# abusch/rustracer

Measured on AMD Instinct MI355X. Metric: Msamples/s, higher is better.
Workload: dtype f32; 1 GPU; cornell-box (synthetic S1, 32 triangles, 2 area lights) 1024x1024 PathIntegrator maxdepth=5 1024spp 02sequence box-filter; sampler_mode=pixel-keyed, light_distribution=cached across frames; first-frame build 32.0 ms

## Files before the change

include/rtx_hip.h:

```cpp
#ifndef RTX_HIP_H
#define RTX_HIP_H

#include <stdint.h>

#ifdef __cplusplus
extern "C" {
#endif

#define RT_OK 0
#define RT_ERR_INVALID (-1)
#define RT_ERR_NO_DEVICE (-2)
#define RT_ERR_HIP (-3)
#define RT_ERR_OOM (-4)
#define RT_ERR_UNSUPPORTED (-5)

typedef struct rt_bvh_node {
  float bmin[3];
  float bmax[3];
  uint32_t offset;
  uint16_t n_prims;
  uint8_t axis;
  uint8_t pad;
} rt_bvh_node;

// ... 132 lines not shown
  uint64_t camera_rays;
  uint64_t rays_closest, rays_shadow, rays_mis;
  uint64_t nodes_closest, nodes_shadow, nodes_mis;
  uint64_t tris_closest, tris_shadow, tris_mis;
  uint64_t paths_scrubbed;
  double ms_total;
  double ms_sampler, ms_raygen, ms_trace_closest, ms_trace_any, ms_trace_mis, ms_shade, ms_resolve, ms_film, ms_lightdist;
  uint64_t launches_trace_closest;
  uint64_t n_passes;
  uint64_t vertices_lambert_const, vertices_lambert, vertices_two_lobe, vertices_generic;
  double ms_shade_lambert_const, ms_shade_lambert, ms_shade_two_lobe, ms_shade_generic, ms_shade_bin, ms_shade_miss;
  uint64_t shade_section_cycles[32];
  uint64_t rays_mis_any, nodes_mis_any, tris_mis_any;
  double ms_trace_mis_any;
  double ms_gather;
  uint64_t rays_mis_not_cast;
  uint64_t rays_tail_not_cast;
  uint64_t launches_trace_path, launches_trace_shadow, launches_trace_mis, launches_trace_mis_any, launches_shade;
  uint64_t rays_shadow_not_cast;
} rt_stats;

#define RT_FLAG_COUNT_TRAVERSAL 1u
#define RT_FLAG_FILM_ON_DEVICE 2u
#define RT_FLAG_TIME_KERNELS 4u
#define RT_FLAG_COUNT_AS_RENDERED 8u
#define RT_FLAG_REF_STREAM 16u
#define RT_FLAG_FRAME_STATS 32u
#define RT_FLAG_FRAME_FEATURES 64u

typedef struct rt_scene rt_scene;

int rt_scene_create(const rt_scene_desc* desc, int device, rt_scene** out);
void rt_scene_destroy(rt_scene* scene);

int rt_bvh_build(const float* tri_p, uint32_t n_tris, int32_t max_prims_per_node, rt_bvh_node* nodes, uint32_t* n_nodes, int32_t* ordered,
                 float* ms_device );

int rt_mip_build(const float* rgb, int32_t width, int32_t height, int32_t px, int32_t py, const int32_t* s_first, const float* s_wts, const int32_t* t_first,
                 const float* t_wts, int32_t wrap, int32_t n_levels, const int32_t* lvl_w, const int32_t* lvl_h, const uint64_t* lvl_off, float* texels_out);
int rt_env_distribution(const rt_image* image, int32_t width, int32_t height, int32_t mode, int32_t il, float delta, const float* sin_theta,
                        float* func, float* cdf, float* func_int, float* marg_cdf, float* marg_func_int);

int rt_render(rt_scene* scene, const rt_camera* camera, const rt_film_desc* film, const rt_sampler_desc* sampler,
              const rt_path_desc* path, const rt_shard* shard, uint32_t flags, void* stream, float* film_xyzw, rt_stats* stats);

typedef struct rt_multi rt_multi;
int rt_multi_create(const rt_scene_desc* desc, const int32_t* devices, int32_t n_devices, rt_multi** out);
void rt_multi_destroy(rt_multi* multi);
int rt_multi_render(rt_multi* multi, const rt_camera* camera, const rt_film_desc* film, const rt_sampler_desc* sampler, const rt_path_desc* path,
                    int32_t chunks_per_device, uint32_t flags, float* film_xyzw, rt_stats* total, rt_stats* per_device);

int rt_trace_closest(rt_scene* scene, const float* rays, uint64_t n, float* hits, uint64_t counters[2]);
int rt_trace_any(rt_scene* scene, const float* rays, uint64_t n, uint32_t* occluded, uint64_t counters[2]);
int rt_trace_closest_device(rt_scene* scene, const void* d_rays, uint64_t n, void* d_hits, int reps, void* stream, float* ms_per_launch);

int rt_sampler_tables(int32_t spp, int32_t dimensions, uint64_t pixel0, uint64_t n_pixels, uint32_t* scrambles, uint16_t* perms);
int rt_sampler_tables_plain(int32_t spp, int32_t dimensions, uint64_t pixel0, uint64_t n_pixels, uint32_t* scrambles, uint16_t* perms);

int rt_offset_ray_origin(const float* p, const float* p_error, const float* n, const float* w, uint64_t count, float* out);

int rt_fourier_eval(rt_scene* scene, int32_t material, uint64_t n, const float* wo, const float* wi, const float* u, float* out);

int rt_texture_eval(rt_scene* scene, int32_t texture, uint64_t n, const float* records, float* rgb_out);

enum { RT_BSDF_FRONT_AUTO = 0, RT_BSDF_FRONT_GENERIC = 1, RT_BSDF_FRONT_LAMBERT = 2, RT_BSDF_FRONT_TWO_LOBE = 3, RT_BSDF_FRONT_TWO_LOBE_WIDE = 4 };
#define RT_BSDF_SURFACE_FLOATS 40
#define RT_BSDF_OUT_FLOATS 13
int rt_bsdf_eval(rt_scene* scene, int32_t material, int32_t front_end, uint64_t n, const float* surface, const float* wo, const float* wi, const float* u,
                 float* out);

#define RT_SAMPLES_MAX 134217728
int rt_render_samples(rt_scene* scene, const rt_camera* camera, const rt_film_desc* film, const rt_sampler_desc* sampler, const rt_path_desc* path,
                      uint32_t flags, void* stream, float* radiance, float* p_film, rt_stats* stats);

#define RT_FEATURE_FLOATS 16
#define RT_FEATURE_SAMPLES_MAX 33554432
int rt_render_sample_features(rt_scene* scene, const rt_camera* camera, const rt_film_desc* film, const rt_sampler_desc* sampler, const rt_path_desc* path,
                              uint32_t flags, void* stream, float* features);

enum { RT_FRAME_XYZW = 0, RT_FRAME_RGB = 1, RT_FRAME_RGB8 = 2, RT_FRAME_STATS = 3, RT_FRAME_FEATURES = 4 };
enum { RT_FRAME_SAMPLES_DONE = 0, RT_FRAME_SPP = 1, RT_FRAME_TABLES_RESIDENT = 2, RT_FRAME_STATE_BYTES = 3, RT_FRAME_SAMPLES_TAKEN = 4, RT_FRAME_ACTIVE_PIXELS = 5 };
typedef struct rt_frame rt_frame;
int rt_frame_begin(rt_scene* scene, const rt_camera* camera, const rt_film_desc* film, const rt_sampler_desc* sampler, const rt_path_desc* path,
                   const rt_shard* shard , uint32_t flags, uint64_t table_budget_bytes, rt_frame** out);
int rt_frame_advance(rt_frame* frame, int32_t n_samples, void* stream, rt_stats* stats );
int rt_frame_advance_adaptive(rt_frame* frame, int32_t n_samples, float threshold, float floor_y, int32_t min_samples, void* stream, rt_stats* stats );
int rt_frame_read(rt_frame* frame, int32_t what, float scale, uint32_t flags, void* stream, void* out);
int rt_frame_query(rt_frame* frame, int32_t what, uint64_t* value);
void rt_frame_end(rt_frame* frame);

typedef struct rt_multi_frame rt_multi_frame;
int rt_multi_frame_begin(rt_multi* multi, const rt_camera* camera, const rt_film_desc* film, const rt_sampler_desc* sampler, const rt_path_desc* path,
                         uint32_t flags, uint64_t table_budget_bytes, rt_multi_frame** out);
int rt_multi_frame_advance(rt_multi_frame* frame, int32_t n_samples, rt_stats* total , rt_stats* per_device );
int rt_multi_frame_advance_adaptive(rt_multi_frame* frame, int32_t n_samples, float threshold, float floor_y, int32_t min_samples, rt_stats* total, rt_stats* per_device);
int rt_multi_frame_read(rt_multi_frame* frame, int32_t what, float scale, uint32_t flags, void* out);
int rt_multi_frame_query(rt_multi_frame* frame, int32_t what, uint64_t* value);
void rt_multi_frame_end(rt_multi_frame* frame);

int rt_light_distribution(rt_scene* scene, int32_t n_voxels[3], float* func, float* cdf, float* func_int);

enum { RT_QUERY_LDS_RESIDENT = 0, RT_QUERY_LDS_NODES_TESTED = 1 ,
       RT_QUERY_LDS_OCCLUSION = 2 ,
       RT_QUERY_SHADOW_PAIRS = 3 ,
       RT_QUERY_SHADOW_EMPTY = 4 ,
       RT_QUERY_BSDF_LAUNCHED = 5  };
int rt_scene_query(rt_scene* scene, int32_t what);
int rt_link_tables(const rt_scene_desc* desc, int32_t mid, uint32_t* link_kept, uint32_t* link_full, uint64_t capacity_words, double* stats);
int rt_shadow_sets(const rt_scene_desc* desc, uint32_t* words, uint64_t capacity_words, int32_t n_voxels[3], uint64_t* stats);
int rt_sizeof(const char* struct_name);

const char* rt_last_error(void);
int rt_device_available(void);
const char* rt_version(void);

#ifdef __cplusplus
}
#endif
#endif
```

include/rtx_host.h:

```cpp
#ifndef RTX_HOST_H
#define RTX_HOST_H
#include <stdint.h>
#include "rtx_hip.h"

#ifdef __cplusplus
extern "C" {
#endif

typedef struct rtxh_scene rtxh_scene;

typedef struct rtxh_render_params {
  int32_t xres, yres;
  float crop[4];
  int32_t filter_kind;
  float filter_params[4];
  float film_scale, max_sample_luminance;
  float cam_to_world[16], cam_to_world_inv[16];
  float fov, lens_radius, focal_distance;
  int32_t spp, sampler_dims;
  int32_t max_depth; float rr_threshold; int32_t light_strategy;
  int32_t pixel_bounds[4];
  int32_t rank, world_size;
  uint32_t flags;
  float screen_window[4];
// ... 26 lines not shown
int rtxh_texture_words(rtxh_scene*, int32_t texture, float* out, int32_t capacity);
int rtxh_scene_add_material(rtxh_scene*, int32_t kind, const int32_t* slots16, int32_t remap_roughness, int32_t bump_texture );
int rtxh_scene_add_light(rtxh_scene*, int32_t kind, int32_t tri, const float* rgb3, int32_t two_sided, const float* vec3, int32_t mip,
                         const float* l2w16, const float* w2l16);
int rtxh_scene_commit(rtxh_scene*, int32_t max_prims_per_node);
int rtxh_scene_commit_device_bvh(rtxh_scene*, int32_t max_prims_per_node, float* ms_device);
int rtxh_scene_upload(rtxh_scene*, int32_t device);

int rtxh_scene_bvh_sizes(rtxh_scene*, int32_t* n_nodes, int32_t* n_prims);
int rtxh_scene_bvh_get(rtxh_scene*, float* bounds6, uint32_t* offset, uint16_t* n_prims, uint8_t* axis, int32_t* ordered);
int rtxh_camera_film_setup(const rtxh_render_params*, float* raster_to_camera16, float* dxdy6, float* filter_table256, int32_t* sample_bounds4,
                           int32_t* cropped4);
int rtxh_mip_level(rtxh_scene*, int32_t mip, int32_t level, int32_t* w, int32_t* h, float* rgb_out );
enum { RTXH_TABLE_TEXTURES = 0, RTXH_TABLE_MATERIALS, RTXH_TABLE_LIGHTS, RTXH_TABLE_P, RTXH_TABLE_N, RTXH_TABLE_UV, RTXH_TABLE_S, RTXH_TABLE_INDICES,
       RTXH_TABLE_TRI_MATERIAL, RTXH_TABLE_TRI_LIGHT, RTXH_TABLE_TRI_FLAGS,
       RTXH_TABLE_ENV_FUNC, RTXH_TABLE_ENV_CDF, RTXH_TABLE_ENV_ROW_INT, RTXH_TABLE_ENV_MARG_CDF,
       RTXH_TABLE_INSTANCES,
       RTXH_TABLE_EMITTERS,
       RTXH_TABLE_QUADRICS,
       RTXH_TABLE_OBJECT_BASE = 1000 ,
       RTXH_TABLE_OBJECT_EXTRA_BASE = 100000  };
typedef struct rtxh_emitter_info { float rgb[3]; int32_t two_sided; } rtxh_emitter_info;
typedef struct rtxh_instance_info { int32_t object; float o2w[16], w2o[16]; } rtxh_instance_info;
typedef struct rtxh_light_info { int32_t kind, tri; float rgb[3]; int32_t two_sided; float vec[3]; int32_t mip; float l2w[12], w2l[12]; } rtxh_light_info;
int rtxh_scene_inspect(rtxh_scene*, int32_t table, void* out, uint64_t capacity_bytes, uint64_t* n_items);
int rtxh_look_at(const float* pos, const float* look, const float* up, float* m16, float* m_inv16);

int rtxh_render(rtxh_scene*, const rtxh_render_params*, void* hip_stream, float* film_xyzw, rt_stats* stats);
int rtxh_render_samples(rtxh_scene*, const rtxh_render_params*, void* hip_stream, float* radiance, float* p_film, rt_stats* stats);
int rtxh_render_sample_features(rtxh_scene*, const rtxh_render_params*, void* hip_stream, float* features);
typedef struct rtxh_frame rtxh_frame;
int rtxh_frame_begin(rtxh_scene*, const rtxh_render_params*, uint64_t table_budget_bytes, rtxh_frame** out);
int rtxh_frame_advance(rtxh_frame*, int32_t n_samples, void* hip_stream, rt_stats* stats );
int rtxh_frame_advance_adaptive(rtxh_frame*, int32_t n_samples, float threshold, float floor_y, int32_t min_samples, void* hip_stream, rt_stats* stats );
int rtxh_frame_read(rtxh_frame*, int32_t what, float scale, uint32_t flags, void* hip_stream, void* out);
int rtxh_frame_query(rtxh_frame*, int32_t what, uint64_t* value);
void rtxh_frame_end(rtxh_frame*);
int rtxh_render_multi(rtxh_scene*, const rtxh_render_params*, const int32_t* devices, int32_t n_devices, int32_t chunks_per_device, float* film_xyzw,
                      rt_stats* total, rt_stats* per_device );
typedef struct rtxh_multi_frame rtxh_multi_frame;
int rtxh_multi_frame_begin(rtxh_scene*, const rtxh_render_params*, const int32_t* devices, int32_t n_devices, uint64_t table_budget_bytes, rtxh_multi_frame** out);
int rtxh_multi_frame_advance(rtxh_multi_frame*, int32_t n_samples, rt_stats* total, rt_stats* per_device);
int rtxh_multi_frame_advance_adaptive(rtxh_multi_frame*, int32_t n_samples, float threshold, float floor_y, int32_t min_samples, rt_stats* total, rt_stats* per_device);
int rtxh_multi_frame_read(rtxh_multi_frame*, int32_t what, float scale, uint32_t flags, void* out);
int rtxh_multi_frame_query(rtxh_multi_frame*, int32_t what, uint64_t* value);
void rtxh_multi_frame_end(rtxh_multi_frame*);
int rtxh_trace(rtxh_scene*, const float* rays, uint64_t n, int32_t any_hit, float* hits4_or_occ, uint64_t counters[2]);
int rtxh_trace_device(rtxh_scene*, const void* d_rays, uint64_t n, void* d_hits, int32_t reps, void* hip_stream, float* ms_per_launch);
int rtxh_light_distribution(rtxh_scene*, int32_t n_voxels[3], float* func, float* cdf, float* func_int);
int rtxh_scene_query(rtxh_scene*, int32_t what);
int rtxh_scene_device(rtxh_scene*, rt_scene** out);
int rtxh_scene_link_tables(rtxh_scene*, int32_t mid, uint32_t* link_kept, uint32_t* link_full, uint64_t capacity_words, double* stats);
int rtxh_scene_shadow_sets(rtxh_scene*, uint32_t* words, uint64_t capacity_words, int32_t n_voxels[3], uint64_t* stats);
int rtxh_sizeof(const char* struct_name);
const char* rtxh_last_error(void);

typedef struct rtxh_ply {
  int32_t n_verts, n_tris;
  float* P;
  float* N;
  float* UV;
  int32_t* idx;
  int32_t n_dropped_faces;
} rtxh_ply;
int rtxh_ply_read(const char* path, rtxh_ply* out);
void rtxh_ply_free(rtxh_ply* ply);
int rtxh_pfm_read(const char* path, int32_t* width, int32_t* height, float** rgb);
void rtxh_free(void* p);
int rtxh_image_read(const char* path, int32_t* width, int32_t* height, float** rgb);

int rtxh_spectrum_from_sampled(const float* lambda_nm, const float* values, int32_t n, float rgb[3]);
int rtxh_spectrum_blackbody(float temperature_kelvin, float scale, float rgb[3]);
void rtxh_copper(float eta_rgb[3], float k_rgb[3]);

typedef struct rtxh_pbrt_result {
  rtxh_scene* scene;
  rtxh_render_params params;
  int32_t max_prims_per_node;
  int32_t n_warnings;
  char film_filename[512];
} rtxh_pbrt_result;
int rtxh_pbrt_load(const char* path, rtxh_pbrt_result* out);
int rtxh_pbrt_parse(const char* text, const char* base_dir, rtxh_pbrt_result* out);
int rtxh_pbrt_tokens(const char* text, char* out, uint64_t capacity);

#ifdef __cplusplus
}
#endif
#endif
```

rustracer_amd/csrc/rtx_hip.hip:

```cpp
#include <hip/hip_runtime.h>
#include <chrono>
#include <cmath>
#include <cstdio>
#include <cstring>
#include <string>
#include <vector>
#include <limits>
#include <algorithm>
#include <memory>
#include <atomic>
#include <mutex>
#include <thread>

#include "../../include/rtx_hip.h"
#include "rtx_kernels.h"
#include "rtx_shade_launch.h"
#include "rtx_ref_launch.h"

using namespace rtx;
#include "rtx_scene_plan.h"

static thread_local std::string g_err;
static int fail(int code, const std::string& msg) { g_err = msg; return code; }
static bool env_is(const char* name, char c) { const char* e = getenv(name); return e && e[0] == c; }
// ... 10 lines not shown
  hipError_t ensure(size_t n) {
    if (n <= bytes && p) return hipSuccess;
    if (p) { (void)hipFree(p); p = nullptr; bytes = 0; }
    hipError_t e = hipMalloc(&p, n > 0 ? n : 16);
    if (e == hipSuccess) bytes = n;
    return e;
  }
  void release() { if (p) (void)hipFree(p); p = nullptr; bytes = 0; }
  template <class T> T* as() const { return (T*)p; }
};

struct SamplerPlan {
  unsigned spp = 0, dims = 0, seg_len = 0, n_segs = 0;
  DevBuf segs, magic, dirty, partners;
};

struct rt_scene {
  int device = 0;
  SamplerPlan sampler_plan;
  DScene d{};
  bool small = false;
  bool lambert_materials = false;
  bool lds_records_q = false;
  bool lds_tables = false;
  bool lds_mats = false;
  bool lds_records = false;
  bool lambert_only = false;
  bool lean_qlights = false;
  bool lean_shade = false;
  int stack_depth = 64;
  unsigned n_nodes = 0, n_tris = 0; int n_lights = 0;
  DevBuf link8, link8_full; unsigned lds_nodes_tested = 0;
  DevBuf pairs, tmin_stack;
  DevBuf top_pairs, deep_stack; bool use_top = false;
  bool top_for_closest = false;
  bool use_pairs = false;
  bool deep_column = false;
  DevBuf quads; bool use_quads = false; int quad_stack_depth = 0;
  DevBuf tri_rec;
  DevBuf nodes, tri_p, tri_n, tri_uv, tri_s, tri_alpha, spheres, textures, images, materials, lights, texels, dist, guides, prim_class;
  DevBuf fourier;
  std::vector<int> mat_kind, mat_table;
  std::vector<uint64_t> fourier_at;
  bool has_spheres = false;
  bool has_instances = false;
  DevBuf instances;
  bool mid = false;
  bool general_prims = false;
  bool obj_general = false;
  bool has_masks = false;
  bool masked_emitters = false;
  DevBuf ld_func, ld_cdf, ld_int, ld_mark, ld_list, ld_slot, ld_guide, ld_rows8, ld_dense8;
  bool shadow_sets = false; RtShadowSets shadow; DevBuf ld_shadow;
  DevBuf self;
  int ld_strategy_built = -1; bool ld_all_voxels = false;
  std::mutex render_mutex;
  DevBuf ws[32];
  DevBuf film_acc, own_acc, film_out, counters, stats, filter_table, ref_samples, ref_stack;
  DevBuf samples_rad, samples_pf;
  DevBuf samples_feat;
  DevBuf feat;
  DevBuf bsdf_self, bsdf_tris;
  int bsdf_launched = -1;
  std::vector<int> mat_class;
  DevBuf bin_words, bin_sorted, bin_at;
  unsigned n_materials = 0, n_code_classes = 0, n_lambert_classes = 0, n_small_classes = 0, n_wide_classes = 0;
  DevBuf scrambles[2], perms[2];
  hipStream_t aux_stream = nullptr;
  hipEvent_t ev_tables[2][3] = {{nullptr, nullptr, nullptr}, {nullptr, nullptr, nullptr}}, ev_batch_done[2] = {nullptr, nullptr}, ev_frame_begin = nullptr;
  int n_cu = 256;
  std::vector<hipEvent_t> event_pool;
  ~rt_scene() {
    for (hipEvent_t e : event_pool) (void)hipEventDestroy(e);
    for (int i = 0; i < 2; ++i) { for (int g = 0; g < 3; ++g) if (ev_tables[i][g]) (void)hipEventDestroy(ev_tables[i][g]); if (ev_batch_done[i]) (void)hipEventDestroy(ev_batch_done[i]); }
    if (ev_frame_begin) (void)hipEventDestroy(ev_frame_begin);
    if (aux_stream) (void)hipStreamDestroy(aux_stream);
  }
};

extern "C" const char* rt_last_error(void) { return g_err.c_str(); }
extern "C" const char* rt_version(void) { return "rtx-mi355x 0.5 (gfx950 wavefront path tracer)"; }
extern "C" int rt_sizeof(const char* name) {
  if (!name) return -1;
#define RT_SZ(T) if (!strcmp(name, #T)) return (int)sizeof(T);
  RT_SZ(rt_bvh_node) RT_SZ(rt_tri_meta) RT_SZ(rt_sphere) RT_SZ(rt_instance) RT_SZ(rt_texture) RT_SZ(rt_image) RT_SZ(rt_material) RT_SZ(rt_light) RT_SZ(rt_scene_desc)
  RT_SZ(rt_camera) RT_SZ(rt_film_desc) RT_SZ(rt_sampler_desc) RT_SZ(rt_path_desc) RT_SZ(rt_shard) RT_SZ(rt_stats)
#undef RT_SZ
  return -1;
}
extern "C" int rt_device_available(void) {
  int n = 0;
  if (hipGetDeviceCount(&n) != hipSuccess || n <= 0) return 0;
  return 1;
}

static int upload(DevBuf& b, const void* src, size_t bytes) {
  HIP_TRY(b.ensure(bytes));
  if (bytes) HIP_TRY(hipMemcpy(b.p, src, bytes, hipMemcpyHostToDevice));
  return RT_OK;
}

static void fill_ewa_lut() {
  float lut[128];
  for (int i = 0; i < 128; ++i) {
    float alpha = 2.0f;
    float r2 = (float)i / (128.0f - 1.0f);
// ... 148 lines not shown
  a.material = material; a.surface = surface ? b[4].as<float4>() : nullptr; a.wo = b[0].as<float>(); a.wi = b[1].as<float>(); a.u = b[2].as<float>(); a.n = (unsigned)n; a.out = b[3].as<float>();
  const unsigned grid = (unsigned)std::min<uint64_t>((n + 255) / 256, (uint64_t)scene->n_cu * 16u);
  rtx_launch_bsdf_eval(mode, const_tex, grid, nullptr, d, a);
  HIP_TRY(hipGetLastError());
  scene->bsdf_launched = 2 * mode + (const_tex ? 1 : 0);
  HIP_TRY(hipMemcpy(out, b[3].p, no, hipMemcpyDeviceToHost));
  return RT_OK;
}
extern "C" int rt_link_tables(const rt_scene_desc* desc, int32_t mid, uint32_t* link_kept, uint32_t* link_full, uint64_t capacity_words, double* stats) {
  if (!desc || !desc->nodes || desc->n_nodes == 0 || !desc->tri_p || !desc->tri_meta || !link_kept || !link_full) return fail(RT_ERR_INVALID, "null argument");
  const size_t words = (size_t)9 * desc->n_nodes + 9;
  if (desc->n_nodes > (mid ? RT_MID_NODES : RT_SMALL_NODES) || desc->n_tris > (uint64_t)(mid ? RT_MID_TRIS : RT_SMALL_TRIS) || desc->n_instances != 0) return fail(RT_ERR_INVALID, "not an LDS-sized scene");
  if (capacity_words < words) return fail(RT_ERR_INVALID, "link table capacity too small");
  {
    const uint32_t nn = desc->n_nodes;
    std::vector<uint32_t> size(nn, 1u);
    for (uint32_t i = nn; i-- > 0;) {
      const rt_bvh_node& n = desc->nodes[i];
      if (n.n_prims != 0) {
        if ((uint64_t)n.offset + n.n_prims > desc->n_tris) return fail(RT_ERR_INVALID, "leaf range out of bounds");
        if (n.n_prims >= (1u << (15 - RT_LINK_OFF_BITS(mid ? RT_MID_NODES : RT_SMALL_NODES)))) return fail(RT_ERR_INVALID, "a leaf holds more primitives than a link word can name");
        continue;
      }
      if (i + 1 >= nn || n.offset != i + 1 + size[i + 1] || n.offset >= nn) return fail(RT_ERR_INVALID, "nodes are not a pre-order tree");
      size[i] = 1u + size[i + 1] + size[n.offset];
    }
    if (size[0] != nn) return fail(RT_ERR_INVALID, "nodes are not one tree");
    for (uint64_t t = 0; t < desc->n_tris; ++t)
      if (desc->tri_meta[t].flags & RT_PRIM_SPHERE) {
        uint32_t k; memcpy(&k, desc->tri_p + 9 * t + 6, 4);
        if (!desc->spheres || k >= desc->n_spheres) return fail(RT_ERR_INVALID, "sphere index out of range");
      }
  }
  RtLinkTables lt;
  rt_build_link_tables(desc, mid != 0, stats != nullptr, lt);
  memcpy(link_kept, lt.link_kept.data(), words * 4); memcpy(link_full, lt.link_full.data(), words * 4);
  if (stats) for (int w = 0; w < 9; ++w) { stats[w] = (double)lt.n_rays[w]; stats[9 + w] = lt.tests_all[w]; stats[18 + w] = lt.tests_kept[w]; }
  return RT_OK;
}
extern "C" int rt_shadow_sets(const rt_scene_desc* desc, uint32_t* words, uint64_t capacity_words, int32_t n_voxels[3], uint64_t* stats) {
  if (!desc || !desc->nodes || desc->n_nodes == 0 || !desc->tri_p || !desc->tri_meta) return fail(RT_ERR_INVALID, "null argument");
  bool plain = desc->n_instances == 0 && desc->n_spheres == 0 && desc->n_nodes <= RT_SMALL_NODES && desc->n_tris <= RT_SMALL_TRIS;
  for (uint32_t i = 0; i < desc->n_tris && plain; ++i) if (desc->tri_meta[i].flags & ~(uint32_t)RT_SHADOW_PLAIN_FLAGS) plain = false;
  if (!shadow_sets_apply(desc, plain)) return fail(RT_ERR_INVALID, "not a scene the shadow sets serve (LDS-resident plain triangles, two triangle lights)");
  int32_t lp[2] = {0, 0};
  for (uint32_t k = 0; k < desc->n_lights; ++k) lp[k] = desc->lights[k].prim;
  RtShadowSets ss;
  rt_build_shadow_sets(desc->tri_p, desc->n_tris, lp, (int)desc->n_lights, desc->nodes[0].bmin, desc->nodes[0].bmax, ss);
  if (n_voxels) { n_voxels[0] = ss.nvox[0]; n_voxels[1] = ss.nvox[1]; n_voxels[2] = ss.nvox[2]; }
  if (stats) { stats[0] = ss.pairs; stats[1] = ss.empty; }
  if (words) {
    if (capacity_words < ss.word.size()) return fail(RT_ERR_INVALID, "rt_shadow_sets: capacity too small");
    std::memcpy(words, ss.word.data(), ss.word.size() * 4);
  }
  return RT_OK;
}

extern "C" int rt_scene_query(rt_scene* s, int32_t what) {
  if (!s) return fail(RT_ERR_INVALID, "null scene");
  if (what == RT_QUERY_LDS_RESIDENT) return s->small ? 1 : 0;
  if (what == RT_QUERY_LDS_NODES_TESTED) return (s->small || s->mid) ? (int)s->lds_nodes_tested : 0;
  if (what == RT_QUERY_LDS_OCCLUSION) return s->mid ? 1 : 0;
  if (what == RT_QUERY_SHADOW_PAIRS) return s->shadow_sets ? (int)s->shadow.pairs : 0;
  if (what == RT_QUERY_SHADOW_EMPTY) return s->shadow_sets ? (int)s->shadow.empty : 0;
  if (what == RT_QUERY_BSDF_LAUNCHED) return s->bsdf_launched < 0 ? 0 : s->bsdf_launched + 1;
  return fail(RT_ERR_INVALID, "unknown rt_scene_query item");
}

static int build_light_distribution(rt_scene* s, int strategy, hipStream_t stream, bool all_voxels = false) {
  DScene& d = s->d;
  if (s->ld_strategy_built == strategy && (s->ld_all_voxels || !all_voxels)) return RT_OK;
  s->ld_strategy_built = -1;
  const int nl = s->n_lights;
  size_t ld_rows_built = 1;
  const bool uniform = strategy == 1 || nl == 1 || nl == 0;
  int glog = -1;
  if (nl >= 64 && nl <= 65534) { const long q = guide_quarters(); glog = 0; while (glog < 16 && (long)(2 << glog) * q <= 4l * nl) ++glog; }
  d.ld_glog = glog; d.ld_guide = nullptr;
  if (uniform) {
    const int n = nl > 0 ? nl : 1;
    std::vector<float> func(n, 1.0f), cdf(n + 1, 0.0f);
    for (int i = 1; i < n + 1; ++i) cdf[i] = cdf[i - 1] + func[i - 1] / (float)n;
    float func_int = cdf[n];
    if (func_int == 0.0f) for (int i = 1; i < n + 1; ++i) cdf[i] = (float)i / (float)n;
    else for (int i = 1; i < n + 1; ++i) cdf[i] /= func_int;
    int rc;
    if ((rc = upload(s->ld_func, func.data(), func.size() * 4)) != RT_OK) return rc;
    if ((rc = upload(s->ld_cdf, cdf.data(), cdf.size() * 4)) != RT_OK) return rc;
    if ((rc = upload(s->ld_int, &func_int, 4)) != RT_OK) return rc;
    if (glog >= 0) {
      const int G = 1 << glog; std::vector<unsigned short> g((size_t)G + 1); int i = 0;
      for (int k = 0; k <= G; ++k) { const float x = (float)k / (float)G; while (i <= n && cdf[i] <= x) ++i; g[k] = (unsigned short)i; }
      if ((rc = upload(s->ld_guide, g.data(), g.size() * 2)) != RT_OK) return rc;
    }
    d.ld_uniform = 1; d.nvox[0] = d.nvox[1] = d.nvox[2] = 1;
  } else {
    float diag[3] = {d.wb_max.x - d.wb_min.x, d.wb_max.y - d.wb_min.y, d.wb_max.z - d.wb_min.z};
    int ext = diag[0] > diag[1] ? (diag[0] > diag[2] ? 0 : 2) : (diag[1] > diag[2] ? 1 : 2);
    float b_max = diag[ext];
    size_t total = 1;
    for (int i = 0; i < 3; ++i) {
      float r = roundf(diag[i] / b_max * 64.0f);
      unsigned v = (r != r || r <= 0.0f) ? 0u : (unsigned)r;
      d.nvox[i] = (int)(v > 1u ? v : 1u);
      total *= (size_t)d.nvox[i];
    }
// ... 93 lines not shown
static size_t deep_stack_bytes(const rt_scene* s) {
  if (!s->use_top) return 0;
  return (size_t)std::max(top_grid(s), top_grid(s, true)) * RT_TOP_BLOCK * (size_t)std::max(1, s->stack_depth - RT_TOP_LDS_DEPTH) * 4;
}
static int scene_from_plan(const RtScenePlan& p, const rt_scene_desc* desc, int device, rt_scene** out) {
  if (device >= 0) HIP_TRY(hipSetDevice(device));
  int dev = 0; HIP_TRY(hipGetDevice(&dev));
  std::unique_ptr<rt_scene> owner(new rt_scene());
  rt_scene* s = owner.get();
  s->device = dev;
  hipDeviceProp_t prop; if (hipGetDeviceProperties(&prop, dev) == hipSuccess) s->n_cu = prop.multiProcessorCount;
  s->n_nodes = desc->n_nodes; s->n_tris = desc->n_tris; s->n_lights = (int)desc->n_lights; s->n_materials = desc->n_materials;
  s->small = p.small; s->mid = p.mid; s->general_prims = p.general_prims; s->obj_general = p.obj_general; s->has_masks = p.has_masks; s->has_spheres = p.has_spheres;
  s->has_instances = p.has_instances; s->masked_emitters = p.masked_emitters; s->lambert_only = p.lambert_only; s->lambert_materials = p.lambert_materials;
  s->lean_shade = p.lean_shade; s->lean_qlights = p.lean_qlights; s->lds_records = p.lds_records; s->lds_records_q = p.lds_records_q; s->lds_tables = p.lds_tables;
  s->lds_mats = p.lds_mats; s->use_pairs = p.use_pairs; s->use_top = p.use_top; s->top_for_closest = p.top_for_closest; s->use_quads = p.use_quads;
  s->deep_column = p.deep_column; s->shadow_sets = p.shadow_sets; s->shadow = p.shadow; s->stack_depth = p.stack_depth; s->quad_stack_depth = p.quad_stack_depth;
  s->mat_kind = p.mat_kind; s->mat_table = p.mat_table; s->mat_class = p.mat_class; s->fourier_at = p.fourier_at;
  s->n_code_classes = p.n_code_classes; s->n_lambert_classes = p.n_lambert_classes; s->n_small_classes = p.n_small_classes; s->n_wide_classes = p.n_wide_classes;
  if (s->mid) {
    int fit_any = 0, fit_closest = 0;
    if (hipOccupancyMaxActiveBlocksPerMultiprocessor(&fit_any, (const void*)(k_trace<true, false, 1024, 16, 0, 1>), 1024, 0) != hipSuccess) fit_any = 0;
    if (hipOccupancyMaxActiveBlocksPerMultiprocessor(&fit_closest, (const void*)(k_trace<false, false, 1024, 16, 0, 1>), 1024, 0) != hipSuccess) fit_closest = 0;
    (void)hipGetLastError();
    if (fit_any < 1 || fit_closest < 1) s->mid = false;
  }
  const bool links = s->small || s->mid;
  if (links) s->lds_nodes_tested = p.links.nodes_tested;
  int rc = RT_OK;
  auto up = [&rc](DevBuf& b, const void* src, size_t bytes) { if (rc == RT_OK) rc = upload(b, src, bytes); };
  auto up_all = [&up](DevBuf& b, const auto& v) { up(b, v.data(), v.size() * sizeof(v[0])); };
  auto room = [&rc](DevBuf& b, size_t bytes, const char* what) { if (rc == RT_OK && bytes && b.ensure(bytes) != hipSuccess) rc = fail(RT_ERR_OOM, what); };
  up(s->nodes, desc->nodes, sizeof(rt_bvh_node) * (size_t)desc->n_nodes);
  up_all(s->tri_p, p.tri_p);
  if (desc->tri_n) up(s->tri_n, desc->tri_n, (size_t)desc->n_tris * 36);
  if (desc->tri_uv) up(s->tri_uv, desc->tri_uv, (size_t)desc->n_tris * 24);
  if (desc->tri_s) up(s->tri_s, desc->tri_s, (size_t)desc->n_tris * 36);
  if (p.has_masks) up(s->tri_alpha, desc->tri_alpha, (size_t)desc->n_tris * 8);
  if (p.has_spheres) up(s->spheres, desc->spheres, (size_t)desc->n_spheres * sizeof(rt_sphere));
  if (p.has_instances) up_all(s->instances, p.instances);
  up_all(s->texels, p.texels); up_all(s->fourier, p.fourier);
  std::vector<DImage> images = p.images;
  for (DImage& im : images) im.texels = s->texels.as<float4>();
  up_all(s->images, images); up_all(s->textures, p.textures); up_all(s->materials, p.materials); up_all(s->prim_class, p.prim_class);
  up_all(s->dist, p.dist); up_all(s->guides, p.guides);
  std::vector<DLight> lights = p.lights;
  for (DLight& l : lights)
    if (l.kind == RT_LIGHT_INFINITE) {
      rt_blob_rebase(l.cf, s->dist.p); rt_blob_rebase(l.func_int, s->dist.p); rt_blob_rebase(l.mfunc, s->dist.p); rt_blob_rebase(l.mcdf, s->dist.p);
      rt_blob_rebase(l.guide, s->guides.p); rt_blob_rebase(l.mguide, s->guides.p);
    }
  up_all(s->lights, lights);
  if (links) { up_all(s->link8_full, p.links.link_full); up_all(s->link8, p.links.link_kept); }
  if (p.use_pairs) up_all(s->pairs, p.pairs);
  if (p.use_top) up_all(s->top_pairs, p.top_pairs);
  if (p.use_quads) up_all(s->quads, p.quads);
  room(s->tmin_stack, tmin_stack_bytes(s), "traversal stack allocation failed");
  room(s->deep_stack, deep_stack_bytes(s), "traversal stack allocation failed");
  room(s->tri_rec, (size_t)desc->n_tris * 128, "shade record allocation failed");
  room(s->self, sizeof(DScene), "scene record allocation failed");
  if (rc != RT_OK) return rc;
  DScene& d = s->d;
  d.nodes = s->nodes.as<float4>(); d.n_nodes = desc->n_nodes;
  d.tri_p = s->tri_p.as<float4>(); d.n_tris = desc->n_tris;
  d.tri_n = s->tri_n.as<float>(); d.tri_uv = s->tri_uv.as<float>(); d.tri_s = s->tri_s.as<float>();
  d.tri_alpha = s->tri_alpha.as<int2>();
  d.spheres = s->spheres.as<DSphere>();
  d.instances = s->instances.as<DInstance>(); d.n_instances = s->has_instances ? desc->n_instances : 0u; d.n_top_prims = p.n_top_prims;
  d.textures = s->textures.as<DTexture>(); d.images = s->images.as<DImage>(); d.materials = s->materials.as<DMaterial>(); d.lights = s->lights.as<DLight>();
  d.fourier = s->fourier.as<unsigned>();
  d.n_materials = (int)desc->n_materials; d.n_textures = (int)desc->n_textures; d.n_images = (int)desc->n_images;
  d.n_lights = (int)desc->n_lights; d.n_infinite = p.n_infinite;
  for (int k = 0; k < 4; ++k) d.infinite_ids[k] = p.infinite_ids[k];
  d.wb_min = f3{desc->nodes[0].bmin[0], desc->nodes[0].bmin[1], desc->nodes[0].bmin[2]};
  d.wb_max = f3{desc->nodes[0].bmax[0], desc->nodes[0].bmax[1], desc->nodes[0].bmax[2]};
  d.ld_uniform = 1; d.nvox[0] = d.nvox[1] = d.nvox[2] = 1; d.ld_glog = -1; d.ld_guide = nullptr;
  d.needs_differentials = p.needs_differentials;
#ifdef RT_ABLATE
  d.dbg = env_int("RTX_DBG", 0);
#endif
  d.obj_pairs = p.obj_pairs; d.obj_general = s->obj_general ? 1 : 0;
  d.link8_full = s->link8_full.as<unsigned>(); d.link8 = s->link8.as<unsigned>();
  d.pairs = s->pairs.as<float4>(); d.top_pairs = s->top_pairs.as<float4>(); d.n_top = (unsigned)(p.top_pairs.size() / 16); d.quads = s->quads.as<float4>();
  fill_ewa_lut();
  d.tri_rec = s->tri_rec.as<float4>();
  hipLaunchKernelGGL(k_tri_records, dim3((desc->n_tris + 255u) / 256u), dim3(256), 0, nullptr, d, s->tri_rec.as<float4>());
  d.n_lights_all = (int)p.n_all_lights;
  if (p.n_all_lights) hipLaunchKernelGGL(k_light_consts, dim3((p.n_all_lights + 255u) / 256u), dim3(256), 0, nullptr, d, s->lights.as<DLight>(), (int)p.n_all_lights);
  if (hipGetLastError() != hipSuccess) return fail(RT_ERR_HIP, "constant precomputation launch failed");
  d.prim_class = s->prim_class.as<unsigned short>();
  d.route_quadric_hits = p.route_quadric_hits;
  d.self = s->self.as<DScene>();
  HIP_TRY(hipMemcpy(s->self.p, &d, sizeof(DScene), hipMemcpyHostToDevice));
  HIP_TRY(hipDeviceSynchronize());
  *out = owner.release();
  return RT_OK;
}

extern "C" int rt_scene_create(const rt_scene_desc* desc, int device, rt_scene** out) {
  if (!desc || !out) return fail(RT_ERR_INVALID, "null argument");
  RtScenePlan plan; std::string why;
  if (const int rc = rt_plan_scene(desc, plan, why)) return fail(rc, why);
  if (!rt_device_available()) return fail(RT_ERR_NO_DEVICE, "no HIP device visible; this backend has no CPU fallback");
  return scene_from_plan(plan, desc, device, out);
}
static bool inst_loop_kernel(const rt_scene* s) { return s->has_instances && !s->has_masks && !s->has_spheres && s->use_pairs && s->d.obj_pairs; }
// ... 61 lines not shown
        if (s->use_quads && s->quad_stack_depth <= 32) {
          RT_GEN_LAUNCH3((k_trace_quad<128, 32, RT_GEN_ALL>), (k_trace_quad<128, 32, RT_GEN_NO_MASKS>), (k_trace_quad<128, 32, RT_GEN_INSTANCES_ONLY>), (trace_grid<ANY, false, 128, 32>(s)), 128, RT_KARGS, s->tmin_stack.as<float>(), refill_min);
          return;
        }
      }
      if (s->use_pairs && s->use_top && (ANY || s->top_for_closest)) {
        RT_GEN_LAUNCH((k_trace_top<ANY, RT_TOP_BLOCK, RT_GEN_ALL>), (k_trace_top<ANY, RT_TOP_BLOCK, RT_GEN_NO_MASKS>), (top_grid(s, ANY)), RT_TOP_BLOCK, RT_KARGS, s->tmin_stack.as<float>(), s->deep_stack.as<unsigned>(), refill_min);
        return;
      }
      if (s->use_pairs) {
        if (s->stack_depth <= 32) RT_GEN_LAUNCH3((k_trace_pair<ANY, 128, 32, RT_GEN_ALL>), (k_trace_pair<ANY, 128, 32, RT_GEN_NO_MASKS>), (k_trace_pair<ANY, 128, 32, RT_GEN_INSTANCES_ONLY>), (trace_grid<ANY, false, 128, 32>(s)), 128, RT_KARGS, s->tmin_stack.as<float>(), refill_min);
        else RT_GEN_LAUNCH3((k_trace_pair<ANY, 128, 64, RT_GEN_ALL>), (k_trace_pair<ANY, 128, 64, RT_GEN_NO_MASKS>), (k_trace_pair<ANY, 128, 64, RT_GEN_INSTANCES_ONLY>), (trace_grid<ANY, false, 128, 64>(s)), 128, RT_KARGS, s->tmin_stack.as<float>(), refill_min);
        return;
      }
#undef RT_GEN_LAUNCH3
#undef RT_GEN_LAUNCH
    }
    if (s->stack_depth > 64) hipLaunchKernelGGL((k_trace_big<ANY, COUNT, 64, 128, true>), dim3(trace_grid<ANY, false, 64, 128>(s)), dim3(64), 0, stream, RT_KARGS, st_nodes, st_tris);
    else if (s->stack_depth <= 32) hipLaunchKernelGGL((k_trace_big<ANY, COUNT, 128, 32, true>), dim3(trace_grid<ANY, false, 128, 32>(s)), dim3(128), 0, stream, RT_KARGS, st_nodes, st_tris);
    else hipLaunchKernelGGL((k_trace_big<ANY, COUNT, 128, 64, true>), dim3(trace_grid<ANY, false, 128, 64>(s)), dim3(128), 0, stream, RT_KARGS, st_nodes, st_tris);
    return;
  }
  if constexpr (!COUNT) {
    if (s->mid && (ANY || mid_closest_on())) {
      hipLaunchKernelGGL((k_trace<ANY, false, 1024, 16, 0, 1>), dim3((unsigned)s->n_cu), dim3(1024), 0, stream, RT_KARGS, st_nodes, st_tris);
      return;
    }
    if (s->small) {
      hipLaunchKernelGGL((k_trace<ANY, false, 256, 16>), dim3(trace_grid<ANY, true, 256, 16>(s, true)), dim3(256), 0, stream, RT_KARGS, st_nodes, st_tris);
      return;
    }
  }
  if (s->small) {
    if (s->stack_depth <= 16) hipLaunchKernelGGL((k_trace<ANY, true, 256, 16>), dim3(trace_grid<ANY, true, 256, 16>(s)), dim3(256), 0, stream, RT_KARGS, st_nodes, st_tris);
    else if (s->stack_depth <= 32) hipLaunchKernelGGL((k_trace<ANY, true, 256, 32>), dim3(trace_grid<ANY, true, 256, 32>(s)), dim3(256), 0, stream, RT_KARGS, st_nodes, st_tris);
    else hipLaunchKernelGGL((k_trace<ANY, true, 128, 64>), dim3(trace_grid<ANY, true, 128, 64>(s)), dim3(128), 0, stream, RT_KARGS, st_nodes, st_tris);
  } else {
    if (s->stack_depth <= 32) launch_trace_hbm<ANY, COUNT, 128, 32>(RT_ARGS);
    else launch_trace_hbm<ANY, COUNT, 128, 64>(RT_ARGS);
  }
#undef RT_KARGS
#undef RT_ARGS
}
static bool closest_is_k_trace(const rt_scene* s, bool count) {
  if (s->general_prims) return !count && !s->obj_general && s->small;
  return s->small || (!count && s->mid && mid_closest_on());
}
template <bool ANY>
static void launch_trace(rt_scene* s, bool count, const TraceIO& io, const unsigned* queue, const unsigned* count_ptr, unsigned shard_cap, unsigned count_static,
                         unsigned long long* stats, int st_rays, int st_nodes, int st_tris, hipStream_t stream) {
  if (count) launch_trace_c<ANY, true>(s, io, queue, count_ptr, shard_cap, count_static, stats, st_rays, st_nodes, st_tris, stream);
  else launch_trace_c<ANY, false>(s, io, queue, count_ptr, shard_cap, count_static, stats, st_rays, st_nodes, st_tris, stream);
}
static TraceIO trace_io_planar(const float4* ro, const float4* rd, float4* hits, unsigned* occ) {
  TraceIO io{}; io.ray_o = ro; io.ray_d = rd; io.ray_stride = 1; io.hits = hits; io.hit_stride = 1; io.hit_b2 = 0; io.occluded = occ; io.occ_stride = 1;
  io.shadow_masks = 1;
  return io;
}

static int trace_batch(rt_scene* s, const float* rays, uint64_t n, bool any, float* hits, uint32_t* occluded, uint64_t counters[2]) {
  if (!s || !rays || n == 0 || n > 0x7fffffffull) return fail(RT_ERR_INVALID, "bad trace batch");
  HIP_TRY(hipSetDevice(s->device));
  DevBuf ro, rd, out, st;
  HIP_TRY(ro.ensure(n * 16)); HIP_TRY(rd.ensure(n * 16)); HIP_TRY(out.ensure(n * 16)); HIP_TRY(st.ensure(ST_COUNT * 8));
  std::vector<float> o(n * 4), d(n * 4);
  for (uint64_t i = 0; i < n; ++i) {
    const float* r = rays + 8 * i;
    o[4 * i] = r[0]; o[4 * i + 1] = r[1]; o[4 * i + 2] = r[2]; o[4 * i + 3] = r[3];
    d[4 * i] = r[4]; d[4 * i + 1] = r[5]; d[4 * i + 2] = r[6]; d[4 * i + 3] = 0.0f;
  }
  HIP_TRY(hipMemcpy(ro.p, o.data(), n * 16, hipMemcpyHostToDevice));
  HIP_TRY(hipMemcpy(rd.p, d.data(), n * 16, hipMemcpyHostToDevice));
  HIP_TRY(hipMemset(st.p, 0, ST_COUNT * 8));
  const TraceIO io = trace_io_planar(ro.as<float4>(), rd.as<float4>(), any ? nullptr : out.as<float4>(), any ? out.as<unsigned>() : nullptr);
  if (any) launch_trace<true>(s, counters != nullptr, io, nullptr, nullptr, 0, (unsigned)n, st.as<unsigned long long>(), ST_RAYS_SHADOW, ST_NODES_SHADOW, ST_TRIS_SHADOW, nullptr);
  else launch_trace<false>(s, counters != nullptr, io, nullptr, nullptr, 0, (unsigned)n, st.as<unsigned long long>(), ST_RAYS_CLOSEST, ST_NODES_CLOSEST, ST_TRIS_CLOSEST, nullptr);
  HIP_TRY(hipGetLastError());
  HIP_TRY(hipDeviceSynchronize());
  if (any) HIP_TRY(hipMemcpy(occluded, out.p, n * 4, hipMemcpyDeviceToHost));
  else HIP_TRY(hipMemcpy(hits, out.p, n * 16, hipMemcpyDeviceToHost));
  if (counters) {
    unsigned long long h[ST_COUNT];
    HIP_TRY(hipMemcpy(h, st.p, sizeof(h), hipMemcpyDeviceToHost));
    counters[0] = any ? h[ST_NODES_SHADOW] : h[ST_NODES_CLOSEST];
    counters[1] = any ? h[ST_TRIS_SHADOW] : h[ST_TRIS_CLOSEST];
  }
  return RT_OK;
}
extern "C" int rt_trace_closest(rt_scene* s, const float* rays, uint64_t n, float* hits, uint64_t counters[2]) { return trace_batch(s, rays, n, false, hits, nullptr, counters); }
extern "C" int rt_trace_any(rt_scene* s, const float* rays, uint64_t n, uint32_t* occluded, uint64_t counters[2]) { return trace_batch(s, rays, n, true, nullptr, occluded, counters); }

extern "C" int rt_trace_closest_device(rt_scene* s, const void* d_rays, uint64_t n, void* d_hits, int reps, void* stream_, float* ms_per_launch) {
  if (!s || !d_rays || !d_hits || n == 0 || reps <= 0) return fail(RT_ERR_INVALID, "bad arguments");
  HIP_TRY(hipSetDevice(s->device));
  hipStream_t stream = (hipStream_t)stream_;
  const float4* ro = (const float4*)d_rays; const float4* rd = ro + n;
  hipEvent_t e0, e1; HIP_TRY(hipEventCreate(&e0)); HIP_TRY(hipEventCreate(&e1));
  HIP_TRY(hipEventRecord(e0, stream));
  const TraceIO io = trace_io_planar(ro, rd, (float4*)d_hits, nullptr);
  for (int i = 0; i < reps; ++i) launch_trace<false>(s, false, io, nullptr, nullptr, 0, (unsigned)n, nullptr, 0, 0, 0, stream);
  HIP_TRY(hipEventRecord(e1, stream));
  HIP_TRY(hipEventSynchronize(e1));
  float ms = 0; HIP_TRY(hipEventElapsedTime(&ms, e0, e1));
  if (ms_per_launch) *ms_per_launch = ms / (float)reps;
  (void)hipEventDestroy(e0); (void)hipEventDestroy(e1);
  return RT_OK;
}

static unsigned next_pow2(unsigned v) { unsigned p = 1; while (p < v) p <<= 1; return p; }
static unsigned sampler_lanes_per_block(unsigned spp) {
  unsigned l = (32u * 1024u) / ((spp + 2u) * 2u);
  if (l >= 64u) return 64u;
  if (l >= 32u) return 32u;
  if (l >= 16u) return 16u;
  if (l >= 8u) return 8u;
  return 4u;
}

static void pcg_advance_constants(unsigned long long n, unsigned long long& mul, unsigned long long& sum) {
  unsigned long long cur_mul = 0x5851f42d4c957f2dULL, cur_sum = 1ull;
  mul = 1ull; sum = 0ull;
  while (n) {
    if (n & 1ull) { sum = sum * cur_mul + cur_sum; mul *= cur_mul; }
    cur_sum = (cur_mul + 1ull) * cur_sum; cur_mul *= cur_mul;
    n >>= 1;
  }
}
static int sampler_plan_prepare(SamplerPlan& pl, unsigned spp_, unsigned dims_) {
  unsigned &spp = pl.spp, &dims = pl.dims, &seg_len = pl.seg_len, &n_segs = pl.n_segs;
  DevBuf &segs = pl.segs, &magic = pl.magic, &dirty = pl.dirty;
  {
    if (spp == spp_ && dims == dims_ && segs.p) return RT_OK;
    seg_len = spp_ < 256u ? spp_ : 256u;
    const unsigned per_half = spp_ / seg_len;
    std::vector<SamplerSeg> h;
    unsigned long long pos = 0;
    for (unsigned t = 0; t < 2u * dims_; ++t) {
      const unsigned n_scr = t < dims_ ? 1u : 2u;
      for (unsigned half = 0; half < 2u; ++half)
        for (unsigned g = 0; g < per_half; ++g) {
          SamplerSeg sg{};
          const bool first = half == 0u && g == 0u;
          const unsigned long long start = first ? pos : pos + n_scr + (unsigned long long)half * spp_ + (unsigned long long)g * seg_len;
// ... 317 lines not shown
    for (const Want& w : want) if (!w.buf->p || w.buf->bytes < w.bytes) grow += w.bytes;
    size_t held = 0;
    for (const Want& w : want) if (w.buf->p && w.buf->bytes < w.bytes) held += w.buf->bytes;
    size_t mem_free = 0, mem_total = 0;
    HIP_TRY(hipMemGetInfo(&mem_free, &mem_total));
    if (grow > mem_free + held - std::min<size_t>(mem_free + held, (size_t)256 << 20)) continue;
    bool ok = true;
    for (const Want& w : want) if (w.buf->ensure(w.bytes) != hipSuccess) { ok = false; break; }
    if (ok) break;
    (void)hipGetLastError();
  }
  if (!s->aux_stream) {
    int lo = 0, hi = 0; (void)hipDeviceGetStreamPriorityRange(&lo, &hi);
    HIP_TRY(hipStreamCreateWithPriority(&s->aux_stream, hipStreamNonBlocking, lo));
    for (int i = 0; i < 2; ++i) { for (int g = 0; g < 3; ++g) HIP_TRY(hipEventCreateWithFlags(&s->ev_tables[i][g], hipEventDisableTiming)); HIP_TRY(hipEventCreateWithFlags(&s->ev_batch_done[i], hipEventDisableTiming)); }
    HIP_TRY(hipEventCreateWithFlags(&s->ev_frame_begin, hipEventDisableTiming));
  }
  float4* const d_out = (flags & RT_FLAG_FILM_ON_DEVICE) ? (float4*)film_xyzw : s->film_out.as<float4>();
  float4* const d_samples_rad = (flags & RT_FLAG_FILM_ON_DEVICE) ? (float4*)samples_rad : s->samples_rad.as<float4>();
  float2* const d_samples_pf = !samples_pf ? nullptr : ((flags & RT_FLAG_FILM_ON_DEVICE) ? (float2*)samples_pf : s->samples_pf.as<float2>());
  FeatureOut fo{};
  if (fsamples) { fo.samples = (flags & RT_FLAG_FILM_ON_DEVICE) ? (float4*)samples_feat : s->samples_feat.as<float4>(); fo.wx0 = wx0; fo.wy0 = wy0; fo.ww = wx1 - wx0; }
  else if (features) { fo.nd = s->feat.as<float4>(); fo.ah = fo.nd + cap; }
  if (!samples && !fsamples && !fr) {
    HIP_TRY(hipMemcpyAsync(s->filter_table.p, film->filter_table, 1024, hipMemcpyHostToDevice, stream));
    HIP_TRY(hipMemsetAsync(s->film_acc.p, 0, (size_t)cw * ch * 16, stream));
  }
  HIP_TRY(hipMemsetAsync(s->stats.p, 0, ST_COUNT * 8, stream));

  PassState ps{};
  ps.spp = spp; ps.spp_log2 = spp_log2; ps.dims = dims;
  auto gen_of = [&](int b) { PathGen g; char* p = (char*)s->ws[b].p; g.o = (float4*)p; g.d = (float4*)(p + n_slots * 16); g.beta = (float4*)(p + n_slots * 32); g.st = (uint4*)(p + n_slots * 48); return g; };
  const PathGen gen0 = gen_of(B_GEN0), gen1 = gen_of(B_GEN1);
  ps.hit = s->ws[B_HIT].as<float4>(); ps.lacc = s->ws[B_LACC].as<float4>(); ps.pfilm = s->ws[B_PFILM].as<float2>();
  { char* p = (char*)s->ws[B_SH].p; ps.sh.o = (float4*)p; ps.sh.d = (float4*)(p + cap * 16); ps.sh.add = (float4*)(p + cap * 32);
    char* q = (char*)s->ws[B_MI].p; ps.mi.o = (float4*)q; ps.mi.d = (float4*)(q + cap * 16); ps.mi.hit = (float4*)(q + cap * 32); ps.mi.a = (float4*)(q + cap * 48);
    ps.mi.b = (float4*)(q + cap * 64); ps.mi.c = (float4*)(q + cap * 80); ps.mi.flags = (unsigned*)(q + cap * 96); }
  ps.occ_sh = s->ws[B_OCCSH].as<unsigned char>(); ps.occ_mi = s->ws[B_OCCMI].as<unsigned char>();
  ps.q_shadow = s->ws[B_QSH].as<unsigned>(); ps.q_mis = s->ws[B_QMI].as<unsigned>(); ps.q_misany = s->ws[B_QMA].as<unsigned>();
  ps.own_acc = s->own_acc.as<float4>(); ps.shard_cap = shard_cap;
  ps.stats = s->stats.as<unsigned long long>();

  if ((rc = sampler_plan_prepare(s->sampler_plan, spp, dims)) != RT_OK) return rc;
  if ((rc = sampler_set_lds_limits(spp)) != RT_OK) return rc;
  TraceIO io_path{}, io_shadow{}, io_mis{}, io_mis_any{};
  {
    io_path.ray_stride = 1; io_path.hits = ps.hit; io_path.hit_stride = 1; io_path.hit_b2 = 1; io_path.queue_is_slots = 1;
    io_shadow.ray_o = ps.sh.o; io_shadow.ray_d = ps.sh.d; io_shadow.ray_stride = 1; io_shadow.occluded = (unsigned*)ps.occ_sh; io_shadow.occ_stride = 0;
    io_shadow.shadow_masks = 1; io_shadow.lacc = ps.lacc; io_shadow.lacc_stride = 1; io_shadow.direct_add = ps.sh.add; io_shadow.add_stride = 1;
    io_mis.ray_o = ps.mi.o; io_mis.ray_d = ps.mi.d; io_mis.ray_stride = 1; io_mis.hits = ps.mi.hit; io_mis.hit_stride = 1; io_mis.hit_b2 = 0;
    io_mis_any = io_mis; io_mis_any.shadow_masks = 0; io_mis_any.hits = nullptr; io_mis_any.occluded = (unsigned*)ps.occ_mi; io_mis_any.occ_stride = 0;
  }
  const bool count = (flags & RT_FLAG_COUNT_TRAVERSAL) != 0;
  const unsigned pgrid = (unsigned)s->n_cu * 8u;
  const unsigned sblock = 256u, sgrid = pgrid;
  unsigned long long* dstats = s->stats.as<unsigned long long>();

  const char* ov = getenv("RTX_K0_OVERLAP");
  hipStream_t aux = (ov && ov[0] == '0') ? stream : s->aux_stream;
  if (build_tables) {
    HIP_TRY(hipEventRecord(s->ev_frame_begin, stream));
    HIP_TRY(hipStreamWaitEvent(aux, s->ev_frame_begin, 0));
  }
  int tables_rc = RT_OK;
  std::vector<std::pair<unsigned long long, unsigned long long>> batches;
  for (unsigned long long first = 0; first < owned_pixels;) {
    const unsigned long long npx = (first == 0 && lead_pixels) ? lead_pixels : std::min(chunk_pixels, owned_pixels - first);
    batches.push_back({first, npx}); first += npx;
  }
  if (resident && !fr->tables_built) {
    fr->scr_off.clear(); fr->perm_off.clear();
    size_t so = 0, po = 0;
    for (const auto& b : batches) {
      fr->scr_off.push_back(so); fr->perm_off.push_back(po);
      so += ((size_t)b.second * 3 * dims * 4 + 255) & ~(size_t)255; po += ((size_t)(b.second * table_bytes_per_pixel) + 255) & ~(size_t)255;
    }
    if (so > fr->scrambles.bytes || po > fr->perms.bytes) return fail(RT_ERR_INVALID, "rt_frame_advance: the batches' sampler tables do not fit the frame's buffers");
  }
  if (resident && fr->scr_off.size() != batches.size()) return fail(RT_ERR_INVALID, "rt_frame_advance: the batch cut changed under resident sampler tables");
  auto scrambles_of = [&](size_t b, int buf) { return resident ? (unsigned*)((char*)fr->scrambles.p + fr->scr_off[b]) : s->scrambles[buf].as<unsigned>(); };
  auto perms_of = [&](size_t b, int buf) { return resident ? (unsigned short*)((char*)fr->perms.p + fr->perm_off[b]) : s->perms[buf].as<unsigned short>(); };
  TableGroups tgroups = table_groups_frame(dims, !(fp.lens_radius > 0.0f));
  auto launch_tables = [&](size_t b, int buf) {
    FrameParams f2 = fp; f2.chunk_first = batches[b].first;
    tm.begin(&stats.ms_sampler, aux);
    const int trc = launch_sampler_tables(s->sampler_plan, f2, (unsigned)batches[b].second, 0ull, 0, scrambles_of(b, buf), perms_of(b, buf), aux, tgroups, s->ev_tables[buf]);
    if (trc != RT_OK && tables_rc == RT_OK) tables_rc = trc;
    tm.end(aux);
  };
  if (!batches.empty() && build_tables) launch_tables(0, 0);
  for (size_t batch_no = 0; batch_no < batches.size(); ++batch_no) {
    const unsigned long long first = batches[batch_no].first, npx = batches[batch_no].second;
    const int buf = (int)(batch_no & 1ull);
    fp.chunk_first = first;
    ps.n_pixels = (unsigned)npx; ps.n_pixels_recip = npx > 1 ? (unsigned)((1ull << 32) / npx) : 0xffffffffu;
    ps.scrambles = scrambles_of(batch_no, buf); ps.perms = perms_of(batch_no, buf);
    if (build_tables && batch_no + 1 < batches.size()) {
      if (batch_no >= 1 && !resident) HIP_TRY(hipStreamWaitEvent(aux, s->ev_batch_done[buf ^ 1], 0));
      launch_tables(batch_no + 1, buf ^ 1);
    }
    const unsigned batch_pass_samples = (unsigned)std::min<unsigned long long>(spp, std::max<unsigned long long>(pass_samples, cap / npx));
    if (tables_rc != RT_OK) { (void)hipDeviceSynchronize(); return tables_rc; }
    if (build_tables) HIP_TRY(hipStreamWaitEvent(stream, s->ev_tables[buf][0], 0));
    for (unsigned s0 = s_begin; s0 < s_end; s0 += batch_pass_samples) {
      ps.s0 = s0; ps.n_samples = std::min(batch_pass_samples, s_end - s0); ps.cap = (unsigned)(npx * ps.n_samples);
      ps.q_in = nullptr; ps.in = gen1; ps.out = gen0;
      HIP_TRY(hipMemsetAsync(s->counters.p, 0, counter_words * 4, stream));
      if (use_bins) HIP_TRY(hipMemsetAsync(s->bin_words.p, 0, (size_t)(fp.max_depth + 1) * bin_stride * 4, stream));
      unsigned* const cb = s->counters.as<unsigned>();
      ps.cnt_in = nullptr; ps.cnt_out = cb;
      ps.all_in_bounds = all_in_bounds ? 1 : 0;
      const int fresh_planes = all_in_bounds ? ((s->lambert_only && s->lds_records) ? (shade_split ? 3 : RT_FRESH_RECORDS_LDS) : RT_FRESH_RECORDS) : 0;
      ps.fresh = fresh_planes;
      ps.shadow_sets = (s->shadow_sets && !count) ? 1 : 0;
      ps.mis_any = (has_infinite && (!count || (flags & RT_FLAG_COUNT_AS_RENDERED))) ? 1 : 0;
      static const bool reach_off = env_is("RTX_MIS_REACH", '0');
      ps.skip_unreachable_mis = (!reach_off && (!count || (flags & RT_FLAG_COUNT_AS_RENDERED))) ? 1 : 0;
      static const bool tail_off = env_is("RTX_DEAD_TAIL", '0');
      ps.skip_dead_tail = (!tail_off && (!count || (flags & RT_FLAG_COUNT_AS_RENDERED))) ? 1 : 0;
      const int skip_dead_tail = ps.skip_dead_tail;
      tm.begin(&stats.ms_raygen);
      if (active_mask) hipLaunchKernelGGL(k_raygen_masked, dim3(pgrid), dim3(256), 0, stream, fp, ps, active_mask);
      else hipLaunchKernelGGL(k_raygen, dim3(pgrid), dim3(256), 0, stream, fp, ps);
      tm.end();
      for (int bounce = 0; bounce <= fp.max_depth; ++bounce) {
        ps.cnt_in = cb + (size_t)bounce * RT_NQ * RT_QSHARDS * RT_CNT_STRIDE; ps.cnt_out = cb + (size_t)(bounce + 1) * RT_NQ * RT_QSHARDS * RT_CNT_STRIDE;
        std::swap(ps.in, ps.out);
        if (bounce == 0 && all_in_bounds) ps.cnt_in = nullptr;
        ps.skip_dead_tail = (features && bounce == 0 && fp.max_depth == 1) ? 0 : skip_dead_tail;
        ps.fresh = bounce == 0 ? fresh_planes : 0;
        io_path.ray_o = ps.in.o; io_path.ray_d = ps.in.d;
        const bool split_launch = shade_split && (bounce >= 1 || all_in_bounds);
        io_path.hit_mask = split_launch ? s->ws[B_HITMASK].as<unsigned long long>() : nullptr;
        tm.begin(&stats.ms_trace_closest);
        launch_trace<false>(s, count, io_path, ps.cnt_in, ps.cnt_in, ps.shard_cap, ps.cap, dstats, ST_RAYS_CLOSEST, ST_NODES_CLOSEST, ST_TRIS_CLOSEST, stream);
        tm.end();
        if (bounce <= 1 && build_tables) HIP_TRY(hipStreamWaitEvent(stream, s->ev_tables[buf][bounce + 1], 0));
#define RT_SHADE(MODE, P) stats.launches_shade += 1, launch_shade<MODE>(gshade, lean_shade, bounce >= 1, sgrid, sblock, stream, s->d, fp, P, qlights, lds_shade)
        if (s->lambert_only) {
          tm.begin(&stats.ms_shade_lambert_const);
          if (split_launch) rtx_launch_shade_split(bounce == 0, sgrid, stream, s->d, fp, ps, io_path.hit_mask);
          else rtx_launch_shade_const(s->lds_records ? 1 : (s->lds_tables ? 3 : 0), sgrid, sblock, stream, s->d, fp, ps);
          tm.end(); stats.launches_shade += 1;
        }
        else if (s->lambert_materials) { tm.begin(&stats.ms_shade_lambert); RT_SHADE(3, ps); tm.end(); }
        else if (!use_bins) { tm.begin(&stats.ms_shade_generic); RT_SHADE(0, ps); tm.end(); }
        else {
          tm.begin(&stats.ms_shade_bin);
          unsigned* bw = s->bin_words.as<unsigned>() + (size_t)bounce * bin_stride;
          unsigned* hist = bw; unsigned* cursor = bw + (RT_BIN_MAX + 1); unsigned* sorted_cnt = cursor + (size_t)(RT_BIN_MAX + 1) * RT_CNT_STRIDE;
          hipLaunchKernelGGL(k_bin_count, dim3(pgrid), dim3(256), 0, stream, s->d, ps, n_bins, hist, s->bin_at.as<unsigned short>());
          unsigned* ranges = sorted_cnt + (size_t)RT_QSHARDS * RT_CNT_STRIDE;
#define RT_BIN_ARGS dim3(pgrid), dim3(256), 0, stream, s->d, ps, n_bins, hist, cursor, s->bin_sorted.as<unsigned>(), sorted_cnt, split_classes ? n_first : 0u, split_classes ? n_first + n_second : 0u, \
                    split_classes ? n_first + n_second + n_third : 0u, ranges, s->bin_at.as<unsigned short>()
          hipLaunchKernelGGL(k_bin_scatter, RT_BIN_ARGS);
#undef RT_BIN_ARGS
          tm.end();
          PassState pb = ps; pb.q_in = s->bin_sorted.as<unsigned>(); pb.cnt_in = sorted_cnt;
          if (split_classes && n_first) { pb.range = ranges; tm.begin(&stats.ms_shade_lambert); RT_SHADE(3, pb); tm.end(); }
          if (split_classes && n_second) { pb.range = ranges + 2; tm.begin(&stats.ms_shade_two_lobe); RT_SHADE(5, pb); tm.end(); }
          if (split_classes && n_third) { pb.range = ranges + 8; tm.begin(&stats.ms_shade_two_lobe); RT_SHADE(6, pb); tm.end(); }
          pb.range = ranges + 4; tm.begin(&stats.ms_shade_generic); RT_SHADE(0, pb); tm.end();
          pb.range = ranges + 6; tm.begin(&stats.ms_shade_miss); hipLaunchKernelGGL(k_shade_miss, dim3(pgrid), dim3(256), 0, stream, s->d, pb); tm.end();
        }
#undef RT_SHADE
        if (features && bounce == 0) {
          tm.begin(&stats.ms_film);
          rtx_launch_feature_hits(fsamples, s->has_spheres || s->has_instances, pgrid, stream, s->d, fp, ps, fo);
          if (fsamples) hipLaunchKernelGGL(k_feature_albedo<true>, dim3(pgrid), dim3(256), 0, stream, fp, ps, fo);
          else hipLaunchKernelGGL(k_feature_albedo<false>, dim3(pgrid), dim3(256), 0, stream, fp, ps, fo);
          tm.end();
          if (fsamples) break;
        }
        tm.begin(&stats.ms_trace_any);
        launch_trace<true>(s, count, io_shadow, ps.q_shadow, ps.cnt_out + RT_QSHARDS * RT_CNT_STRIDE, ps.shard_cap, 0, dstats, ST_RAYS_SHADOW, ST_NODES_SHADOW, ST_TRIS_SHADOW, stream);
        tm.end();
        tm.begin(&stats.ms_trace_mis);
        launch_trace<false>(s, count, io_mis, ps.q_mis, ps.cnt_out + 2 * RT_QSHARDS * RT_CNT_STRIDE, ps.shard_cap, 0, dstats, ST_RAYS_MIS, ST_NODES_MIS, ST_TRIS_MIS, stream);
        tm.end();
        if (ps.mis_any) {
          tm.begin(&stats.ms_trace_mis_any);
          launch_trace<true>(s, count, io_mis_any, ps.q_misany, ps.cnt_out + 3 * RT_QSHARDS * RT_CNT_STRIDE, ps.shard_cap, 0, dstats, ST_RAYS_MISANY, ST_NODES_MISANY, ST_TRIS_MISANY, stream);
          tm.end();
        }
        tm.begin(&stats.ms_resolve);
        if (s->has_spheres || s->has_instances) hipLaunchKernelGGL(k_resolve<true>, dim3(pgrid), dim3(256), 0, stream, s->d, ps);
        else hipLaunchKernelGGL(k_resolve<false>, dim3(pgrid), dim3(256), 0, stream, s->d, ps);
        tm.end();
        stats.launches_trace_closest += 2; stats.launches_trace_path += 1; stats.launches_trace_mis += 1; stats.launches_trace_shadow += 1; stats.launches_trace_mis_any += ps.mis_any ? 1 : 0;
      }
      tm.begin(&stats.ms_film);
      if (fsamples) { }
      else if (samples) hipLaunchKernelGGL(k_sample_store, dim3(pgrid), dim3(256), 0, stream, fp, ps, wx0, wy0, wx1 - wx0, d_samples_rad, d_samples_pf);
      else if (fr && fr->stats) hipLaunchKernelGGL(k_film_accumulate_frame_stats, dim3(pgrid), dim3(256), 0, stream, fp, ps, fr->filter_table.as<float>(), fr->film_acc.as<float4>(), fr->own_acc.as<float4>(), fr->moments.as<PixMoments>());
      else if (fr) hipLaunchKernelGGL(k_film_accumulate_frame, dim3(pgrid), dim3(256), 0, stream, fp, ps, fr->filter_table.as<float>(), fr->film_acc.as<float4>(), fr->own_acc.as<float4>());
      else hipLaunchKernelGGL(k_film_accumulate, dim3(pgrid), dim3(256), 0, stream, fp, ps, s->filter_table.as<float>(), s->film_acc.as<float4>());
      if (fr && fr->features) hipLaunchKernelGGL(k_feature_accumulate, dim3(pgrid), dim3(256), 0, stream, fp, ps, fo.nd, fo.ah, fr->feature_plane.as<PixFeatures>());
      tm.end();
      stats.n_passes += 1;
      HIP_TRY(hipGetLastError());
    }
    HIP_TRY(hipEventRecord(s->ev_batch_done[buf], stream));
  }
  if (fr) {
    if (resident && build_tables) {
      HIP_TRY(hipStreamSynchronize(aux));
      fr->tables_built = true; fr->batch_pixels = batch_pixels; fr->lead_pixels = lead_pixels;
    }
  } else if (fsamples) {
    if (!(flags & RT_FLAG_FILM_ON_DEVICE)) HIP_TRY(hipMemcpyAsync(samples_feat, fo.samples, (size_t)n_window_samples * RT_FEATURE_FLOATS * 4, hipMemcpyDeviceToHost, stream));
  } else if (!samples) {
    tm.begin(&stats.ms_film);
    {
      unsigned long long n = (unsigned long long)cw * ch;
      hipLaunchKernelGGL(k_film_finalize, dim3((unsigned)((n + 255) / 256)), dim3(256), 0, stream, s->film_acc.as<float4>(), d_out, n);
    }
    tm.end();
    HIP_TRY(hipGetLastError());
    if (!(flags & RT_FLAG_FILM_ON_DEVICE)) HIP_TRY(hipMemcpyAsync(film_xyzw, d_out, (size_t)cw * ch * 16, hipMemcpyDeviceToHost, stream));
  } else if (!(flags & RT_FLAG_FILM_ON_DEVICE)) {
    HIP_TRY(hipMemcpyAsync(samples_rad, d_samples_rad, (size_t)n_window_samples * 16, hipMemcpyDeviceToHost, stream));
    if (samples_pf) HIP_TRY(hipMemcpyAsync(samples_pf, d_samples_pf, (size_t)n_window_samples * 8, hipMemcpyDeviceToHost, stream));
  }
  HIP_TRY(hipStreamSynchronize(stream));
  tm.collect();
  stats.ms_shade = stats.ms_shade_lambert_const + stats.ms_shade_lambert + stats.ms_shade_two_lobe + stats.ms_shade_generic + stats.ms_shade_bin + stats.ms_shade_miss;
  unsigned long long h[ST_COUNT];
  HIP_TRY(hipMemcpy(h, s->stats.p, sizeof(h), hipMemcpyDeviceToHost));
// ... 567 lines not shown
```

rustracer_amd/csrc/rtx_host.cpp:

```cpp
#include "../../include/rtx_host.h"

#include <algorithm>
#include <array>
#include <initializer_list>
#include <map>
#include <atomic>
#include <thread>
#include <cmath>
#include <cstdio>
#include <cstdlib>
#include <cstring>
#include <limits>
#include <sstream>
#include <string>
#include <vector>

namespace {

thread_local std::string g_err;
int fail(int code, const std::string& m) { g_err = m; return code; }

struct Box { float lo[3], hi[3]; };
const float kFmax = std::numeric_limits<float>::max();
inline Box box_empty() { return Box{{kFmax, kFmax, kFmax}, {-kFmax, -kFmax, -kFmax}}; }
// ... 1343 lines not shown
  if (!f || !value) return fail(RT_ERR_INVALID, "rtxh_multi_frame_query: null argument");
  g_err.clear();
  return rt_multi_frame_query(f->f, what, value);
}
void rtxh_multi_frame_end(rtxh_multi_frame* f) {
  if (!f) return;
  rt_multi_frame_end(f->f);
  f->scene->multi_frames -= 1;
  delete f;
}
int rtxh_trace(rtxh_scene* s, const float* rays, uint64_t n, int32_t any_hit, float* out, uint64_t counters[2]) {
  if (!s) return fail(RT_ERR_INVALID, "null scene");
  g_err.clear();
  if (!s->dev) { int rc = rtxh_scene_upload(s, -1); if (rc != RT_OK) return rc; }
  return any_hit ? rt_trace_any(s->dev, rays, n, (uint32_t*)out, counters) : rt_trace_closest(s->dev, rays, n, out, counters);
}
int rtxh_trace_device(rtxh_scene* s, const void* d_rays, uint64_t n, void* d_hits, int32_t reps, void* stream, float* ms) {
  if (!s) return fail(RT_ERR_INVALID, "null scene");
  g_err.clear();
  if (!s->dev) { int rc = rtxh_scene_upload(s, -1); if (rc != RT_OK) return rc; }
  return rt_trace_closest_device(s->dev, d_rays, n, d_hits, reps, stream, ms);
}
int rtxh_light_distribution(rtxh_scene* s, int32_t n_voxels[3], float* func, float* cdf, float* func_int) {
  if (!s) return fail(RT_ERR_INVALID, "null scene");
  g_err.clear();
  if (!s->dev) { int rc = rtxh_scene_upload(s, -1); if (rc != RT_OK) return rc; }
  return rt_light_distribution(s->dev, n_voxels, func, cdf, func_int);
}
int rtxh_scene_query(rtxh_scene* s, int32_t what) {
  if (!s) return fail(RT_ERR_INVALID, "null scene");
  g_err.clear();
  if (!s->dev) { int rc = rtxh_scene_upload(s, -1); if (rc != RT_OK) return rc; }
  return rt_scene_query(s->dev, what);
}
int rtxh_scene_device(rtxh_scene* s, rt_scene** out) {
  if (!s || !out) return fail(RT_ERR_INVALID, "null argument");
  g_err.clear();
  if (!s->dev) { int rc = rtxh_scene_upload(s, -1); if (rc != RT_OK) return rc; }
  *out = s->dev;
  return RT_OK;
}
int rtxh_scene_link_tables(rtxh_scene* s, int32_t mid, uint32_t* link_kept, uint32_t* link_full, uint64_t capacity_words, double* stats) {
  if (!s || !s->committed) return fail(RT_ERR_INVALID, "scene not committed");
  g_err.clear();
  rt_scene_desc d = make_desc(s);
  return rt_link_tables(&d, mid, link_kept, link_full, capacity_words, stats);
}
int rtxh_scene_shadow_sets(rtxh_scene* s, uint32_t* words, uint64_t capacity_words, int32_t n_voxels[3], uint64_t* stats) {
  if (!s || !s->committed) return fail(RT_ERR_INVALID, "scene not committed");
  g_err.clear();
  rt_scene_desc d = make_desc(s);
  return rt_shadow_sets(&d, words, capacity_words, n_voxels, stats);
}
int rtxh_sizeof(const char* name) {
  if (!name) return -1;
#define RTXH_SZ(T) if (!strcmp(name, #T)) return (int)sizeof(T);
  RTXH_SZ(rtxh_render_params) RTXH_SZ(rtxh_emitter_info) RTXH_SZ(rtxh_instance_info) RTXH_SZ(rtxh_light_info) RTXH_SZ(rtxh_ply) RTXH_SZ(rtxh_pbrt_result)
#undef RTXH_SZ
  return rt_sizeof(name);
}


namespace {
struct PlyProp { std::string name; int type = -1; bool is_list = false; int count_type = -1; };
struct PlyElem { std::string name; size_t count = 0; std::vector<PlyProp> props; };
int ply_type_id(const std::string& t) {
  static const char* names[][2] = {{"char", "int8"}, {"uchar", "uint8"}, {"short", "int16"}, {"ushort", "uint16"}, {"int", "int32"}, {"uint", "uint32"}, {"float", "float32"}, {"double", "float64"}};
  for (int i = 0; i < 8; ++i) if (t == names[i][0] || t == names[i][1]) return i;
  return -1;
}
const int kPlySize[8] = {1, 1, 2, 2, 4, 4, 4, 8};
struct PlyReader {
  FILE* f = nullptr; int format = 0;
  bool read_scalar(int type, double& out) {
    if (format == 0) { return fscanf(f, "%lf", &out) == 1; }
    unsigned char b[8]; const int n = kPlySize[type];
    if (fread(b, 1, (size_t)n, f) != (size_t)n) return false;
    if (format == 2) for (int i = 0; i < n / 2; ++i) std::swap(b[i], b[n - 1 - i]);
    switch (type) {
      case 0: { int8_t v; memcpy(&v, b, 1); out = v; break; }
      case 1: { uint8_t v; memcpy(&v, b, 1); out = v; break; }
      case 2: { int16_t v; memcpy(&v, b, 2); out = v; break; }
      case 3: { uint16_t v; memcpy(&v, b, 2); out = v; break; }
      case 4: { int32_t v; memcpy(&v, b, 4); out = v; break; }
      case 5: { uint32_t v; memcpy(&v, b, 4); out = v; break; }
      case 6: { float v; memcpy(&v, b, 4); out = v; break; }
      default: { double v; memcpy(&v, b, 8); out = v; break; }
    }
    return true;
  }
};
}

static int ply_read_unguarded(const char* path, rtxh_ply* out);
int rtxh_ply_read(const char* path, rtxh_ply* out) {
  if (!path || !out) return fail(RT_ERR_INVALID, "null argument");
  g_err.clear();
  memset(out, 0, sizeof(*out));
  try { return ply_read_unguarded(path, out); }
  catch (const std::bad_alloc&) { rtxh_ply_free(out); return fail(RT_ERR_OOM, std::string("out of memory while reading ") + path); }
  catch (const std::exception& e) { rtxh_ply_free(out); return fail(RT_ERR_INVALID, std::string(e.what()) + " (" + path + ")"); }
}
static int ply_read_unguarded(const char* path, rtxh_ply* out) {
  PlyReader rd; rd.f = fopen(path, "rb");
  if (!rd.f) return fail(RT_ERR_INVALID, std::string("cannot open ") + path);
  struct Closer { FILE* f; ~Closer() { if (f) fclose(f); } } closer{rd.f};
// ... 180 lines not shown
```

rustracer_amd/csrc/rtx_kernels.h:

```cpp
#pragma once
#include <type_traits>
#include "rtx_dev_shading.h"

namespace rtx {


#ifndef RT_NT_STREAMS
#define RT_NT_STREAMS 1
#endif
#if RT_NT_STREAMS
typedef float nt_v4f __attribute__((ext_vector_type(4)));
typedef unsigned nt_v4u __attribute__((ext_vector_type(4)));
typedef float nt_v2f __attribute__((ext_vector_type(2)));
RT_DEV float4 nt_ld(const float4* p) { const nt_v4f v = __builtin_nontemporal_load((const nt_v4f*)p); return make_float4(v.x, v.y, v.z, v.w); }
RT_DEV uint4 nt_ld(const uint4* p) { const nt_v4u v = __builtin_nontemporal_load((const nt_v4u*)p); return make_uint4(v.x, v.y, v.z, v.w); }
RT_DEV float2 nt_ld(const float2* p) { const nt_v2f v = __builtin_nontemporal_load((const nt_v2f*)p); return make_float2(v.x, v.y); }
RT_DEV unsigned nt_ld(const unsigned* p) { return __builtin_nontemporal_load(p); }
RT_DEV unsigned char nt_ld(const unsigned char* p) { return __builtin_nontemporal_load(p); }
RT_DEV void nt_st(float4 a, float4* p) { nt_v4f v; v.x = a.x; v.y = a.y; v.z = a.z; v.w = a.w; __builtin_nontemporal_store(v, (nt_v4f*)p); }
RT_DEV void nt_st(uint4 a, uint4* p) { nt_v4u v; v.x = a.x; v.y = a.y; v.z = a.z; v.w = a.w; __builtin_nontemporal_store(v, (nt_v4u*)p); }
RT_DEV void nt_st(float2 a, float2* p) { nt_v2f v; v.x = a.x; v.y = a.y; __builtin_nontemporal_store(v, (nt_v2f*)p); }
RT_DEV void nt_st(unsigned a, unsigned* p) { __builtin_nontemporal_store(a, p); }
RT_DEV void nt_st(unsigned char a, unsigned char* p) { __builtin_nontemporal_store(a, p); }
template <class T> struct NtRef {
  T* p;
  RT_DEV operator T() const { return nt_ld((const T*)p); }
  RT_DEV void operator=(const T& v) const { nt_st(v, p); }
};
template <class T> struct NtPtr {
  typedef typename std::remove_const<T>::type V;
  T* p;
  __host__ __device__ NtPtr() : p(nullptr) {}
  __host__ __device__ NtPtr(T* q) : p(q) {}
  template <class U> __host__ __device__ NtPtr(const NtPtr<U>& q) : p(q.p) {}
  RT_DEV typename std::conditional<std::is_const<T>::value, V, NtRef<V>>::type operator[](size_t i) const { if constexpr (std::is_const<T>::value) return nt_ld(p + i); else return NtRef<V>{p + i}; }
  __host__ __device__ explicit operator bool() const { return p != nullptr; }
  __host__ __device__ bool operator!=(std::nullptr_t) const { return p != nullptr; }
  __host__ __device__ bool operator==(std::nullptr_t) const { return p == nullptr; }
};
template <class T> using SPtr = NtPtr<T>;
#define RT_SPTR_R(T) NtPtr<T>
template <class T> __host__ __device__ T* sraw(NtPtr<T> q) { return q.p; }
template <bool NT, class T> RT_DEV typename std::conditional<NT, NtPtr<T>, T*>::type sp(NtPtr<T> q) { if constexpr (NT) return q; else return q.p; }
#else
template <class T> using SPtr = T*;
#define RT_SPTR_R(T) T* __restrict__
template <class T> __host__ __device__ T* sraw(T* q) { return q; }
template <bool NT, class T> RT_DEV T* sp(T* q) { return q; }
#endif
struct PathGen { SPtr<float4> o; SPtr<float4> d; SPtr<float4> beta; SPtr<uint4> st; };
struct ShadowPlanes { SPtr<float4> o; SPtr<float4> d; SPtr<float4> add; };
struct MisPlanes { SPtr<float4> o; SPtr<float4> d; SPtr<float4> hit; SPtr<float4> a; SPtr<float4> b; SPtr<float4> c; SPtr<unsigned> flags; };
#define RT_PEND_SHADOW 1u
#define RT_PEND_MIS_ANY 0x40000000u
struct PassState {
  unsigned cap;
  unsigned spp, spp_log2, dims;
  unsigned n_pixels;
  unsigned n_pixels_recip;
  unsigned s0, n_samples;
  float4* own_acc;
  const unsigned* scrambles;
  const unsigned short* perms;
  PathGen in, out;
  SPtr<float4> hit;
  float4* lacc;
  SPtr<float2> pfilm;
  ShadowPlanes sh; MisPlanes mi;
  unsigned char* occ_sh; unsigned char* occ_mi;
  const unsigned* q_in; unsigned* q_shadow; unsigned* q_mis; unsigned* q_misany;
  const unsigned* cnt_in; unsigned* cnt_out; unsigned shard_cap;
  int all_in_bounds;
  int fresh;
#ifndef RT_FRESH_RECORDS
#define RT_FRESH_RECORDS 3
#endif
#ifndef RT_FRESH_RECORDS_LDS
#define RT_FRESH_RECORDS_LDS 2
#endif
#define RT_FRESH_BETA(ps) (((ps).fresh & 1) != 0)
#define RT_FRESH_ST(ps) (((ps).fresh & 2) != 0)
  int shadow_sets;
  int mis_any;
  int skip_unreachable_mis;
  int skip_dead_tail;
  const unsigned* range;
  unsigned long long* stats;
};
#define RT_NQ 4
#define RT_SHADOW_WALK 0u
#define RT_SHADOW_EMPTY 1u
#define RT_SHADOW_KIND(w) ((w) & 3u)
enum { ST_CAMERA = 0, ST_RAYS_CLOSEST, ST_RAYS_SHADOW, ST_RAYS_MIS, ST_NODES_CLOSEST, ST_NODES_SHADOW, ST_NODES_MIS,
       ST_TRIS_CLOSEST, ST_TRIS_SHADOW, ST_TRIS_MIS, ST_SCRUBBED, ST_UNBUILT_VOXEL,
       ST_RAYS_MISANY, ST_NODES_MISANY, ST_TRIS_MISANY,
       ST_MIS_UNREACHED,
       ST_TAIL_UNCAST,
       ST_SHADED,
       ST_STAMP = ST_SHADED + 4,
       ST_SHADOW_SETS = ST_STAMP + 32,
       ST_COUNT };
#ifdef RT_ABLATE
#define RT_STAMP(k) do { const unsigned long long t_ = clock64(); stamp_acc[k] += t_ - stamp_last; stamp_last = t_; } while (0)
#else
#define RT_STAMP(k) do { } while (0)
#endif

RT_DEV void split_path_id(const PassState& ps, unsigned pid, unsigned& sl, unsigned& pix) {
  unsigned q = __umulhi(pid, ps.n_pixels_recip), r = pid - q * ps.n_pixels;
  if (r >= ps.n_pixels) { q += 1u; r -= ps.n_pixels; }
  sl = q; pix = r;
}

struct FrameParams {
  float r2c[16]; float c2w[16]; f3 dx_camera, dy_camera; float lens_radius, focal_distance;
  int crop_x0, crop_y0, crop_x1, crop_y1; int sb_x0, sb_y0, sb_x1, sb_y1;
  float radius_x, radius_y, max_sample_luminance;
  int max_depth; float rr_threshold; int pb_x0, pb_y0, pb_x1, pb_y1;
  int rank, world, shard_log2;
  unsigned long long chunk_first;
  unsigned w_recip;
};

#define RT_STATE_OUT_OF_BOUNDS (1u << 17)
RT_DEV unsigned pack_state(int bounces, bool spec, int c1, int c2) { return (unsigned)bounces | ((unsigned)spec << 8) | ((unsigned)c1 << 9) | ((unsigned)c2 << 13); }

RT_DEV unsigned wave_push(unsigned* counter, bool pred) {
  unsigned long long mask = __ballot(pred);
  if (mask == 0ull) return 0u;
  unsigned lane = __lane_id();
  int leader = __ffsll((long long)mask) - 1;
  unsigned base = 0;
  if ((int)lane == leader) base = atomicAdd(counter, (unsigned)__popcll(mask));
  base = __shfl(base, leader);
  return base + (unsigned)__popcll(mask & ((1ull << lane) - 1ull));
}

#define RT_QSHARDS 8
#ifndef RT_CNT_STRIDE
#define RT_CNT_STRIDE 64
#endif
struct QView {
  const unsigned* ids; unsigned pre[RT_QSHARDS + 1]; unsigned shard_cap;
  RT_DEV void init(const unsigned* ids_, const unsigned* counts, unsigned cap) {
    ids = ids_; shard_cap = cap; pre[0] = 0;
// ... 579 lines not shown
    }
  }
  return found;
}
template <int N, int T, bool FINITE, int LEAF_MIN, int GENERAL = 0>
RT_DEV bool occluded_small_links_rounds(const float* __restrict__ s_nodes, const float* __restrict__ s_tris, const unsigned* __restrict__ link, const int n_nodes, const int start, const Ray ray, const GeneralCtx gen = GeneralCtx{nullptr, false}) {
  const f3 inv_dir = mk3(1.0f / ray.d.x, 1.0f / ray.d.y, 1.0f / ray.d.z);
  const int neg_x = inv_dir.x < 0.0f, neg_y = inv_dir.y < 0.0f, neg_z = inv_dir.z < 0.0f;
  const RayPre rp = ray_pre(ray);
  const float* const tpx = s_tris + rp.kx * T; const float* const tpy = s_tris + rp.ky * T; const float* const tpz = s_tris + rp.kz * T;
  const f3 op = permute(ray.o, rp.kx, rp.ky, rp.kz);
  bool found = false;
  int cur = start, leaf_off = 0, leaf_n = 0;
  for (;;) {
    unsigned long long holders = 0ull;
    for (;;) {
      if (leaf_n == 0 && cur < n_nodes) {
        const float* nd = s_nodes + cur;
        const float4 n0 = make_float4(nd[0], nd[2 * N], nd[4 * N], nd[N]), n1 = make_float4(nd[3 * N], nd[5 * N], 0.0f, 0.0f);
        const unsigned lk = link[cur];
        int next = (int)(lk & 0xffffu);
        if (slab_test_t<FINITE>(n0, n1, ray, inv_dir, neg_x, neg_y, neg_z)) {
          if ((int)lk < 0) { leaf_off = RT_LINK_LEAF_OFF(lk, N); leaf_n = RT_LINK_LEAF_N(lk, N); }
          else next = (int)(lk >> 16);
        }
        cur = next;
      }
      holders = __ballot(leaf_n > 0);
      if (__ballot(leaf_n == 0 && cur < n_nodes) == 0ull) break;
      if (__builtin_popcount((unsigned)holders) + __builtin_popcount((unsigned)(holders >> 32)) >= LEAF_MIN) break;
    }
    if (holders == 0ull) break;
    if (leaf_n > 0) {
      const int t = leaf_off;
      TriHit h;
      leaf_off += 1; leaf_n -= 1;
      if (GENERAL) { if (leaf_prim_test<GENERAL>(LdsSrcT<N, T>{s_nodes, s_tris}, gen, t, ray, rp, h)) { found = true; cur = n_nodes; leaf_n = 0; } }
      else { const f3 p0t = mk3(tpx[t] - op.x, tpy[t] - op.y, tpz[t] - op.z), p1t = mk3(tpx[3 * T + t] - op.x, tpy[3 * T + t] - op.y, tpz[3 * T + t] - op.z), p2t = mk3(tpx[6 * T + t] - op.x, tpy[6 * T + t] - op.y, tpz[6 * T + t] - op.z);
        if (tri_test_permuted<RT_ANY_EARLY_SIGN != 0>(p0t, p1t, p2t, rp.sx, rp.sy, rp.sz, ray.t_max, h)) { found = true; cur = n_nodes; leaf_n = 0; } }
    }
  }
  return found;
}


struct TraceIO {
  SPtr<const float4> ray_o; SPtr<const float4> ray_d; unsigned ray_stride;
  SPtr<float4> hits; unsigned hit_stride; int hit_b2;
  unsigned* occluded; unsigned occ_stride;
  float4* lacc; unsigned lacc_stride; SPtr<const float4> direct_add; unsigned add_stride;
  int shadow_masks;
  int queue_is_slots;
  unsigned long long* hit_mask;
};
template <class AddPtr>
RT_DEV void trace_write_any(float4* __restrict__ lacc, size_t ls, const AddPtr direct_add, size_t as, unsigned* __restrict__ occluded, size_t os,
                            unsigned pid, float dw, bool found) {
  if (lacc != nullptr && (__float_as_uint(dw) >> 31) != 0u) {
    if (!found) { const size_t path = __float_as_uint(dw) & 0x7fffffffu; float4 a = direct_add[pid * as]; float4 l = lacc[path * ls]; lacc[path * ls] = make_float4(l.x + a.x, l.y + a.y, l.z + a.z, l.w); }
  } else if (os == 0) ((unsigned char*)occluded)[pid] = found ? (unsigned char)1 : (unsigned char)0;
  else occluded[pid * os] = found ? 1u : 0u;
}

#ifndef RT_LDS_TRACE_WAVES
#define RT_LDS_TRACE_WAVES 7
#endif
#ifndef RT_LDS_ANY_WAVES
#define RT_LDS_ANY_WAVES 8
#endif
#ifndef RT_MID_LEAF_MIN_ANY
#define RT_MID_LEAF_MIN_ANY 8
#endif
#ifndef RT_LDS_LEAF_MIN_CLOSEST_GENERAL
#define RT_LDS_LEAF_MIN_CLOSEST_GENERAL 16
#endif
#ifndef RT_LDS_LEAF_MIN_ANY_GENERAL
#define RT_LDS_LEAF_MIN_ANY_GENERAL 56
#endif
#ifndef RT_MID_LEAF_MIN_CLOSEST
#define RT_MID_LEAF_MIN_CLOSEST 16
#endif
#define RT_MID_NODES 2816
#define RT_MID_TRIS 1408
template <bool ANY, bool COUNT, int BLOCK, int DEPTH, int GENERAL = 0, int MID = 0>
__global__ void __launch_bounds__(BLOCK, MID ? 4 : ((GENERAL == 0 && !COUNT) ? (ANY ? RT_LDS_ANY_WAVES : RT_LDS_TRACE_WAVES) : RT_GEN_MIN_WAVES(GENERAL))) k_trace(DScene sc, TraceIO io, const unsigned* __restrict__ queue, const unsigned* __restrict__ shard_counts, unsigned shard_cap,
                                                 unsigned count_static, unsigned long long* stats, int st_rays, int st_nodes, int st_tris) {
  const float4* __restrict__ ray_o = sraw(io.ray_o); const float4* __restrict__ ray_d = sraw(io.ray_d); const size_t rs = io.ray_stride;
  float4* __restrict__ hits = sraw(io.hits); const size_t hs = io.hit_stride; const bool hit_b2 = io.hit_b2 != 0;
  unsigned* __restrict__ occluded = io.occluded; const size_t os = io.occ_stride;
  float4* __restrict__ lacc = io.lacc; const size_t ls = io.lacc_stride; const float4* __restrict__ direct_add = sraw(io.direct_add); const size_t as = io.add_stride;
  typedef unsigned short StackT;
  constexpr bool LINKS = !COUNT;
  __shared__ StackT stack[LINKS ? 1 : DEPTH * BLOCK];
  constexpr int NN = MID ? RT_MID_NODES : RT_SMALL_NODES, NT = MID ? RT_MID_TRIS : RT_SMALL_TRIS;
  static_assert(!MID || (!COUNT && GENERAL == 0), "mid-size LDS scenes: plain triangles, no visit counts");
  constexpr bool MIDC = MID != 0 && !ANY;
  typedef LdsSrcT<NN, NT> LdsS;
  __shared__ float s_nodes[(MIDC ? 6 : 8) * NN];
  __shared__ float s_tris[MIDC ? 1 : 10 * NT];
  QView qv; if (queue) qv.init(io.queue_is_slots ? nullptr : queue, shard_counts, shard_cap);
  const unsigned count = queue ? qv.total() : count_static;
  if (blockIdx.x * BLOCK >= count) return;
  __shared__ unsigned s_link[LINKS ? (ANY ? 1 : 8) * NN + 8 : 1];
  stage_small_scene<BLOCK, NN, NT, MIDC>(sc, s_nodes, s_tris); __syncthreads();
  if (LINKS) {
    if (ANY) { for (unsigned k = threadIdx.x; k < sc.n_nodes; k += BLOCK) s_link[k] = sc.link8[8u * sc.n_nodes + 8u + k]; if (threadIdx.x == 0u) s_link[NN] = sc.link8[9u * sc.n_nodes + 8u]; }
// ... 1 lines not shown
      for (unsigned i = threadIdx.x; i < 8u * sc.n_nodes; i += BLOCK) { const unsigned o = i / sc.n_nodes, k = i - o * sc.n_nodes; s_link[o * NN + k] = sc.link8[i]; }
      if (threadIdx.x < 8u) s_link[8 * NN + threadIdx.x] = sc.link8[8u * sc.n_nodes + threadIdx.x];
    }
    __syncthreads();
  }
  const unsigned stride = gridDim.x * BLOCK;
  unsigned n_nodes = 0, n_tris = 0, n_rays = 0;
  auto trace_one = [&](unsigned pid) {
    float4 o4 = ray_o[pid * rs], d4 = ray_d[pid * rs];
    Ray ray; ray.o = mk3(o4.x, o4.y, o4.z); ray.d = mk3(d4.x, d4.y, d4.z); ray.t_max = o4.w;
    int prim = -1; TriHit h; h.t = kInf; h.b0 = h.b1 = h.b2 = 0.0f;
    bool found;
    constexpr int LM = ANY ? (MID ? RT_MID_LEAF_MIN_ANY : (GENERAL ? RT_LDS_LEAF_MIN_ANY_GENERAL : RT_LDS_LEAF_MIN_ANY)) : (MID ? RT_MID_LEAF_MIN_CLOSEST : (GENERAL ? RT_LDS_LEAF_MIN_CLOSEST_GENERAL : RT_LDS_LEAF_MIN_CLOSEST));
    const GeneralCtx gen{sc.self, ANY && io.shadow_masks != 0};
    constexpr bool FIN_FORMS = !COUNT;
    const bool fin = FIN_FORMS && __ballot(!inv_dir_finite(mk3(1.0f / ray.d.x, 1.0f / ray.d.y, 1.0f / ray.d.z))) == 0ull;
    if (LINKS) {
      static_assert(!LINKS || ANY || (LM > 1 && LM < 64), "the closest-hit link walk tests its leaves in phases: 1 < LEAF_MIN < 64");
      if (!ANY) {
        if (fin) found = closest_small_links<NN, NT, true, LM, GENERAL, MIDC>(s_nodes, s_tris, s_link, NN, (int)sc.n_nodes, ray, prim, h, gen, sc.tri_p);
        else found = closest_small_links<NN, NT, false, LM, GENERAL, MIDC>(s_nodes, s_tris, sc.link8_full, (int)sc.n_nodes, (int)sc.n_nodes, ray, prim, h, gen, sc.tri_p);
      } else if (LM > 1 && LM < 64) {
        found = fin ? occluded_small_links_rounds<NN, NT, true, LM, GENERAL>(s_nodes, s_tris, s_link, (int)sc.n_nodes, (int)s_link[NN], ray, gen)
                    : occluded_small_links_rounds<NN, NT, false, LM, GENERAL>(s_nodes, s_tris, sc.link8_full + 8u * sc.n_nodes + 8u, (int)sc.n_nodes, (int)sc.link8_full[9u * sc.n_nodes + 8u], ray, gen);
      } else {
        found = fin ? occluded_small_links<NN, NT, true, GENERAL>(s_nodes, s_tris, s_link, (int)sc.n_nodes, (int)s_link[NN], ray, gen)
                    : occluded_small_links<NN, NT, false, GENERAL>(s_nodes, s_tris, sc.link8_full + 8u * sc.n_nodes + 8u, (int)sc.n_nodes, (int)sc.link8_full[9u * sc.n_nodes + 8u], ray, gen);
      }
    }
    else {
      LdsS src{s_nodes, s_tris};
      found = traverse<ANY, COUNT, LdsS, StackT, GENERAL>(src, ray, stack + threadIdx.x, BLOCK, prim, h, n_nodes, n_tris, gen);
    }
    n_rays += 1;
    if (ANY) trace_write_any(lacc, ls, direct_add, as, occluded, os, pid, d4.w, found);
    else hits[pid * hs] = make_float4(hit_b2 ? h.b2 : (found ? h.t : kInf), __int_as_float(found ? prim : -1), h.b0, h.b1);
    return found;
  };
  for (unsigned i = blockIdx.x * BLOCK + threadIdx.x; i < count; i += stride) {
    const bool found = trace_one(queue ? qv.get(i) : i);
    if constexpr (!ANY) {
      if (io.hit_mask != nullptr) { const unsigned long long m = __ballot(found); if ((threadIdx.x & 63u) == 0u) io.hit_mask[i >> 6] = m; }
    } else (void)found;
  }
  if (stats) {
    for (int off = 32; off > 0; off >>= 1) { n_rays += __shfl_down(n_rays, off); if (COUNT) { n_nodes += __shfl_down(n_nodes, off); n_tris += __shfl_down(n_tris, off); } }
    if ((threadIdx.x & 63u) == 0u) {
      if (n_rays) atomicAdd(&stats[st_rays], (unsigned long long)n_rays);
      if (COUNT) { atomicAdd(&stats[st_nodes], (unsigned long long)n_nodes); atomicAdd(&stats[st_tris], (unsigned long long)n_tris); }
    }
  }
}

struct TraceOut { SPtr<float4> hits; size_t hs; bool hit_b2; unsigned* occluded; size_t os; float4* lacc; size_t ls; SPtr<const float4> direct_add; size_t as; };
RT_DEV TraceOut trace_out_of(const TraceIO& io) {
  TraceOut o; o.hits = io.hits; o.hs = io.hit_stride; o.hit_b2 = io.hit_b2 != 0; o.occluded = io.occluded; o.os = io.occ_stride;
  o.lacc = io.lacc; o.ls = io.lacc_stride; o.direct_add = io.direct_add; o.as = io.add_stride; return o;
}

#ifndef RT_REFILL_MIN
#define RT_REFILL_MIN 16
#endif
struct NestedCtx { const float4* pairs; float* tstack; size_t grid_lanes; };
template <bool ANY, class StackT>
RT_DEV bool nested_pair_walk(const float4* __restrict__ pairs, const float4* __restrict__ nodes, const float4* __restrict__ tri_p, Ray& r, StackT* stack, int stack_stride,
                             float* tstack, size_t grid_lanes, int& prim_out, TriHit& hit_out);
struct ObjWalkOut { int found, prim; float t, b0, b1, b2; unsigned n_nodes, n_tris; };
template <bool ANY, bool COUNT, class StackT, int G>
RT_DEVN ObjWalkOut object_walk_general(const DScene* self, unsigned node_base, unsigned prim_base, float ox, float oy, float oz, float dx, float dy, float dz, float t_max,
                                       StackT* stack, int stack_stride, bool shadow_masks) {
  const DScene& sc = *self;
  Ray r; r.o = mk3(ox, oy, oz); r.d = mk3(dx, dy, dz); r.t_max = t_max;
  const GlobalSrc src{sc.nodes + 2 * (size_t)node_base, sc.tri_p + 3 * (size_t)prim_base};
  const GeneralCtx gen{self, shadow_masks, (int)prim_base};
  ObjWalkOut o{}; TriHit h; h.t = kInf; h.b0 = h.b1 = h.b2 = 0.0f;
  o.found = traverse<ANY, COUNT, GlobalSrc, StackT, G>(src, r, stack, stack_stride, o.prim, h, o.n_nodes, o.n_tris, gen) ? 1 : 0;
  o.t = h.t; o.b0 = h.b0; o.b1 = h.b1; o.b2 = h.b2;
  return o;
}
template <bool ANY, bool COUNT, class StackT, bool MASKS = false, bool QUADRICS = false>
RT_DEV bool instance_intersect(const DScene& sc, unsigned inst, f3 o, f3 d, float& t_max, int& prim_out, TriHit& hit_out, unsigned& n_nodes, unsigned& n_tris,
                               StackT* stack, int stack_stride, NestedCtx nc = NestedCtx{nullptr, nullptr, 0}, bool shadow_masks = false) {
  const DInstance& in = sc.instances[inst];
  Ray r; r.o = xf34_point(in.w2o, o); r.d = xf34_vector(in.w2o, d); r.t_max = t_max;
  bool found;
  constexpr int OBJ_GENERAL = MASKS ? RT_GEN_ALL : (QUADRICS ? RT_GEN_NO_MASKS : 0);
  if (in.n_nodes == 0u) {
    const float4 pa = sc.tri_p[3 * (size_t)in.prim_base], pb = sc.tri_p[3 * (size_t)in.prim_base + 1], pc = sc.tri_p[3 * (size_t)in.prim_base + 2];
    const f3 p0 = mk3(pa.x, pa.y, pa.z), p1 = mk3(pb.x, pb.y, pb.z), p2 = mk3(pc.x, pc.y, pc.z);
    const unsigned flags = __float_as_uint(pc.w);
    if (COUNT) n_tris += 1;
    TriHit h;
    if (OBJ_GENERAL != 0 && (flags & (RT_FLAG_SPHERE | RT_FLAG_GENERAL_TRI))) found = general_prim_test<MASKS, QUADRICS>(*sc.self, (int)in.prim_base, p0, p1, p2, flags, r, ray_pre(r), shadow_masks, h);
    else found = tri_test(p0, p1, p2, r, h);
    if (found) { prim_out = 0; hit_out = h; r.t_max = h.t; }
  } else if (OBJ_GENERAL != 0 && sc.obj_general) {
    const ObjWalkOut w = object_walk_general<ANY, COUNT, StackT, OBJ_GENERAL>(sc.self, in.node_base, in.prim_base, r.o.x, r.o.y, r.o.z, r.d.x, r.d.y, r.d.z, r.t_max, stack, stack_stride, shadow_masks);
    found = w.found != 0;
    if (COUNT) { n_nodes += w.n_nodes; n_tris += w.n_tris; }
    if (found) { prim_out = w.prim; hit_out.t = w.t; hit_out.b0 = w.b0; hit_out.b1 = w.b1; hit_out.b2 = w.b2; if (!ANY) r.t_max = w.t; }
  } else {
    if (!COUNT && nc.pairs != nullptr) {
      found = nested_pair_walk<ANY, StackT>(nc.pairs + 4 * (size_t)in.node_base, sc.nodes + 2 * (size_t)in.node_base, sc.tri_p + 3 * (size_t)in.prim_base, r, stack, stack_stride,
                                            nc.tstack, nc.grid_lanes, prim_out, hit_out);
    } else {
      const GlobalSrc src{sc.nodes + 2 * (size_t)in.node_base, sc.tri_p + 3 * (size_t)in.prim_base};
// ... 1502 lines not shown
```

rustracer_amd/csrc/rtx_link_tables.h:

```cpp
#pragma once
#include <algorithm>
#include <cmath>
#include <cstdint>
#include <cstdio>
#include <cstdlib>
#include <cstring>
#include <functional>
#include <limits>
#include <vector>
#include "../../include/rtx_hip.h"

struct RtLinkTables {
  std::vector<uint16_t> skip8;
  std::vector<uint32_t> link_full, link_kept;
  std::vector<std::vector<char>> kept;
  std::vector<char> any_swap;
  uint32_t nodes_tested = 0;
  size_t n_rays[9] = {0, 0, 0, 0, 0, 0, 0, 0, 0};
  double tests_all[9] = {0, 0, 0, 0, 0, 0, 0, 0, 0}, tests_kept[9] = {0, 0, 0, 0, 0, 0, 0, 0, 0};
};

static void rt_build_link_tables(const rt_scene_desc* desc, bool mid, bool want_stats, RtLinkTables& out) {
    const uint32_t nn = desc->n_nodes;
    std::vector<uint16_t>& skip = out.skip8; skip.assign((size_t)8 * nn, (uint16_t)nn);
    std::vector<uint32_t> st; st.reserve(64);
    for (uint32_t o = 0; o < 8; ++o) {
      st.clear();
      uint32_t cur = 0;
      for (;;) {
        skip[(size_t)o * nn + cur] = (uint16_t)(st.empty() ? nn : st.back());
        const rt_bvh_node& n = desc->nodes[cur];
        if (n.n_prims == 0) {
          const bool neg = ((o >> (n.axis < 2 ? n.axis : 2)) & 1u) != 0u;
          if (neg) { st.push_back(cur + 1); cur = n.offset; } else { st.push_back(n.offset); cur = cur + 1; }
        } else {
          if (st.empty()) break;
          cur = st.back(); st.pop_back();
        }
      }
    }
    std::vector<std::vector<char>>& kept = out.kept; kept.assign(9, std::vector<char>(nn, 1));
    std::vector<char>& any_swap = out.any_swap; any_swap.assign(nn, 0);
    bool nested = nn >= 3;
    for (uint32_t i = 0; i < nn && nested; ++i) {
      const rt_bvh_node& n = desc->nodes[i];
      if (n.n_prims != 0) continue;
      const uint32_t kids[2] = {i + 1, n.offset};
      for (uint32_t c : kids) for (int k = 0; k < 3; ++k) if (!(desc->nodes[c].bmin[k] >= n.bmin[k] && desc->nodes[c].bmax[k] <= n.bmax[k])) nested = false;
    }
    const char* prune_env = getenv("RTX_LDS_PRUNE");
    out.nodes_tested = nn;
    if (nested && !(prune_env && prune_env[0] == '0')) {
      const uint32_t K = nn <= 64 ? 8192u : 4096u;
      struct CalRay { double o[3], d[3], t_max; };
      std::vector<CalRay> rays[9];
      std::vector<double> cum(desc->n_tris + 1, 0.0);
      auto P = [&](uint32_t t, int v, int k) { return (double)desc->tri_p[9 * (size_t)t + 3 * v + k]; };
      auto quadric = [&](uint32_t t, double* c, double* rad) {
        if (!(desc->tri_meta[t].flags & RT_PRIM_SPHERE)) return 0;
        uint32_t k; memcpy(&k, desc->tri_p + 9 * (size_t)t + 6, 4);
        const rt_sphere& q = desc->spheres[k];
        if (q.kind != 0 || q.z_min > -q.radius || q.z_max < q.radius || q.phi_max < 6.28f) return 2;
        for (int a = 0; a < 3; ++a) c[a] = q.o2w[4 * a + 3];
        *rad = (double)q.radius * std::sqrt((double)q.o2w[0] * q.o2w[0] + (double)q.o2w[4] * q.o2w[4] + (double)q.o2w[8] * q.o2w[8]);
        return 1;
      };
      for (uint32_t t = 0; t < desc->n_tris; ++t) {
        double c[3], rad;
        const int qk = quadric(t, c, &rad);
        if (qk) { cum[t + 1] = cum[t] + (qk == 1 ? 12.566370614359172 * rad * rad : 0.0); continue; }
        const double e1[3] = {P(t, 1, 0) - P(t, 0, 0), P(t, 1, 1) - P(t, 0, 1), P(t, 1, 2) - P(t, 0, 2)}, e2[3] = {P(t, 2, 0) - P(t, 0, 0), P(t, 2, 1) - P(t, 0, 1), P(t, 2, 2) - P(t, 0, 2)};
        const double cx = e1[1] * e2[2] - e1[2] * e2[1], cy = e1[2] * e2[0] - e1[0] * e2[2], cz = e1[0] * e2[1] - e1[1] * e2[0];
        const double ar = 0.5 * std::sqrt(cx * cx + cy * cy + cz * cz);
        cum[t + 1] = cum[t] + (ar < 1e300 ? ar : 0.0);
      }
      std::vector<uint32_t> emitters;
      for (uint32_t i = 0; i < desc->n_lights; ++i) if (desc->lights[i].kind == RT_LIGHT_DIFFUSE_AREA && desc->lights[i].prim >= 0 && (uint32_t)desc->lights[i].prim < desc->n_tris) emitters.push_back((uint32_t)desc->lights[i].prim);
      unsigned long long rs = 0x9e3779b97f4a7c15ull;
      auto rnd = [&]() { rs += 0x9e3779b97f4a7c15ull; unsigned long long z = rs; z = (z ^ (z >> 30)) * 0xbf58476d1ce4e5b9ull; z = (z ^ (z >> 27)) * 0x94d049bb133111ebull; z ^= z >> 31; return (double)(z >> 11) * (1.0 / 9007199254740992.0); };
      const rt_bvh_node& root = desc->nodes[0];
      const double ctr[3] = {0.5 * ((double)root.bmin[0] + root.bmax[0]), 0.5 * ((double)root.bmin[1] + root.bmax[1]), 0.5 * ((double)root.bmin[2] + root.bmax[2])};
      auto surface_point = [&](uint32_t t, double* p, double* n) {
        double c[3], rad;
        const int qk = quadric(t, c, &rad);
        if (qk == 2) return false;
        if (qk == 1) {
          const double z = 1.0 - 2.0 * rnd(), rr = std::sqrt(std::max(0.0, 1.0 - z * z)), ph = 6.283185307179586 * rnd();
          n[0] = rr * std::cos(ph); n[1] = rr * std::sin(ph); n[2] = z;
          for (int k = 0; k < 3; ++k) p[k] = c[k] + rad * n[k];
          return true;
        }
        const double su = std::sqrt(rnd()), b0 = 1.0 - su, b1 = rnd() * su, b2 = 1.0 - b0 - b1;
        for (int k = 0; k < 3; ++k) p[k] = b0 * P(t, 0, k) + b1 * P(t, 1, k) + b2 * P(t, 2, k);
        const double e1[3] = {P(t, 1, 0) - P(t, 0, 0), P(t, 1, 1) - P(t, 0, 1), P(t, 1, 2) - P(t, 0, 2)}, e2[3] = {P(t, 2, 0) - P(t, 0, 0), P(t, 2, 1) - P(t, 0, 1), P(t, 2, 2) - P(t, 0, 2)};
        n[0] = e1[1] * e2[2] - e1[2] * e2[1]; n[1] = e1[2] * e2[0] - e1[0] * e2[2]; n[2] = e1[0] * e2[1] - e1[1] * e2[0];
        const double nl = std::sqrt(n[0] * n[0] + n[1] * n[1] + n[2] * n[2]);
        if (!(nl > 0.0)) return false;
        for (int k = 0; k < 3; ++k) n[k] /= nl;
        return true;
      };
      auto prim_hit = [&](const CalRay& cr, uint32_t t) -> double {
        const double none = std::numeric_limits<double>::infinity();
        double sc_[3], srad;
        const int qk = quadric(t, sc_, &srad);
        if (qk == 2) return none;
        if (qk == 1) {
          const double oc[3] = {cr.o[0] - sc_[0], cr.o[1] - sc_[1], cr.o[2] - sc_[2]};
          const double A = cr.d[0] * cr.d[0] + cr.d[1] * cr.d[1] + cr.d[2] * cr.d[2], B = 2.0 * (oc[0] * cr.d[0] + oc[1] * cr.d[1] + oc[2] * cr.d[2]), Cq = oc[0] * oc[0] + oc[1] * oc[1] + oc[2] * oc[2] - srad * srad;
// ... 34 lines not shown
      auto pick_tri = [&]() { const double x = rnd() * cum[desc->n_tris]; return (uint32_t)std::min<size_t>(desc->n_tris - 1, (size_t)(std::upper_bound(cum.begin(), cum.end(), x) - cum.begin()) - 1); };
      static const char* walk_env = getenv("RTX_CAL_WALK"); static const bool walk_on = !(walk_env && walk_env[0] == '0');
      bool have_vertex = false; int depth = 0; double vp[3] = {0, 0, 0}, vn[3] = {0, 0, 1};
      for (uint32_t r = 0; r < K && cum[desc->n_tris] > 0.0; ++r) {
        CalRay cr; cr.t_max = 1e300;
        double n[3];
        if (walk_on && have_vertex && depth < 5) { for (int k = 0; k < 3; ++k) { n[k] = vn[k]; cr.o[k] = vp[k] + n[k] * 1e-6 * (std::fabs(vp[k]) + 1.0); } }
        else {
          const uint32_t t = pick_tri();
          if (!surface_point(t, cr.o, n)) continue;
          const double side = ((ctr[0] - cr.o[0]) * n[0] + (ctr[1] - cr.o[1]) * n[1] + (ctr[2] - cr.o[2]) * n[2]) < 0.0 ? -1.0 : 1.0;
          const double flip = (rnd() < 0.25 ? -1.0 : 1.0) * side;
          for (int k = 0; k < 3; ++k) { n[k] *= flip; cr.o[k] += n[k] * 1e-6 * (std::fabs(cr.o[k]) + 1.0); }
          depth = 0; have_vertex = false;
          if (walk_on) { for (int k = 0; k < 3; ++k) { vp[k] = cr.o[k]; vn[k] = n[k]; } have_vertex = true; }
        }
        if ((r & 3u) == 3u) {
          double q[3], qn[3];
          if (!surface_point(emitters.empty() ? pick_tri() : emitters[(size_t)(rnd() * emitters.size()) % emitters.size()], q, qn)) continue;
          for (int k = 0; k < 3; ++k) cr.d[k] = q[k] - cr.o[k];
          cr.t_max = 1.0 - 1e-4;
          if (cr.d[0] == 0.0 || cr.d[1] == 0.0 || cr.d[2] == 0.0) continue;
          rays[8].push_back(cr);
          continue;
        }
        const double a[3] = {std::fabs(n[0]) > 0.9 ? 0.0 : 1.0, std::fabs(n[0]) > 0.9 ? 1.0 : 0.0, 0.0};
        double tx[3] = {n[1] * a[2] - n[2] * a[1], n[2] * a[0] - n[0] * a[2], n[0] * a[1] - n[1] * a[0]};
        const double tl = std::sqrt(tx[0] * tx[0] + tx[1] * tx[1] + tx[2] * tx[2]);
        for (int k = 0; k < 3; ++k) tx[k] /= tl;
        const double ty[3] = {n[1] * tx[2] - n[2] * tx[1], n[2] * tx[0] - n[0] * tx[2], n[0] * tx[1] - n[1] * tx[0]};
        const double r1 = rnd(), ph = 6.283185307179586 * rnd(), rr = std::sqrt(r1), cz = std::sqrt(1.0 - r1);
        for (int k = 0; k < 3; ++k) cr.d[k] = tx[k] * rr * std::cos(ph) + ty[k] * rr * std::sin(ph) + n[k] * cz;
        if (cr.d[0] == 0.0 || cr.d[1] == 0.0 || cr.d[2] == 0.0) continue;
        rays[(cr.d[0] < 0.0 ? 1 : 0) | (cr.d[1] < 0.0 ? 2 : 0) | (cr.d[2] < 0.0 ? 4 : 0)].push_back(cr);
        if (walk_on) {
          double th; uint32_t hp;
          have_vertex = closest_hit(cr, th, hp);
          if (have_vertex) {
            double c[3], rad;
            for (int k = 0; k < 3; ++k) vp[k] = cr.o[k] + th * cr.d[k];
            if (quadric(hp, c, &rad) == 1) { for (int k = 0; k < 3; ++k) vn[k] = (vp[k] - c[k]) / rad; }
            else {
              const double e1[3] = {P(hp, 1, 0) - P(hp, 0, 0), P(hp, 1, 1) - P(hp, 0, 1), P(hp, 1, 2) - P(hp, 0, 2)}, e2[3] = {P(hp, 2, 0) - P(hp, 0, 0), P(hp, 2, 1) - P(hp, 0, 1), P(hp, 2, 2) - P(hp, 0, 2)};
              vn[0] = e1[1] * e2[2] - e1[2] * e2[1]; vn[1] = e1[2] * e2[0] - e1[0] * e2[2]; vn[2] = e1[0] * e2[1] - e1[1] * e2[0];
              const double nl = std::sqrt(vn[0] * vn[0] + vn[1] * vn[1] + vn[2] * vn[2]);
              if (nl > 0.0) { for (int k = 0; k < 3; ++k) vn[k] /= nl; } else have_vertex = false;
            }
            if (vn[0] * cr.d[0] + vn[1] * cr.d[1] + vn[2] * cr.d[2] > 0.0) for (int k = 0; k < 3; ++k) vn[k] = -vn[k];
            depth += 1;
          }
        }
      }
      const float kNone = std::numeric_limits<float>::infinity(), kUnknown = std::numeric_limits<float>::quiet_NaN();
      std::vector<float> t_node[9], t_prim[9];
      for (int w = 0; w < 9; ++w) { t_node[w].assign(rays[w].size() * nn, kUnknown); t_prim[w].assign(rays[w].size() * (size_t)desc->n_tris, kUnknown); }
      auto node_t = [&](int w, size_t r, uint32_t i) -> float {
        float& out = t_node[w][r * nn + i];
        if (out == out) return out;
        const CalRay& cr = rays[w][r];
        const rt_bvh_node& n = desc->nodes[i];
        double tn = -1e300, tf = 1e300;
        for (int k = 0; k < 3; ++k) { const double iv = 1.0 / cr.d[k]; double a0 = ((double)n.bmin[k] - cr.o[k]) * iv, a1 = ((double)n.bmax[k] - cr.o[k]) * iv; if (a0 > a1) std::swap(a0, a1); tn = std::max(tn, a0); tf = std::min(tf, a1); }
        return out = (tn <= tf && tf > 0.0) ? (float)tn : kNone;
      };
      auto prim_t = [&](int w, size_t r, uint32_t t) -> float {
        float& out = t_prim[w][r * (size_t)desc->n_tris + t];
        if (out == out) return out;
        const double tt = prim_hit(rays[w][r], t);
        return out = tt < 3.0e38 ? (float)tt : kNone;
      };
      auto simulate = [&](int w, std::vector<uint32_t>& n_pass, std::vector<uint32_t>& n_fail) {
        unsigned long long tests = 0;
        std::fill(n_pass.begin(), n_pass.end(), 0u); std::fill(n_fail.begin(), n_fail.end(), 0u);
        std::vector<uint32_t> stk; stk.reserve(64);
        const std::vector<char>& kp = kept[w];
        const unsigned oct = w < 8 ? (unsigned)w : 0u;
        for (size_t r = 0; r < rays[w].size(); ++r) {
          float t_max = (float)std::min(rays[w][r].t_max, 3.0e38); stk.clear(); uint32_t cur = 0; bool done = false;
          while (!done) {
            const rt_bvh_node& n = desc->nodes[cur];
            const bool would = node_t(w, r, cur) < t_max;
            (would ? n_pass : n_fail)[cur] += 1u;
            bool hit = true;
            if (kp[cur]) { tests += 1; hit = would; }
            if (hit && n.n_prims != 0) {
              for (uint32_t t = n.offset; t < n.offset + n.n_prims; ++t) {
                const float tp = prim_t(w, r, t);
                if (tp < t_max) { if (w == 8) { done = true; break; } t_max = tp; }
              }
            }
            if (done) break;
            if (hit && n.n_prims == 0) {
              const bool neg = w < 8 ? ((oct >> (n.axis < 2 ? n.axis : 2)) & 1u) != 0u : any_swap[cur] != 0;
              if (neg) { stk.push_back(cur + 1); cur = n.offset; } else { stk.push_back(n.offset); cur = cur + 1; }
            } else { if (stk.empty()) break; cur = stk.back(); stk.pop_back(); }
          }
        }
        return tests;
      };
      static const char* order_env = getenv("RTX_LDS_ANY_ORDER");
      if (rays[8].size() >= 64 && !(order_env && order_env[0] == '0')) {
        std::vector<double> sum_tests(nn, 0.0); std::vector<uint32_t> occ(nn, 0u);
        struct Res { uint32_t tests; bool occ; };
        for (size_t r = 0; r < rays[8].size(); ++r) {
          const float t_max = (float)std::min(rays[8][r].t_max, 3.0e38);
          std::function<Res(uint32_t)> explore = [&](uint32_t i) -> Res {
            Res res{1u, false};
            if (!(node_t(8, r, i) < t_max)) return res;
            const rt_bvh_node& n = desc->nodes[i];
            if (n.n_prims != 0) { for (uint32_t t = n.offset; t < n.offset + n.n_prims; ++t) if (prim_t(8, r, t) < t_max) res.occ = true; return res; }
            const Res a = explore(i + 1), b = explore(n.offset);
            sum_tests[i + 1] += a.tests; sum_tests[n.offset] += b.tests; occ[i + 1] += a.occ ? 1u : 0u; occ[n.offset] += b.occ ? 1u : 0u;
            res.tests += a.tests + b.tests; res.occ = a.occ || b.occ;
            return res;
          };
          (void)explore(0);
        }
        for (uint32_t i = 0; i < nn; ++i) {
          const rt_bvh_node& n = desc->nodes[i];
          if (n.n_prims == 0) any_swap[i] = (double)occ[n.offset] * sum_tests[i + 1] > (double)occ[i + 1] * sum_tests[n.offset] ? 1 : 0;
        }
      }
      uint32_t nt = 0;
      std::vector<uint32_t> n_pass(nn), n_fail(nn), frontier(nn);
      for (int w = 0; w < 9; ++w) {
        if (rays[w].size() >= 64) {
          for (int sweep = 0; sweep < 6; ++sweep) {
            (void)simulate(w, n_pass, n_fail);
            bool changed = false;
            for (uint32_t i = nn; i-- > 0;) {
              const rt_bvh_node& n = desc->nodes[i];
              if (n.n_prims != 0) { frontier[i] = 1u; continue; }
              const uint32_t a = i + 1, b2 = n.offset;
              frontier[i] = (kept[w][a] ? 1u : frontier[a]) + (kept[w][b2] ? 1u : frontier[b2]);
              const char keep = (n_pass[i] + n_fail[i] < 8u || (unsigned long long)n_fail[i] * (frontier[i] - 1u) > (unsigned long long)n_pass[i]) ? 1 : 0;
              if (keep != kept[w][i]) { kept[w][i] = keep; changed = true; }
            }
            if (!changed) break;
          }
        }
        if (w < 8) for (uint32_t i = 0; i < nn; ++i) nt += kept[w][i] ? 1u : 0u;
      }
      static const bool prune_report = getenv("RTX_PRUNE_REPORT") != nullptr;
      if (prune_report || want_stats) {
        for (int w = 0; w < 9; ++w) if (rays[w].size() >= 64) {
          std::vector<char> sel = kept[w]; kept[w].assign(nn, 1);
          const unsigned long long full = simulate(w, n_pass, n_fail); kept[w] = sel;
          const unsigned long long now = simulate(w, n_pass, n_fail);
          uint32_t k = 0; for (uint32_t i = 0; i < nn; ++i) k += sel[i] ? 1u : 0u;
          out.n_rays[w] = rays[w].size(); out.tests_all[w] = (double)full; out.tests_kept[w] = (double)now;
          if (prune_report) fprintf(stderr, "[rtx] prune set %d: %zu rays, %.2f -> %.2f node tests per ray, %u of %u nodes tested\n", w, rays[w].size(), (double)full / rays[w].size(), (double)now / rays[w].size(), k, nn);
        }
      }
      out.nodes_tested = (nt + 4u) / 8u;
    }
    {
      const size_t tab = (size_t)9 * nn + 9;
      std::vector<uint32_t>& link_full = out.link_full; std::vector<uint32_t>& link_kept = out.link_kept; link_full.assign(tab, 0u); link_kept.assign(tab, 0u);
      std::vector<uint32_t> order; std::vector<uint32_t> pos(nn), end_(nn);
      std::vector<uint32_t> size(nn, 1u);
      for (uint32_t i = nn; i-- > 0;) if (desc->nodes[i].n_prims == 0) size[i] = 1u + size[i + 1] + size[desc->nodes[i].offset];
      for (uint32_t row = 0; row < 9; ++row) {
        const uint32_t o = row < 8 ? row : 0u;
        order.clear(); st.clear();
        uint32_t cur = 0;
        for (;;) {
          pos[cur] = (uint32_t)order.size(); order.push_back(cur);
          const rt_bvh_node& n = desc->nodes[cur];
          if (n.n_prims == 0) {
            const bool neg = row < 8 ? ((o >> (n.axis < 2 ? n.axis : 2)) & 1u) != 0u : any_swap[cur] != 0;
            if (neg) { st.push_back(cur + 1); cur = n.offset; } else { st.push_back(n.offset); cur = cur + 1; }
          } else { if (st.empty()) break; cur = st.back(); st.pop_back(); }
        }
        for (uint32_t i = 0; i < nn; ++i) end_[i] = pos[i] + size[i];
        const size_t base = row < 8 ? (size_t)row * nn : (size_t)8 * nn + 8, start_at = row < 8 ? (size_t)8 * nn + row : (size_t)9 * nn + 8;
        for (int which = 0; which < 2; ++which) {
          std::vector<uint32_t>& L = which == 0 ? link_full : link_kept;
          auto tested = [&](uint32_t i) { return which == 0 || kept[row][i] != 0; };
          std::vector<uint32_t> next_tested(nn + 1, nn);
          for (uint32_t p_ = nn; p_-- > 0;) next_tested[p_] = tested(order[p_]) ? order[p_] : next_tested[p_ + 1];
          for (uint32_t i = 0; i < nn; ++i) {
            const uint32_t enter = pos[i] + 1 < end_[i] ? next_tested[pos[i] + 1] : nn;
            const uint32_t skp = end_[i] < nn ? next_tested[end_[i]] : nn;
            const rt_bvh_node& nd = desc->nodes[i];
            const int off_bits = mid ? RT_LINK_OFF_BITS(RT_MID_NODES) : RT_LINK_OFF_BITS(RT_SMALL_NODES);
            L[base + i] = nd.n_prims != 0 ? (0x80000000u | ((uint32_t)nd.n_prims << (16 + off_bits)) | ((uint32_t)nd.offset << 16) | skp) : ((enter << 16) | skp);
          }
          L[start_at] = next_tested[0];
        }
      }
    }
}
```

rustracer_amd/csrc/rtx_scene_plan.h:

```cpp
#pragma once
#include <map>
#include <string>
#include "rtx_link_tables.h"
#include "rtx_shadow_sets.h"

struct RtScenePlan {
  std::vector<float> tri_p;
  std::vector<DInstance> instances;
  std::vector<float> texels; std::vector<DImage> images;
  std::vector<uint32_t> fourier; std::vector<uint64_t> fourier_at;
  std::vector<DTexture> textures;
  std::vector<DMaterial> materials; std::vector<int> mat_kind, mat_table, mat_class;
  unsigned n_code_classes = 0, n_lambert_classes = 0, n_small_classes = 0, n_wide_classes = 0;
  std::vector<uint16_t> prim_class;
  std::vector<DLight> lights; std::vector<float> dist; std::vector<unsigned short> guides;
  int n_infinite = 0, infinite_ids[4] = {0, 0, 0, 0};
  std::vector<float> pairs, top_pairs, quads;
  RtLinkTables links; RtShadowSets shadow;
  uint32_t n_top_nodes = 0, n_top_prims = 0, n_all_lights = 0;
  int stack_depth = 64, quad_stack_depth = 0, needs_differentials = 0, obj_pairs = 0, route_quadric_hits = 0;
  bool small = false, mid = false, general_prims = false, obj_general = false, has_masks = false, has_spheres = false, has_instances = false, masked_emitters = false;
  bool lambert_only = false, lambert_materials = false, lean_shade = false, lean_qlights = false, lds_records = false, lds_records_q = false, lds_tables = false, lds_mats = false;
  bool use_pairs = false, use_top = false, top_for_closest = false, use_quads = false, deep_column = false, shadow_sets = false;
};

static int rt_refuse(std::string& why, int code, const std::string& msg) { why = msg; return code; }
template <class T> static const T* rt_blob_offset(size_t n) { return reinterpret_cast<const T*>(n * sizeof(T)); }
template <class T> static void rt_blob_rebase(const T*& p, const void* blob) { p = reinterpret_cast<const T*>((const char*)blob + reinterpret_cast<uintptr_t>(p)); }
static bool is_const_texture(const rt_scene_desc* desc, int id) { return id >= 0 && (uint32_t)id < desc->n_textures && desc->textures[id].kind == RT_TEX_CONST; }
static long guide_quarters() { return 4; }

static bool sphere_lights_clear(const rt_scene_desc* desc) {
  std::vector<uint32_t> emitters;
  for (uint32_t i = 0; i < desc->n_lights; ++i) {
    const rt_light& l = desc->lights[i];
    if (l.kind != RT_LIGHT_DIFFUSE_AREA || l.prim < 0 || (uint32_t)l.prim >= desc->n_tris) continue;
    if (!(desc->tri_meta[l.prim].flags & RT_PRIM_SPHERE)) continue;
    uint32_t k; memcpy(&k, &desc->tri_p[9 * (size_t)l.prim + 6], 4);
    if (k >= desc->n_spheres || desc->spheres[k].kind != 0) return false;
    emitters.push_back(k);
  }
  if ((double)emitters.size() * (double)desc->n_tris > 2e8) return false;
  for (uint32_t k : emitters) {
    const rt_sphere& sp = desc->spheres[k];
    const double c[3] = {sp.o2w[3], sp.o2w[7], sp.o2w[11]};
    const double r = (double)sp.radius * 1.001 + 1e-6 * std::max(std::max(fabs(c[0]), fabs(c[1])), fabs(c[2])), r2 = r * r;
    for (uint32_t t = 0; t < desc->n_tris; ++t) {
      if (desc->tri_meta[t].flags & (RT_PRIM_SPHERE | RT_PRIM_INSTANCE)) continue;
      const float* q = desc->tri_p + 9 * (size_t)t;
      double a[3], b[3], cc[3];
      for (int j = 0; j < 3; ++j) { a[j] = q[j] - c[j]; b[j] = q[3 + j] - c[j]; cc[j] = q[6 + j] - c[j]; }
      auto dot3 = [](const double* x, const double* y) { return x[0] * y[0] + x[1] * y[1] + x[2] * y[2]; };
      double ab[3], ac[3]; for (int j = 0; j < 3; ++j) { ab[j] = b[j] - a[j]; ac[j] = cc[j] - a[j]; }
      double best[3];
      const double d1 = -dot3(ab, a), d2 = -dot3(ac, a);
      const double d3 = -dot3(ab, b), d4 = -dot3(ac, b), d5 = -dot3(ab, cc), d6 = -dot3(ac, cc);
      const double vc = d1 * d4 - d3 * d2, vb = d5 * d2 - d1 * d6, va = d3 * d6 - d5 * d4;
      if (d1 <= 0 && d2 <= 0) { for (int j = 0; j < 3; ++j) best[j] = a[j]; }
      else if (d3 >= 0 && d4 <= d3) { for (int j = 0; j < 3; ++j) best[j] = b[j]; }
      else if (vc <= 0 && d1 >= 0 && d3 <= 0) { const double v = d1 / (d1 - d3); for (int j = 0; j < 3; ++j) best[j] = a[j] + v * ab[j]; }
      else if (d6 >= 0 && d5 <= d6) { for (int j = 0; j < 3; ++j) best[j] = cc[j]; }
      else if (vb <= 0 && d2 >= 0 && d6 <= 0) { const double w = d2 / (d2 - d6); for (int j = 0; j < 3; ++j) best[j] = a[j] + w * ac[j]; }
      else if (va <= 0 && (d4 - d3) >= 0 && (d5 - d6) >= 0) { const double w = (d4 - d3) / ((d4 - d3) + (d5 - d6)); for (int j = 0; j < 3; ++j) best[j] = b[j] + w * (cc[j] - b[j]); }
      else { const double den = 1.0 / (va + vb + vc), v = vb * den, w = vc * den; for (int j = 0; j < 3; ++j) best[j] = a[j] + ab[j] * v + ac[j] * w; }
      if (!(dot3(best, best) > r2)) return false;
    }
  }
  return true;
}

#define RT_SHADOW_PLAIN_FLAGS (RT_TRI_FLIP | RT_TRI_HAS_N | RT_TRI_HAS_UV | RT_TRI_HAS_S)
// ... 501 lines not shown
    const bool kd_leaf = kd >= 0 && (uint32_t)kd < desc->n_textures && (desc->textures[kd].kind == RT_TEX_CONST || desc->textures[kd].kind == RT_TEX_IMAGE);
    if (!sigma_zero_matte(desc, m) || !is_const_texture(desc, kd)) p.lambert_only = false;
    if (!sigma_zero_matte(desc, m) || !kd_leaf) p.lambert_materials = false;
  }
  for (uint32_t i = 0; i < desc->n_lights; ++i) {
    if (desc->lights[i].kind != RT_LIGHT_DIFFUSE_AREA) all_area_lights = false;
    else if (desc->tri_meta[desc->lights[i].prim].flags & RT_TRI_HAS_ALPHA) p.masked_emitters = true;
  }
  if (p.has_spheres || p.has_instances) p.masked_emitters = true;
  p.lean_shade = !p.masked_emitters && all_area_lights && all_const_textures;
  p.lean_qlights = p.has_spheres && !p.has_instances && !p.has_masks && all_area_lights && all_const_textures && sphere_lights_clear(desc);
  if (!all_area_lights || p.masked_emitters) p.lambert_only = false;
  p.route_quadric_hits = (p.lean_qlights && p.n_code_classes > 1 && !p.lambert_materials) ? 1 : 0;
  p.small = desc->n_nodes <= RT_SMALL_NODES && desc->n_tris <= RT_SMALL_TRIS && !p.has_instances;
  p.mid = !p.small && !p.general_prims && !p.has_instances && desc->n_nodes <= RT_MID_NODES && desc->n_tris <= RT_MID_TRIS;
  for (uint32_t i = 0; i < desc->n_nodes && p.mid; ++i) if (desc->nodes[i].n_prims > 15) p.mid = false;
  const char* ldsrec = getenv("RTX_SHADE_LDSREC");
  p.lds_mats = desc->n_materials <= RT_LDS_MATERIALS && desc->n_textures <= RT_LDS_TEXTURES && !(ldsrec && ldsrec[0] == '0');
  p.lds_tables = p.lds_mats && p.n_all_lights <= RT_LDS_LIGHTS && desc->n_images <= RT_LDS_IMAGES;
  p.lds_records_q = p.lds_mats && p.n_all_lights <= RT_LDS_LIGHTS && desc->n_tris <= RT_SMALL_TRIS && !p.has_instances;
  p.lds_records = p.lds_records_q && p.small && !p.has_spheres;
}

static void pair_record(const rt_bvh_node& a, const rt_bvh_node& b, uint32_t ca, uint32_t cb, float* q) {
  q[0] = a.bmin[0]; q[1] = a.bmin[1]; q[2] = a.bmin[2]; q[3] = a.bmax[0]; q[4] = a.bmax[1]; q[5] = a.bmax[2]; memcpy(q + 6, &ca, 4); memcpy(q + 7, &cb, 4);
  q[8] = b.bmin[0]; q[9] = b.bmin[1]; q[10] = b.bmin[2]; q[11] = b.bmax[0]; q[12] = b.bmax[1]; q[13] = b.bmax[2];
}
static int plan_trees(const rt_scene_desc* desc, RtScenePlan& p, std::string& why) {
  const uint32_t n_top_nodes = p.n_top_nodes, n_top_prims = p.n_top_prims;
  auto tree_depth = [&](uint32_t base, uint32_t nn, uint32_t np, int& maxd) -> bool {
    std::vector<int> depth(nn, 0); maxd = 0;
    for (uint32_t i = 0; i < nn; ++i) {
      const rt_bvh_node& n = desc->nodes[base + i];
      if (n.n_prims == 0) {
        if (i + 1 >= nn || n.offset >= nn || n.offset <= i) return false;
        depth[i + 1] = depth[i] + 1; depth[n.offset] = depth[i] + 1;
      } else if ((uint64_t)n.offset + n.n_prims > np) return false;
      if (depth[i] > maxd) maxd = depth[i];
    }
    return true;
  };
  int maxd = 0;
  if (!tree_depth(0, n_top_nodes, n_top_prims, maxd)) return rt_refuse(why, RT_ERR_INVALID, "malformed BVH");
  if (maxd + 1 > 64) return rt_refuse(why, RT_ERR_INVALID, "BVH deeper than the 64-entry traversal stack");
  int max_obj_depth = 0;
  for (uint32_t k = 0; k < desc->n_instances; ++k) {
    const rt_instance& in = desc->instances[k];
    int od = 0;
    if (in.n_nodes && (!tree_depth(in.node_base, in.n_nodes, in.n_prims, od) || od + 1 > 64)) return rt_refuse(why, RT_ERR_INVALID, "malformed or too deep object BVH");
    if (in.n_nodes) max_obj_depth = std::max(max_obj_depth, od + 1);
  }
  p.stack_depth = maxd + 1 + max_obj_depth;
  p.deep_column = p.stack_depth > 64;
  if (p.small || p.mid) rt_build_link_tables(desc, p.mid, false, p.links);
  const char* sets = getenv("RTX_SHADOW_SETS");
  if (shadow_sets_apply(desc, p.small && !p.general_prims && !p.has_instances) && !(sets && sets[0] == '0')) {
    int32_t lp[2] = {0, 0};
    for (uint32_t k = 0; k < desc->n_lights; ++k) lp[k] = desc->lights[k].prim;
    rt_build_shadow_sets(desc->tri_p, desc->n_tris, lp, (int)desc->n_lights, desc->nodes[0].bmin, desc->nodes[0].bmax, p.shadow);
    p.shadow_sets = p.shadow.empty > 0;
  }
  if (p.small || p.deep_column) return RT_OK;
  const uint32_t n_pair_nodes = n_top_nodes;
  const bool gen = p.general_prims;
  auto general_leaf = [&](const rt_bvh_node& n) {
    for (uint32_t t = n.offset; t < n.offset + n.n_prims; ++t)
      if (desc->tri_meta[t].flags & (RT_TRI_HAS_ALPHA | RT_TRI_HAS_SHADOW_ALPHA | RT_PRIM_SPHERE | RT_PRIM_INSTANCE)) return true;
    return false;
  };
  bool ok = n_pair_nodes < (1u << 29) && n_top_prims < (gen ? (1u << 25) : (1u << 26)) && desc->nodes[0].n_prims <= 32;
  auto code_of = [&](uint32_t base, uint32_t c, bool& good) -> uint32_t {
    const rt_bvh_node& n = desc->nodes[base + c];
    if (n.n_prims > 0) { if (n.n_prims > 32) good = false; return 0x80000000u | n.offset | ((uint32_t)(n.n_prims - 1) << 26) | (base == 0 && gen && general_leaf(n) ? RT_PAIR_GENERAL : 0u); }
    return c | ((uint32_t)n.axis << 29);
  };
  auto pair_tree = [&](uint32_t base, uint32_t nn, bool& good) {
    for (uint32_t i = 0; i < nn && good; ++i) {
      const rt_bvh_node& n = desc->nodes[base + i];
      if (n.n_prims != 0) continue;
      const uint32_t ca = code_of(base, i + 1, good), cb = code_of(base, n.offset, good);
      pair_record(desc->nodes[base + i + 1], desc->nodes[base + n.offset], ca, cb, p.pairs.data() + (size_t)(base + i) * 16);
    }
  };
  p.pairs.assign((size_t)(p.has_instances ? desc->n_nodes : n_pair_nodes) * 16, 0.0f);
  pair_tree(0, n_pair_nodes, ok);
  bool obj_ok = ok && p.has_instances;
  if (obj_ok) {
    std::vector<char> done(desc->n_nodes, 0);
    for (uint32_t k = 0; k < desc->n_instances && obj_ok; ++k) {
      const rt_instance& in = desc->instances[k];
      if (in.n_nodes == 0 || done[in.node_base]) continue;
      done[in.node_base] = 1;
      if (in.n_nodes >= (1u << 29) || in.n_prims >= (1u << 26) || desc->nodes[in.node_base].n_prims > 32) { obj_ok = false; break; }
      pair_tree(in.node_base, in.n_nodes, obj_ok);
    }
  }
  if (!ok) { p.pairs.clear(); return RT_OK; }
  p.use_pairs = true;
  p.obj_pairs = (obj_ok && !p.obj_general) ? 1 : 0;
  if (n_pair_nodes < (1u << 28) && desc->nodes[0].n_prims == 0 && !p.has_instances) {
    std::vector<uint32_t> top; std::vector<int> slot_of(n_pair_nodes, -1);
    top.push_back(0); slot_of[0] = 0;
    for (size_t head = 0; head < top.size(); ++head) {
      const uint32_t P = top[head]; const uint32_t kids[2] = {P + 1, desc->nodes[P].offset};
      for (uint32_t c : kids)
        if (desc->nodes[c].n_prims == 0 && top.size() < RT_TOP_MAX) { slot_of[c] = (int)top.size(); top.push_back(c); }
    }
    p.top_pairs.assign(top.size() * 16, 0.0f);
    for (size_t k = 0; k < top.size(); ++k) {
      uint32_t code[2]; memcpy(code, p.pairs.data() + (size_t)top[k] * 16 + 6, 8);
      for (int side = 0; side < 2; ++side)
        if (!(code[side] & 0x80000000u) && slot_of[code[side] & 0x0fffffffu] >= 0) code[side] = (code[side] & 0x60000000u) | RT_PAIR_TOP | (uint32_t)slot_of[code[side] & 0x0fffffffu];
      pair_record(desc->nodes[top[k] + 1], desc->nodes[desc->nodes[top[k]].offset], code[0], code[1], p.top_pairs.data() + 16 * k);
// ... 51 lines not shown
```

rustracer_amd/csrc/rtx_shadow_sets.h:

```cpp
#pragma once
#include <algorithm>
#include <cmath>
#include <cstdint>
#include <vector>


struct RtShadowSets {
  int nvox[3] = {1, 1, 1};
  int n_lights = 0;
  std::vector<uint32_t> word;
  uint64_t pairs = 0, empty = 0;
};

namespace rtss {
struct D3 { double x, y, z; };
static inline D3 sub(D3 a, D3 b) { return D3{a.x - b.x, a.y - b.y, a.z - b.z}; }
static inline D3 crs(D3 a, D3 b) { return D3{a.y * b.z - a.z * b.y, a.z * b.x - a.x * b.z, a.x * b.y - a.y * b.x}; }
static inline double dot(D3 a, D3 b) { return a.x * b.x + a.y * b.y + a.z * b.z; }
static inline double l1(D3 a) { return std::fabs(a.x) + std::fabs(a.y) + std::fabs(a.z); }
static inline D3 unit(D3 a) { const double l = std::sqrt(dot(a, a)); return l > 0.0 ? D3{a.x / l, a.y / l, a.z / l} : D3{0, 0, 0}; }
struct Box { D3 lo, hi; };
static inline double box_min(const Box& b, D3 a) { return (a.x < 0 ? b.hi.x : b.lo.x) * a.x + (a.y < 0 ? b.hi.y : b.lo.y) * a.y + (a.z < 0 ? b.hi.z : b.lo.z) * a.z; }
static inline double box_max(const Box& b, D3 a) { return (a.x < 0 ? b.lo.x : b.hi.x) * a.x + (a.y < 0 ? b.lo.y : b.hi.y) * a.y + (a.z < 0 ? b.lo.z : b.hi.z) * a.z; }
}

static void rt_shadow_grid(const float wb_min[3], const float wb_max[3], int nvox[3]) {
  const float diag[3] = {wb_max[0] - wb_min[0], wb_max[1] - wb_min[1], wb_max[2] - wb_min[2]};
  const int ext = diag[0] > diag[1] ? (diag[0] > diag[2] ? 0 : 2) : (diag[1] > diag[2] ? 1 : 2);
  for (int i = 0; i < 3; ++i) {
    const float r = roundf(diag[i] / diag[ext] * 64.0f);
    const unsigned v = (r != r || r <= 0.0f) ? 0u : (unsigned)r;
    nvox[i] = (int)(v > 1u ? v : 1u);
  }
}

static void rt_build_shadow_sets(const float* tri_p, uint32_t n_tris, const int32_t* light_prims, int n_lights, const float wb_min[3], const float wb_max[3], RtShadowSets& out) {
  using namespace rtss;
  rt_shadow_grid(wb_min, wb_max, out.nvox);
  out.n_lights = n_lights;
  const int nx = out.nvox[0], ny = out.nvox[1], nz = out.nvox[2];
  const size_t total = (size_t)nx * ny * nz;
  out.word.assign(total * 2, RT_SHADOW_WALK);
  out.pairs = out.empty = 0;
  if (n_lights != 2 || n_tris == 0) return;
  const D3 wmin{wb_min[0], wb_min[1], wb_min[2]}, wmax{wb_max[0], wb_max[1], wb_max[2]};
  const D3 ext = sub(wmax, wmin);
  const double scale = std::max(ext.x, std::max(ext.y, ext.z));
  const double mag = std::max(scale, std::max(std::max(std::fabs(wmin.x), std::fabs(wmax.x)), std::max(std::max(std::fabs(wmin.y), std::fabs(wmax.y)), std::max(std::fabs(wmin.z), std::fabs(wmax.z)))));
  if (!(scale > 0.0) || !(mag <= 64.0 * scale)) return;
  const double PAD_V = 1e-4 * scale + 1e-5 * mag, PAD_O = 2e-4 * mag, PAD_L = 1e-4 * mag, SEP = 1e-4 * mag, COPLANAR = 1e-9 * mag;
  const double ONE_MINUS_TMAX = 0.99e-4;
  const double T_GAP = 5e-5;
  auto vtx = [&](uint32_t t, int k) { const float* p = tri_p + 9 * (size_t)t + 3 * k; return D3{p[0], p[1], p[2]}; };
  std::vector<Box> tbox(n_tris);
  std::vector<D3> tn(n_tris);
  for (uint32_t t = 0; t < n_tris; ++t) {
    const D3 a = vtx(t, 0), b = vtx(t, 1), c = vtx(t, 2);
    tbox[t].lo = D3{std::min(a.x, std::min(b.x, c.x)), std::min(a.y, std::min(b.y, c.y)), std::min(a.z, std::min(b.z, c.z))};
    tbox[t].hi = D3{std::max(a.x, std::max(b.x, c.x)), std::max(a.y, std::max(b.y, c.y)), std::max(a.z, std::max(b.z, c.z))};
    tn[t] = unit(crs(sub(b, a), sub(c, a)));
  }
  auto sdist = [&](uint32_t t, D3 x) { return dot(tn[t], sub(x, vtx(t, 0))); };
  auto coplanar = [&](uint32_t t, uint32_t s) {
    if (dot(tn[t], tn[t]) == 0.0) return false;
    for (int k = 0; k < 3; ++k) if (std::fabs(sdist(t, vtx(s, k))) > COPLANAR) return false;
    return true;
  };
  std::vector<uint32_t> surf;
  for (int z = 0; z < nz; ++z)
    for (int y = 0; y < ny; ++y)
      for (int x = 0; x < nx; ++x) {
        const size_t v = ((size_t)z * ny + y) * nx + x;
        Box vb;
        vb.lo = D3{wmin.x + ext.x * x / nx - PAD_V, wmin.y + ext.y * y / ny - PAD_V, wmin.z + ext.z * z / nz - PAD_V};
        vb.hi = D3{wmin.x + ext.x * (x + 1) / nx + PAD_V, wmin.y + ext.y * (y + 1) / ny + PAD_V, wmin.z + ext.z * (z + 1) / nz + PAD_V};
        surf.clear();
        for (uint32_t t = 0; t < n_tris; ++t) {
          const Box& b = tbox[t];
          if (b.lo.x <= vb.hi.x + PAD_O && b.hi.x >= vb.lo.x - PAD_O && b.lo.y <= vb.hi.y + PAD_O && b.hi.y >= vb.lo.y - PAD_O && b.lo.z <= vb.hi.z + PAD_O && b.hi.z >= vb.lo.z - PAD_O)
            surf.push_back(t);
        }
        if (surf.empty()) continue;
        Box ob;
        ob.lo = D3{vb.lo.x - PAD_O, vb.lo.y - PAD_O, vb.lo.z - PAD_O}; ob.hi = D3{vb.hi.x + PAD_O, vb.hi.y + PAD_O, vb.hi.z + PAD_O};
        for (int l = 0; l < n_lights; ++l) {
          out.pairs += 1;
          const uint32_t lp = (uint32_t)light_prims[l];
          if (lp >= n_tris) continue;
          const D3 L[3] = {vtx(lp, 0), vtx(lp, 1), vtx(lp, 2)};
          auto separated = [&](uint32_t t) {
            const D3 T[3] = {vtx(t, 0), vtx(t, 1), vtx(t, 2)};
            const D3 te[3] = {sub(T[1], T[0]), sub(T[2], T[1]), sub(T[0], T[2])}, le[3] = {sub(L[1], L[0]), sub(L[2], L[1]), sub(L[0], L[2])};
            const D3 ax3[3] = {D3{1, 0, 0}, D3{0, 1, 0}, D3{0, 0, 1}};
            const D3 oc{0.5 * (ob.lo.x + ob.hi.x), 0.5 * (ob.lo.y + ob.hi.y), 0.5 * (ob.lo.z + ob.hi.z)};
            const D3 lc{(L[0].x + L[1].x + L[2].x) / 3.0, (L[0].y + L[1].y + L[2].y) / 3.0, (L[0].z + L[1].z + L[2].z) / 3.0};
            auto test = [&](D3 a) {
              a = unit(a);
              if (dot(a, a) == 0.0) return false;
              double h0 = box_min(ob, a), h1 = box_max(ob, a);
              const double lpad = PAD_L * l1(a);
              for (int k = 0; k < 3; ++k) { const double p = dot(a, L[k]); h0 = std::min(h0, p - lpad); h1 = std::max(h1, p + lpad); }
              double t0 = dot(a, T[0]), t1 = t0;
              for (int k = 1; k < 3; ++k) { const double p = dot(a, T[k]); t0 = std::min(t0, p); t1 = std::max(t1, p); }
              return t1 < h0 - SEP || t0 > h1 + SEP;
            };
            for (int k = 0; k < 3; ++k) if (test(ax3[k])) return true;
            if (test(tn[t]) || test(tn[lp])) return true;
            for (int i = 0; i < 3; ++i) {
              for (int k = 0; k < 3; ++k) if (test(crs(te[i], ax3[k])) || test(crs(te[i], le[k]))) return true;
              if (test(crs(te[i], sub(lc, oc)))) return true;
              for (int k = 0; k < 3; ++k) if (test(crs(te[i], sub(L[k], oc)))) return true;
            }
            return false;
          };
          auto behind = [&](uint32_t t) {
            if (dot(tn[t], tn[t]) == 0.0) return false;
            for (int sg = -1; sg <= 1; sg += 2) {
              auto s = [&](D3 p) { return sg * sdist(t, p); };
              const bool l_in = coplanar(t, lp);
              double st_min = l_in ? 0.0 : std::min(s(L[0]), std::min(s(L[1]), s(L[2]))) - PAD_L * std::sqrt(3.0);
              if (!l_in && !(st_min > 0.0)) continue;
              double so_min = HUGE_VAL, so_max = -HUGE_VAL; bool ok = true;
              for (uint32_t si : surf) {
                if (coplanar(t, si)) {
                  if (l_in) { ok = false; break; }
                  so_min = std::min(so_min, 0.0); so_max = std::max(so_max, PAD_O);
                  continue;
                }
                Box c;
                c.lo = D3{std::max(tbox[si].lo.x - PAD_O, ob.lo.x), std::max(tbox[si].lo.y - PAD_O, ob.lo.y), std::max(tbox[si].lo.z - PAD_O, ob.lo.z)};
                c.hi = D3{std::min(tbox[si].hi.x + PAD_O, ob.hi.x), std::min(tbox[si].hi.y + PAD_O, ob.hi.y), std::min(tbox[si].hi.z + PAD_O, ob.hi.z)};
                const D3 a{sg * tn[t].x, sg * tn[t].y, sg * tn[t].z};
                const double off = sg * dot(tn[t], vtx(t, 0));
                const double mn = box_min(c, a) - off, mx = box_max(c, a) - off;
                if (!(mn >= 0.0)) { ok = false; break; }
                so_min = std::min(so_min, mn); so_max = std::max(so_max, mx);
              }
              if (!ok) continue;
              const double se_min = ONE_MINUS_TMAX * so_min + (1.0 - ONE_MINUS_TMAX) * st_min;
              if (se_min > 0.0 && se_min >= T_GAP * so_max) return true;
            }
            return false;
          };
          bool empty = true;
          for (uint32_t t = 0; t < n_tris && empty; ++t) if (!behind(t) && !separated(t)) empty = false;
          if (empty) { out.word[2 * v + l] = RT_SHADOW_EMPTY; out.empty += 1; }
        }
      }
}
```

rustracer_amd/host.py:

```python
from __future__ import annotations

import ctypes as C
import os
import subprocess

import numpy as np

_HERE = os.path.dirname(os.path.abspath(__file__))
_CSRC = os.path.join(_HERE, "csrc")
_BUILD = os.environ.get("RTX_LIB_DIR") or os.path.join(_CSRC, "_build")
HOST_LIB = os.path.join(_BUILD, "librtx_host.so")
HIP_LIB = os.path.join(_BUILD, "librtx_hip.so")

RT_FLAG_COUNT_TRAVERSAL = 1
RT_FLAG_FILM_ON_DEVICE = 2
RT_FLAG_TIME_KERNELS = 4
RT_FLAG_COUNT_AS_RENDERED = 8
RT_FLAG_REF_STREAM = 16
RT_FLAG_FRAME_STATS = 32
RT_FLAG_FRAME_FEATURES = 64
RT_FEATURE_FLOATS = 16
RT_FEATURE_SAMPLES_MAX = 1 << 25
RT_BSDF_FRONT_AUTO, RT_BSDF_FRONT_GENERIC, RT_BSDF_FRONT_LAMBERT, RT_BSDF_FRONT_TWO_LOBE, RT_BSDF_FRONT_TWO_LOBE_WIDE = range(5)
RT_BSDF_SURFACE_FLOATS = 40
# ... 211 lines not shown
            w2l = None if l.w2l is None else np.ascontiguousarray(l.w2l, np.float32)
            tri = l.tri if getattr(l, "sphere", -1) < 0 else -2 - l.sphere
            _check(L.rtxh_scene_add_light(self.h, l.kind, tri, _p(np.float32(l.rgb)), int(l.two_sided), _p(np.float32(l.vec)), l.mip, _p(l2w), _p(w2l)), "add_light")
        self.bvh_build_ms = None
        if device_bvh:
            ms = C.c_float()
            _check(L.rtxh_scene_commit_device_bvh(self.h, desc.max_prims_per_node, C.byref(ms)), "commit_device_bvh")
            self.bvh_build_ms = ms.value
        else:
            _check(L.rtxh_scene_commit(self.h, desc.max_prims_per_node), "commit")

    def __del__(self):
        try:
            lib().rtxh_scene_free(self.h)
        except Exception:
            pass

    def bvh(self):
        L = lib()
        nn, npr = C.c_int32(), C.c_int32()
        L.rtxh_scene_bvh_sizes(self.h, C.byref(nn), C.byref(npr))
        bounds = np.zeros((nn.value, 6), np.float32)
        offset = np.zeros(nn.value, np.uint32)
        nprims = np.zeros(nn.value, np.uint16)
        axis = np.zeros(nn.value, np.uint8)
        ordered = np.zeros(npr.value, np.int32)
        L.rtxh_scene_bvh_get(self.h, _p(bounds), _p(offset, C.c_uint32), _p(nprims, C.c_uint16), _p(axis, C.c_uint8), _p(ordered, C.c_int32))
        return dict(bounds=bounds, offset=offset, n_prims=nprims, axis=axis, ordered=ordered)

    def bvh_sizes(self):
        nn, npr = C.c_int32(), C.c_int32()
        lib().rtxh_scene_bvh_sizes(self.h, C.byref(nn), C.byref(npr))
        return nn.value, npr.value

    def link_tables(self, mid=False):
        nn = self.bvh_sizes()[0]
        words = 9 * nn + 9
        kept, full, stats = np.zeros(words, np.uint32), np.zeros(words, np.uint32), np.zeros(27, np.float64)
        _check(lib().rtxh_scene_link_tables(self.h, C.c_int32(1 if mid else 0), _p(kept, C.c_uint32), _p(full, C.c_uint32), C.c_uint64(words), _p(stats, C.c_double)), "rtxh_scene_link_tables")

        def split(t):
            rows = np.concatenate([t[:8 * nn].reshape(8, nn), t[8 * nn + 8:9 * nn + 8].reshape(1, nn)])
            return rows, np.concatenate([t[8 * nn:8 * nn + 8], t[9 * nn + 8:9 * nn + 9]])
        (rk, sk), (rf, sf) = split(kept), split(full)
        return dict(kept=rk, full=rf, start_kept=sk, start_full=sf, rays=stats[:9], tests_all=stats[9:18], tests_kept=stats[18:27])

    def shadow_sets(self):
        nv, st = np.zeros(3, np.int32), np.zeros(2, np.uint64)
        _check(lib().rtxh_scene_shadow_sets(self.h, None, C.c_uint64(0), _p(nv, C.c_int32), _p(st, C.c_uint64)), "rtxh_scene_shadow_sets")
        words = np.zeros(2 * int(np.prod(nv)), np.uint32)
        _check(lib().rtxh_scene_shadow_sets(self.h, _p(words, C.c_uint32), C.c_uint64(words.size), _p(nv, C.c_int32), _p(st, C.c_uint64)), "rtxh_scene_shadow_sets")
        return dict(nvox=tuple(int(x) for x in nv), kind=(words & 3).reshape(int(nv[2]), int(nv[1]), int(nv[0]), 2), pairs=int(st[0]), empty=int(st[1]))

    def scene_query(self, what):
        return _check(lib().rtxh_scene_query(self.h, C.c_int32(what)), "scene_query")

    def lds_resident(self):
        return bool(_check(lib().rtxh_scene_query(self.h, 0), "scene_query"))

    def _render_params(self, **kw):
        return render_params(self.desc, **kw)

    def n_lights(self):
        return len(self.desc.lights)

    def table(self, name):
        return scene_table(self.h, name)

    def setup(self, **kw):
        p = self._render_params(**kw)
        r2c = np.zeros((4, 4), np.float32)
        dxdy = np.zeros(6, np.float32)
        table = np.zeros(256, np.float32)
        sb = np.zeros(4, np.int32)
        cr = np.zeros(4, np.int32)
        _check(lib().rtxh_camera_film_setup(C.byref(p), _p(r2c), _p(dxdy), _p(table), _p(sb, C.c_int32), _p(cr, C.c_int32)), "camera_film_setup")
        return dict(raster_to_camera=r2c, dx_camera=dxdy[:3].copy(), dy_camera=dxdy[3:].copy(), filter_table=table, sample_bounds=sb, cropped=cr, params=p)

    def mip_levels(self, mip):
        L = lib()
        w, h = C.c_int32(), C.c_int32()
        n = _check(L.rtxh_mip_level(self.h, mip, 0, C.byref(w), C.byref(h), None), "mip_level")
        out = []
        for lvl in range(n):
            L.rtxh_mip_level(self.h, mip, lvl, C.byref(w), C.byref(h), None)
            a = np.zeros((h.value, w.value, 3), np.float32)
            L.rtxh_mip_level(self.h, mip, lvl, C.byref(w), C.byref(h), _p(a))
            out.append(a)
        return out

    def upload(self, device=-1):
        _check(lib().rtxh_scene_upload(self.h, device), "upload")

    def render(self, rank=0, world_size=1, count_traversal=False, time_kernels=False, device_out=None, stream=0, count_as_rendered=False, ref_stream=False):
        flags = ((RT_FLAG_COUNT_TRAVERSAL if count_traversal else 0) | (RT_FLAG_TIME_KERNELS if time_kernels else 0) |
                 (RT_FLAG_COUNT_AS_RENDERED if count_as_rendered else 0) | (RT_FLAG_REF_STREAM if ref_stream else 0))
        st = self.setup(rank=rank, world_size=world_size)
        cr = st["cropped"]
        w, h = int(cr[2] - cr[0]), int(cr[3] - cr[1])
        p = st["params"]
        stats = Stats()
        if device_out is not None:
            assert tuple(device_out.shape) == (h, w, 4) and device_out.is_contiguous()
            p.flags = flags | RT_FLAG_FILM_ON_DEVICE
            _check(lib().rtxh_render(self.h, C.byref(p), C.c_void_p(stream), C.c_void_p(device_out.data_ptr()), C.byref(stats)), "render")
            return device_out, stats.as_dict()
# ... 483 lines not shown
```

Before: 2152 Msamples/s.

## Add per-voxel shadow-ray link-table rows to prune BVH traversal for light segments

Result: slower. 2104 Msamples/s (-2.2%).

```diff
diff --git a/include/rtx_hip.h b/include/rtx_hip.h
--- a/include/rtx_hip.h
+++ b/include/rtx_hip.h
@@ -208,6 +208,7 @@
 
 int rt_trace_closest(rt_scene* scene, const float* rays, uint64_t n, float* hits, uint64_t counters[2]);
 int rt_trace_any(rt_scene* scene, const float* rays, uint64_t n, uint32_t* occluded, uint64_t counters[2]);
+int rt_trace_any_rows(rt_scene* scene, const float* rays, const uint32_t* row, uint64_t n, uint32_t* occluded);
 int rt_trace_closest_device(rt_scene* scene, const void* d_rays, uint64_t n, void* d_hits, int reps, void* stream, float* ms_per_launch);
 
 int rt_sampler_tables(int32_t spp, int32_t dimensions, uint64_t pixel0, uint64_t n_pixels, uint32_t* scrambles, uint16_t* perms);
@@ -264,6 +265,8 @@
 int rt_scene_query(rt_scene* scene, int32_t what);
 int rt_link_tables(const rt_scene_desc* desc, int32_t mid, uint32_t* link_kept, uint32_t* link_full, uint64_t capacity_words, double* stats);
 int rt_shadow_sets(const rt_scene_desc* desc, uint32_t* words, uint64_t capacity_words, int32_t n_voxels[3], uint64_t* stats);
+int rt_shadow_rows(const rt_scene_desc* desc, uint32_t* words, uint64_t capacity_words, int32_t n_voxels[3], uint32_t* n_rows, uint32_t* links, uint32_t* starts,
+                   uint8_t* leaf_sets, uint8_t* tested, uint64_t capacity_links, double* stats, uint64_t* cand);
 int rt_sizeof(const char* struct_name);
 
 const char* rt_last_error(void);
diff --git a/include/rtx_host.h b/include/rtx_host.h
--- a/include/rtx_host.h
+++ b/include/rtx_host.h
@@ -102,6 +102,9 @@
 int rtxh_scene_device(rtxh_scene*, rt_scene** out);
 int rtxh_scene_link_tables(rtxh_scene*, int32_t mid, uint32_t* link_kept, uint32_t* link_full, uint64_t capacity_words, double* stats);
 int rtxh_scene_shadow_sets(rtxh_scene*, uint32_t* words, uint64_t capacity_words, int32_t n_voxels[3], uint64_t* stats);
+int rtxh_scene_shadow_rows(rtxh_scene*, uint32_t* words, uint64_t capacity_words, int32_t n_voxels[3], uint32_t* n_rows, uint32_t* links, uint32_t* starts,
+                           uint8_t* leaf_sets, uint8_t* tested, uint64_t capacity_links, double* stats, uint64_t* cand);
+int rtxh_trace_any_rows(rtxh_scene*, const float* rays, const uint32_t* row, uint64_t n, uint32_t* occluded);
 int rtxh_sizeof(const char* struct_name);
 const char* rtxh_last_error(void);
 
diff --git a/rustracer_amd/csrc/rtx_hip.hip b/rustracer_amd/csrc/rtx_hip.hip
--- a/rustracer_amd/csrc/rtx_hip.hip
+++ b/rustracer_amd/csrc/rtx_hip.hip
@@ -86,6 +86,7 @@
   bool masked_emitters = false;
   DevBuf ld_func, ld_cdf, ld_int, ld_mark, ld_list, ld_slot, ld_guide, ld_rows8, ld_dense8;
   bool shadow_sets = false; RtShadowSets shadow; DevBuf ld_shadow;
+  DevBuf shadow_row_links; unsigned n_shadow_rows = 0;
   DevBuf self;
   int ld_strategy_built = -1; bool ld_all_voxels = false;
   std::mutex render_mutex;
@@ -340,6 +341,51 @@
   if (words) {
     if (capacity_words < ss.word.size()) return fail(RT_ERR_INVALID, "rt_shadow_sets: capacity too small");
     std::memcpy(words, ss.word.data(), ss.word.size() * 4);
+  }
+  return RT_OK;
+}
+extern "C" int rt_shadow_rows(const rt_scene_desc* desc, uint32_t* words, uint64_t capacity_words, int32_t n_voxels[3], uint32_t* n_rows, uint32_t* links, uint32_t* starts,
+                              uint8_t* leaf_sets, uint8_t* tested, uint64_t capacity_links, double* stats, uint64_t* cand) {
+  if (!desc || !desc->nodes || desc->n_nodes == 0 || !desc->tri_p || !desc->tri_meta || !n_rows) return fail(RT_ERR_INVALID, "null argument");
+  bool plain = desc->n_instances == 0 && desc->n_spheres == 0 && desc->n_nodes <= RT_SMALL_NODES && desc->n_tris <= RT_SMALL_TRIS;
+  for (uint32_t i = 0; i < desc->n_tris && plain; ++i) if (desc->tri_meta[i].flags & ~(uint32_t)RT_SHADOW_PLAIN_FLAGS) plain = false;
+  if (!shadow_sets_apply(desc, plain)) return fail(RT_ERR_INVALID, "not a scene the shadow sets serve (LDS-resident plain triangles, two triangle lights)");
+  {
+    std::vector<uint32_t> lk((size_t)9 * desc->n_nodes + 9), lf((size_t)9 * desc->n_nodes + 9);
+    const int rc = rt_link_tables(desc, 0, lk.data(), lf.data(), lk.size(), nullptr);
+    if (rc != RT_OK) return rc;
+  }
+  int32_t lp[2] = {0, 0};
+  for (uint32_t k = 0; k < desc->n_lights; ++k) lp[k] = desc->lights[k].prim;
+  const char* srows = getenv("RTX_SHADOW_ROWS");
+  const bool with_rows = !(srows && srows[0] == '0');
+  RtShadowSets ss; ss.want_cand = with_rows;
+  rt_build_shadow_sets(desc->tri_p, desc->n_tris, lp, (int)desc->n_lights, desc->nodes[0].bmin, desc->nodes[0].bmax, ss);
+  RtLinkTables lt; RtShadowRows rw;
+  rt_build_link_tables(desc, false, false, lt, with_rows ? &ss : nullptr, with_rows ? &rw : nullptr);
+  if (n_voxels) { n_voxels[0] = ss.nvox[0]; n_voxels[1] = ss.nvox[1]; n_voxels[2] = ss.nvox[2]; }
+  const uint32_t nr = rw.n_rows > 1 ? rw.n_rows : 0u, nn = desc->n_nodes;
+  *n_rows = nr;
+  if (words) {
+    if (capacity_words < ss.word.size()) return fail(RT_ERR_INVALID, "rt_shadow_rows: capacity too small");
+    for (size_t i = 0; i < ss.word.size(); ++i) words[i] = ss.word[i] | ((nr && RT_SHADOW_KIND(ss.word[i]) == RT_SHADOW_WALK) ? (uint32_t)rw.pair_row[i] << 2 : 0u);
+  }
+  if (cand) {
+    if (capacity_words < ss.word.size()) return fail(RT_ERR_INVALID, "rt_shadow_rows: capacity too small");
+    for (size_t i = 0; i < 2 * ss.word.size(); ++i) cand[i] = i < ss.cand.size() ? ss.cand[i] : 0ull;
+  }
+  if (nr && (links || starts || leaf_sets || tested)) {
+    if (capacity_links < (uint64_t)nr * nn) return fail(RT_ERR_INVALID, "rt_shadow_rows: link capacity too small");
+    for (uint32_t r = 0; r < nr; ++r) {
+      if (links) memcpy(links + (size_t)r * nn, rw.link.data() + (size_t)r * nn, (size_t)nn * 4);
+      if (starts) starts[r] = rw.link[(size_t)nr * nn + r];
+      if (leaf_sets) for (uint32_t i = 0; i < nn; ++i) leaf_sets[(size_t)r * nn + i] = (uint8_t)rw.leaf[r][i];
+      if (tested) for (uint32_t i = 0; i < nn; ++i) tested[(size_t)r * nn + i] = (uint8_t)rw.tested[r][i];
+    }
+  }
+  if (stats) for (uint32_t r = 0; r < 16; ++r) {
+    stats[r] = r < nr ? rw.segs[r] : 0.0; stats[16 + r] = r < nr ? rw.nodes_row0[r] : 0.0; stats[32 + r] = r < nr ? rw.nodes_own[r] : 0.0;
+    stats[48 + r] = r < nr ? rw.tris_row0[r] : 0.0; stats[64 + r] = r < nr ? rw.tris_own[r] : 0.0;
   }
   return RT_OK;
 }
@@ -539,6 +585,7 @@
     }
   up_all(s->lights, lights);
   if (links) { up_all(s->link8_full, p.links.link_full); up_all(s->link8, p.links.link_kept); }
+  if (links && p.small && p.shadow_sets && p.rows.n_rows > 1 && p.rows.n_nodes == desc->n_nodes && (size_t)p.rows.n_rows * p.rows.n_nodes <= RT_ROW_WORDS && p.rows.n_rows <= 16) { up_all(s->shadow_row_links, p.rows.link); s->n_shadow_rows = p.rows.n_rows; }
   if (p.use_pairs) up_all(s->pairs, p.pairs);
   if (p.use_top) up_all(s->top_pairs, p.top_pairs);
   if (p.use_quads) up_all(s->quads, p.quads);
@@ -706,6 +753,10 @@
   if (count) launch_trace_c<ANY, true>(s, io, queue, count_ptr, shard_cap, count_static, stats, st_rays, st_nodes, st_tris, stream);
   else launch_trace_c<ANY, false>(s, io, queue, count_ptr, shard_cap, count_static, stats, st_rays, st_nodes, st_tris, stream);
 }
+static bool shadow_rows_apply(const rt_scene* s) { return s->small && !s->general_prims && s->n_shadow_rows > 1; }
+static void launch_trace_rows(rt_scene* s, const TraceIO& io, const unsigned* queue, const unsigned* count_ptr, unsigned shard_cap, unsigned count_static, unsigned long long* stats, int st_rays, hipStream_t stream) {
+  hipLaunchKernelGGL((k_trace_rows<256>), dim3((unsigned)s->n_cu * 8u), dim3(256), 0, stream, s->d, io, s->shadow_row_links.as<unsigned>(), s->n_shadow_rows, queue, count_ptr, shard_cap, count_static, stats, st_rays);
+}
 static TraceIO trace_io_planar(const float4* ro, const float4* rd, float4* hits, unsigned* occ) {
   TraceIO io{}; io.ray_o = ro; io.ray_d = rd; io.ray_stride = 1; io.hits = hits; io.hit_stride = 1; io.hit_b2 = 0; io.occluded = occ; io.occ_stride = 1;
   io.shadow_masks = 1;
@@ -743,6 +794,32 @@
 }
 extern "C" int rt_trace_closest(rt_scene* s, const float* rays, uint64_t n, float* hits, uint64_t counters[2]) { return trace_batch(s, rays, n, false, hits, nullptr, counters); }
 extern "C" int rt_trace_any(rt_scene* s, const float* rays, uint64_t n, uint32_t* occluded, uint64_t counters[2]) { return trace_batch(s, rays, n, true, nullptr, occluded, counters); }
+
+extern "C" int rt_trace_any_rows(rt_scene* s, const float* rays, const uint32_t* row, uint64_t n, uint32_t* occluded) {
+  if (!s || !rays || !row || !occluded || n == 0 || n > 0x7fffffffull) return fail(RT_ERR_INVALID, "bad trace batch");
+  if (!shadow_rows_apply(s)) return fail(RT_ERR_INVALID, "rt_trace_any_rows: the scene has no shadow rows");
+  HIP_TRY(hipSetDevice(s->device));
+  DevBuf ro, rd, out;
+  HIP_TRY(ro.ensure(n * 16)); HIP_TRY(rd.ensure(n * 16)); HIP_TRY(out.ensure(n * 4));
+  std::vector<float> o(n * 4), d(n * 4);
+  const float t_seg = 1.0f - 1e-4f;
+  for (uint64_t i = 0; i < n; ++i) {
+    const float* r = rays + 8 * i;
+    if (r[3] != t_seg) return fail(RT_ERR_INVALID, "rt_trace_any_rows: a ray's t_max is not a shadow segment's");
+    if (row[i] >= s->n_shadow_rows) return fail(RT_ERR_INVALID, "rt_trace_any_rows: row out of range");
+    o[4 * i] = r[0]; o[4 * i + 1] = r[1]; o[4 * i + 2] = r[2]; memcpy(&o[4 * i + 3], &row[i], 4);
+    d[4 * i] = r[4]; d[4 * i + 1] = r[5]; d[4 * i + 2] = r[6]; d[4 * i + 3] = 0.0f;
+  }
+  HIP_TRY(hipMemcpy(ro.p, o.data(), n * 16, hipMemcpyHostToDevice));
+  HIP_TRY(hipMemcpy(rd.p, d.data(), n * 16, hipMemcpyHostToDevice));
+  TraceIO io = trace_io_planar(ro.as<float4>(), rd.as<float4>(), nullptr, out.as<unsigned>());
+  io.shadow_rows = 1;
+  launch_trace_rows(s, io, nullptr, nullptr, 0, (unsigned)n, nullptr, 0, nullptr);
+  HIP_TRY(hipGetLastError());
+  HIP_TRY(hipDeviceSynchronize());
+  HIP_TRY(hipMemcpy(occluded, out.p, n * 4, hipMemcpyDeviceToHost));
+  return RT_OK;
+}
 
 extern "C" int rt_trace_closest_device(rt_scene* s, const void* d_rays, uint64_t n, void* d_hits, int reps, void* stream_, float* ms_per_launch) {
   if (!s || !d_rays || !d_hits || n == 0 || reps <= 0) return fail(RT_ERR_INVALID, "bad arguments");
@@ -1166,6 +1243,8 @@
     io_mis_any = io_mis; io_mis_any.shadow_masks = 0; io_mis_any.hits = nullptr; io_mis_any.occluded = (unsigned*)ps.occ_mi; io_mis_any.occ_stride = 0;
   }
   const bool count = (flags & RT_FLAG_COUNT_TRAVERSAL) != 0;
+  const bool shadow_rows_on = shadow_rows_apply(s) && s->shadow_sets && s->lambert_only && s->lds_records && !count;
+  io_shadow.shadow_rows = shadow_rows_on ? 1 : 0;
   const unsigned pgrid = (unsigned)s->n_cu * 8u;
   const unsigned sblock = 256u, sgrid = pgrid;
   unsigned long long* dstats = s->stats.as<unsigned long long>();
@@ -1226,7 +1305,7 @@
       ps.all_in_bounds = all_in_bounds ? 1 : 0;
       const int fresh_planes = all_in_bounds ? ((s->lambert_only && s->lds_records) ? (shade_split ? 3 : RT_FRESH_RECORDS_LDS) : RT_FRESH_RECORDS) : 0;
       ps.fresh = fresh_planes;
-      ps.shadow_sets = (s->shadow_sets && !count) ? 1 : 0;
+      ps.shadow_sets = (s->shadow_sets && !count) ? (shadow_rows_on ? 3 : 1) : 0;
       ps.mis_any = (has_infinite && (!count || (flags & RT_FLAG_COUNT_AS_RENDERED))) ? 1 : 0;
       static const bool reach_off = env_is("RTX_MIS_REACH", '0');
       ps.skip_unreachable_mis = (!reach_off && (!count || (flags & RT_FLAG_COUNT_AS_RENDERED))) ? 1 : 0;
@@ -1287,7 +1366,8 @@
           if (fsamples) break;
         }
         tm.begin(&stats.ms_trace_any);
-        launch_trace<true>(s, count, io_shadow, ps.q_shadow, ps.cnt_out + RT_QSHARDS * RT_CNT_STRIDE, ps.shard_cap, 0, dstats, ST_RAYS_SHADOW, ST_NODES_SHADOW, ST_TRIS_SHADOW, stream);
+        if (shadow_rows_on) launch_trace_rows(s, io_shadow, ps.q_shadow, ps.cnt_out + RT_QSHARDS * RT_CNT_STRIDE, ps.shard_cap, 0, dstats, ST_RAYS_SHADOW, stream);
+        else launch_trace<true>(s, count, io_shadow, ps.q_shadow, ps.cnt_out + RT_QSHARDS * RT_CNT_STRIDE, ps.shard_cap, 0, dstats, ST_RAYS_SHADOW, ST_NODES_SHADOW, ST_TRIS_SHADOW, stream);
         tm.end();
         tm.begin(&stats.ms_trace_mis);
         launch_trace<false>(s, count, io_mis, ps.q_mis, ps.cnt_out + 2 * RT_QSHARDS * RT_CNT_STRIDE, ps.shard_cap, 0, dstats, ST_RAYS_MIS, ST_NODES_MIS, ST_TRIS_MIS, stream);
diff --git a/rustracer_amd/csrc/rtx_host.cpp b/rustracer_amd/csrc/rtx_host.cpp
--- a/rustracer_amd/csrc/rtx_host.cpp
+++ b/rustracer_amd/csrc/rtx_host.cpp
@@ -1419,6 +1419,19 @@
   rt_scene_desc d = make_desc(s);
   return rt_shadow_sets(&d, words, capacity_words, n_voxels, stats);
 }
+int rtxh_scene_shadow_rows(rtxh_scene* s, uint32_t* words, uint64_t capacity_words, int32_t n_voxels[3], uint32_t* n_rows, uint32_t* links, uint32_t* starts,
+                           uint8_t* leaf_sets, uint8_t* tested, uint64_t capacity_links, double* stats, uint64_t* cand) {
+  if (!s || !s->committed) return fail(RT_ERR_INVALID, "scene not committed");
+  g_err.clear();
+  rt_scene_desc d = make_desc(s);
+  return rt_shadow_rows(&d, words, capacity_words, n_voxels, n_rows, links, starts, leaf_sets, tested, capacity_links, stats, cand);
+}
+int rtxh_trace_any_rows(rtxh_scene* s, const float* rays, const uint32_t* row, uint64_t n, uint32_t* occluded) {
+  if (!s) return fail(RT_ERR_INVALID, "null scene");
+  g_err.clear();
+  if (!s->dev) { int rc = rtxh_scene_upload(s, -1); if (rc != RT_OK) return rc; }
+  return rt_trace_any_rows(s->dev, rays, row, n, occluded);
+}
 int rtxh_sizeof(const char* name) {
   if (!name) return -1;
 #define RTXH_SZ(T) if (!strcmp(name, #T)) return (int)sizeof(T);
diff --git a/rustracer_amd/csrc/rtx_kernels.h b/rustracer_amd/csrc/rtx_kernels.h
--- a/rustracer_amd/csrc/rtx_kernels.h
+++ b/rustracer_amd/csrc/rtx_kernels.h
@@ -48,6 +48,20 @@
 template <class T> __host__ __device__ T* sraw(T* q) { return q; }
 template <bool NT, class T> RT_DEV T* sp(T* q) { return q; }
 #endif
+RT_DEV void rec_st_w(float4* p, unsigned w) {
+#if RT_NT_STREAMS
+  __builtin_nontemporal_store(w, (unsigned*)p + 3);
+#else
+  ((unsigned*)p)[3] = w;
+#endif
+}
+RT_DEV void rec_st_xyz(float4* p, float x, float y, float z) {
+#if RT_NT_STREAMS
+  __builtin_nontemporal_store(x, (float*)p); __builtin_nontemporal_store(y, (float*)p + 1); __builtin_nontemporal_store(z, (float*)p + 2);
+#else
+  ((float*)p)[0] = x; ((float*)p)[1] = y; ((float*)p)[2] = z;
+#endif
+}
 struct PathGen { SPtr<float4> o; SPtr<float4> d; SPtr<float4> beta; SPtr<uint4> st; };
 struct ShadowPlanes { SPtr<float4> o; SPtr<float4> d; SPtr<float4> add; };
 struct MisPlanes { SPtr<float4> o; SPtr<float4> d; SPtr<float4> hit; SPtr<float4> a; SPtr<float4> b; SPtr<float4> c; SPtr<unsigned> flags; };
@@ -91,6 +105,7 @@
 #define RT_SHADOW_WALK 0u
 #define RT_SHADOW_EMPTY 1u
 #define RT_SHADOW_KIND(w) ((w) & 3u)
+#define RT_SHADOW_ROW(w) (((w) >> 2) & 15u)
 enum { ST_CAMERA = 0, ST_RAYS_CLOSEST, ST_RAYS_SHADOW, ST_RAYS_MIS, ST_NODES_CLOSEST, ST_NODES_SHADOW, ST_NODES_MIS,
        ST_TRIS_CLOSEST, ST_TRIS_SHADOW, ST_TRIS_MIS, ST_SCRUBBED, ST_UNBUILT_VOXEL,
        ST_RAYS_MISANY, ST_NODES_MISANY, ST_TRIS_MISANY,
@@ -776,6 +791,7 @@
   int shadow_masks;
   int queue_is_slots;
   unsigned long long* hit_mask;
+  int shadow_rows;
 };
 template <class AddPtr>
 RT_DEV void trace_write_any(float4* __restrict__ lacc, size_t ls, const AddPtr direct_add, size_t as, unsigned* __restrict__ occluded, size_t os,
@@ -883,6 +899,53 @@
   }
 }
 
+#define RT_ROW_WORDS 1536
+#ifndef RT_ROWS_LEAF_MIN
+#define RT_ROWS_LEAF_MIN 1
+#endif
+template <int BLOCK>
+__global__ void __launch_bounds__(BLOCK, RT_LDS_ANY_WAVES) k_trace_rows(DScene sc, TraceIO io, const unsigned* __restrict__ row_links , unsigned n_rows,
+                                                                         const unsigned* __restrict__ queue, const unsigned* __restrict__ shard_counts, unsigned shard_cap, unsigned count_static, unsigned long long* stats, int st_rays) {
+  const float4* __restrict__ ray_o = sraw(io.ray_o); const float4* __restrict__ ray_d = sraw(io.ray_d); const size_t rs = io.ray_stride;
+  unsigned* __restrict__ occluded = io.occluded; const size_t os = io.occ_stride;
+  float4* __restrict__ lacc = io.lacc; const size_t ls = io.lacc_stride; const float4* __restrict__ direct_add = sraw(io.direct_add); const size_t as = io.add_stride;
+  constexpr int NN = RT_SMALL_NODES, NT = RT_SMALL_TRIS;
+  __shared__ float s_nodes[8 * NN];
+  __shared__ float s_tris[10 * NT];
+  __shared__ unsigned s_rows[RT_ROW_WORDS];
+  __shared__ unsigned s_start[16];
+  QView qv; if (queue) qv.init(io.queue_is_slots ? nullptr : queue, shard_counts, shard_cap);
+  const unsigned count = queue ? qv.total() : count_static;
+  if (blockIdx.x * BLOCK >= count) return;
+  stage_small_scene<BLOCK, NN, NT, false>(sc, s_nodes, s_tris);
+  const unsigned nn = sc.n_nodes;
+  const unsigned words = n_rows * nn < (unsigned)RT_ROW_WORDS ? n_rows * nn : (unsigned)RT_ROW_WORDS;
+  for (unsigned k = threadIdx.x; k < words; k += BLOCK) s_rows[k] = row_links[k];
+  if (threadIdx.x < 16u) s_start[threadIdx.x] = threadIdx.x < n_rows ? row_links[n_rows * nn + threadIdx.x] : nn;
+  __syncthreads();
+  const unsigned stride = gridDim.x * BLOCK;
+  unsigned n_rays = 0;
+  for (unsigned i = blockIdx.x * BLOCK + threadIdx.x; i < count; i += stride) {
+    const unsigned pid = queue ? qv.get(i) : i;
+    const float4 o4 = ray_o[pid * rs], d4 = ray_d[pid * rs];
+    Ray ray; ray.o = mk3(o4.x, o4.y, o4.z); ray.d = mk3(d4.x, d4.y, d4.z); ray.t_max = 1.0f - 1e-4f;
+    unsigned row = __float_as_uint(o4.w) & 15u; if (row >= n_rows || (row + 1u) * nn > (unsigned)RT_ROW_WORDS) row = 0u;
+    const bool fin = __ballot(!inv_dir_finite(mk3(1.0f / ray.d.x, 1.0f / ray.d.y, 1.0f / ray.d.z))) == 0ull;
+    const GeneralCtx gen{sc.self, false};
+    bool found;
+    if constexpr (RT_ROWS_LEAF_MIN > 1) found = fin ? occluded_small_links_rounds<NN, NT, true, RT_ROWS_LEAF_MIN, 0>(s_nodes, s_tris, s_rows + row * nn, (int)nn, (int)s_start[row], ray, gen)
+                           : occluded_small_links<NN, NT, false, 0>(s_nodes, s_tris, sc.link8_full + 8u * nn + 8u, (int)nn, (int)sc.link8_full[9u * nn + 8u], ray, gen);
+    else found = fin ? occluded_small_links<NN, NT, true, 0>(s_nodes, s_tris, s_rows + row * nn, (int)nn, (int)s_start[row], ray, gen)
+                           : occluded_small_links<NN, NT, false, 0>(s_nodes, s_tris, sc.link8_full + 8u * nn + 8u, (int)nn, (int)sc.link8_full[9u * nn + 8u], ray, gen);
+    n_rays += 1;
+    trace_write_any(lacc, ls, direct_add, as, occluded, os, pid, d4.w, found);
+  }
+  if (stats) {
+    for (int off = 32; off > 0; off >>= 1) n_rays += __shfl_down(n_rays, off);
+    if ((threadIdx.x & 63u) == 0u && n_rays) atomicAdd(&stats[st_rays], (unsigned long long)n_rays);
+  }
+}
+
 struct TraceOut { SPtr<float4> hits; size_t hs; bool hit_b2; unsigned* occluded; size_t os; float4* lacc; size_t ls; SPtr<const float4> direct_add; size_t as; };
 RT_DEV TraceOut trace_out_of(const TraceIO& io) {
   TraceOut o; o.hits = io.hits; o.hs = io.hit_stride; o.hit_b2 = io.hit_b2 != 0; o.occluded = io.occluded; o.os = io.occ_stride;
diff --git a/rustracer_amd/csrc/rtx_link_tables.h b/rustracer_amd/csrc/rtx_link_tables.h
--- a/rustracer_amd/csrc/rtx_link_tables.h
+++ b/rustracer_amd/csrc/rtx_link_tables.h
@@ -1,5 +1,6 @@
 #pragma once
 #include <algorithm>
+#include <array>
 #include <cmath>
 #include <cstdint>
 #include <cstdio>
@@ -7,8 +8,10 @@
 #include <cstring>
 #include <functional>
 #include <limits>
+#include <map>
 #include <vector>
 #include "../../include/rtx_hip.h"
+#include "rtx_shadow_sets.h"
 
 struct RtLinkTables {
   std::vector<uint16_t> skip8;
@@ -20,7 +23,22 @@
   double tests_all[9] = {0, 0, 0, 0, 0, 0, 0, 0, 0}, tests_kept[9] = {0, 0, 0, 0, 0, 0, 0, 0, 0};
 };
 
-static void rt_build_link_tables(const rt_scene_desc* desc, bool mid, bool want_stats, RtLinkTables& out) {
+#define RT_SHADOW_ROW_WORDS 1536
+#define RT_SHADOW_ROWS_MAX 15
+struct RtShadowRows {
+  uint32_t n_nodes = 0, n_rows = 0;
+  std::vector<uint32_t> link;
+  std::vector<std::vector<char>> leaf;
+  std::vector<std::vector<char>> tested;
+  std::vector<uint8_t> pair_row;
+  std::vector<double> segs, nodes_row0, nodes_own, tris_row0, tris_own;
+};
+static inline uint32_t rt_shadow_rows_budget(uint32_t n_nodes) {
+  if (n_nodes == 0 || RT_SHADOW_ROW_WORDS / n_nodes < 2u) return 0u;
+  return std::min<uint32_t>(RT_SHADOW_ROWS_MAX, RT_SHADOW_ROW_WORDS / n_nodes - 1u);
+}
+
+static void rt_build_link_tables(const rt_scene_desc* desc, bool mid, bool want_stats, RtLinkTables& out, const RtShadowSets* shadow = nullptr, RtShadowRows* rows = nullptr) {
     const uint32_t nn = desc->n_nodes;
     std::vector<uint16_t>& skip = out.skip8; skip.assign((size_t)8 * nn, (uint16_t)nn);
     std::vector<uint32_t> st; st.reserve(64);
@@ -53,7 +71,7 @@
     if (nested && !(prune_env && prune_env[0] == '0')) {
       const uint32_t K = nn <= 64 ? 8192u : 4096u;
       struct CalRay { double o[3], d[3], t_max; };
-      std::vector<CalRay> rays[9];
+      std::vector<CalRay> rays[10];
       std::vector<double> cum(desc->n_tris + 1, 0.0);
       auto P = [&](uint32_t t, int v, int k) { return (double)desc->tri_p[9 * (size_t)t + 3 * v + k]; };
       auto quadric = [&](uint32_t t, double* c, double* rad) {
@@ -194,7 +212,7 @@
         }
       }
       const float kNone = std::numeric_limits<float>::infinity(), kUnknown = std::numeric_limits<float>::quiet_NaN();
-      std::vector<float> t_node[9], t_prim[9];
+      std::vector<float> t_node[10], t_prim[10];
       for (int w = 0; w < 9; ++w) { t_node[w].assign(rays[w].size() * nn, kUnknown); t_prim[w].assign(rays[w].size() * (size_t)desc->n_tris, kUnknown); }
       auto node_t = [&](int w, size_t r, uint32_t i) -> float {
         float& out = t_node[w][r * nn + i];
@@ -295,6 +313,152 @@
         }
       }
       out.nodes_tested = (nt + 4u) / 8u;
+      if (rows) { rows->n_nodes = nn; rows->n_rows = 0; rows->link.clear(); rows->leaf.clear(); rows->tested.clear(); rows->pair_row.clear(); }
+      if (rows && shadow && !mid && shadow->n_lights == 2 && emitters.size() == 2 && !shadow->cand.empty() && shadow->cand.size() == 2 * shadow->word.size() && rt_shadow_rows_budget(nn) > 0u && desc->n_tris <= 128u && nn <= 256u) {
+        typedef std::array<uint64_t, 4> Set;
+        auto set_count = [](const Set& a) { int c = 0; for (int k = 0; k < 4; ++k) c += __builtin_popcountll(a[k]); return c; };
+        auto set_or = [](const Set& a, const Set& b) { Set u; for (int k = 0; k < 4; ++k) u[k] = a[k] | b[k]; return u; };
+        auto set_in = [](const Set& a, const Set& b) { for (int k = 0; k < 4; ++k) if (a[k] & ~b[k]) return false; return true; };
+        std::vector<uint32_t> leaf_of(desc->n_tris, 0u);
+        for (uint32_t i = 0; i < nn; ++i) { const rt_bvh_node& n = desc->nodes[i]; for (uint32_t t = n.offset; n.n_prims != 0 && t < n.offset + n.n_prims; ++t) leaf_of[t] = i; }
+        const size_t n_pairs = shadow->word.size();
+        auto pair_set = [&](size_t pr) {
+          Set s{{0ull, 0ull, 0ull, 0ull}};
+          for (int h = 0; h < 2; ++h) for (uint64_t m = shadow->cand[2 * pr + h]; m != 0ull; m &= m - 1ull) { const uint32_t lf = leaf_of[64u * h + (uint32_t)__builtin_ctzll(m)]; s[lf >> 6] |= 1ull << (lf & 63u); }
+          return s;
+        };
+        std::map<Set, double> weight;
+        for (size_t pr = 0; pr < n_pairs; ++pr) if (shadow->cand[2 * pr] | shadow->cand[2 * pr + 1]) weight[pair_set(pr)] += 1.0;
+        struct Cl { Set s; double w; int n; };
+        std::vector<Cl> cl;
+        for (const auto& kv : weight) cl.push_back(Cl{kv.first, kv.second, set_count(kv.first)});
+        auto merge_cost = [&](const Cl& a, const Cl& b) { return (a.w + b.w) * set_count(set_or(a.s, b.s)) - a.w * a.n - b.w * b.n; };
+        auto merge = [&](size_t i, size_t j) { cl[i].s = set_or(cl[i].s, cl[j].s); cl[i].w += cl[j].w; cl[i].n = set_count(cl[i].s); cl.erase(cl.begin() + (long)j); };
+        const size_t R = rt_shadow_rows_budget(nn);
+        while (cl.size() > std::max<size_t>(R, 256)) {
+          size_t a = 0; for (size_t i = 1; i < cl.size(); ++i) if (cl[i].w < cl[a].w) a = i;
+          size_t b = a == 0 ? 1 : 0; double best = merge_cost(cl[a], cl[b]);
+          for (size_t i = 0; i < cl.size(); ++i) if (i != a) { const double c = merge_cost(cl[a], cl[i]); if (c < best) { best = c; b = i; } }
+          merge(std::min(a, b), std::max(a, b));
+        }
+        while (cl.size() > R) {
+          size_t a = 0, b = 1; double best = merge_cost(cl[0], cl[1]);
+          for (size_t i = 0; i < cl.size(); ++i) for (size_t j = i + 1; j < cl.size(); ++j) { const double c = merge_cost(cl[i], cl[j]); if (c < best) { best = c; a = i; b = j; } }
+          merge(a, b);
+        }
+        std::stable_sort(cl.begin(), cl.end(), [](const Cl& a, const Cl& b) { return a.n != b.n ? a.n < b.n : a.s < b.s; });
+        const uint32_t n_rows = (uint32_t)cl.size() + 1u;
+        rows->leaf.assign(n_rows, std::vector<char>(nn, 0)); rows->tested.assign(n_rows, std::vector<char>(nn, 0));
+        for (uint32_t i = 0; i < nn; ++i) if (desc->nodes[i].n_prims != 0) rows->leaf[0][i] = 1;
+        for (uint32_t r = 1; r < n_rows; ++r) for (uint32_t i = 0; i < nn; ++i) rows->leaf[r][i] = (char)((cl[r - 1].s[i >> 6] >> (i & 63u)) & 1ull);
+        std::map<Set, uint8_t> row_of;
+        for (const auto& kv : weight) { uint8_t r = 0; for (uint32_t k = 1; k < n_rows && r == 0; ++k) if (set_in(kv.first, cl[k - 1].s)) r = (uint8_t)k; row_of[kv.first] = r; }
+        rows->pair_row.assign(n_pairs, 0);
+        for (size_t pr = 0; pr < n_pairs; ++pr) if (shadow->cand[2 * pr] | shadow->cand[2 * pr + 1]) rows->pair_row[pr] = row_of[pair_set(pr)];
+        std::vector<uint8_t> seg_row;
+        {
+          const double wmin[3] = {root.bmin[0], root.bmin[1], root.bmin[2]}, wext[3] = {(double)root.bmax[0] - root.bmin[0], (double)root.bmax[1] - root.bmin[1], (double)root.bmax[2] - root.bmin[2]};
+          for (uint32_t r = 0; r < 2u * K && cum[desc->n_tris] > 0.0; ++r) {
+            CalRay cr; cr.t_max = 1.0 - 1e-4;
+            double n[3], q[3], qn[3], p[3];
+            if (!surface_point(pick_tri(), p, n)) continue;
+            const uint32_t l = rnd() < 0.5 ? 0u : 1u;
+            if (!surface_point(emitters[l], q, qn)) continue;
+            const double side = ((q[0] - p[0]) * n[0] + (q[1] - p[1]) * n[1] + (q[2] - p[2]) * n[2]) < 0.0 ? -1.0 : 1.0;
+            for (int k = 0; k < 3; ++k) { cr.o[k] = p[k] + side * n[k] * 1e-6 * (std::fabs(p[k]) + 1.0); cr.d[k] = q[k] - cr.o[k]; }
+            if (cr.d[0] == 0.0 || cr.d[1] == 0.0 || cr.d[2] == 0.0) continue;
+            size_t vx[3];
+            for (int k = 0; k < 3; ++k) { const double o = wext[k] > 0.0 ? (p[k] - wmin[k]) / wext[k] : 0.0; const long v = (long)(o * shadow->nvox[k]); vx[k] = (size_t)std::min<long>(std::max<long>(v, 0), shadow->nvox[k] - 1); }
+            const size_t pr = 2 * ((vx[2] * (size_t)shadow->nvox[1] + vx[1]) * (size_t)shadow->nvox[0] + vx[0]) + l;
+            if (!(shadow->cand[2 * pr] | shadow->cand[2 * pr + 1])) continue;
+            rays[9].push_back(cr); seg_row.push_back(rows->pair_row[pr]);
+          }
+          t_node[9].assign(rays[9].size() * nn, kUnknown); t_prim[9].assign(rays[9].size() * (size_t)desc->n_tris, kUnknown);
+        }
+        auto simulate_row = [&](const std::vector<uint32_t>& segs, const std::vector<char>& kp, const std::vector<char>& live, std::vector<uint32_t>& n_pass, std::vector<uint32_t>& n_fail, unsigned long long& tri_tests) {
+          unsigned long long tests = 0; tri_tests = 0;
+          std::fill(n_pass.begin(), n_pass.end(), 0u); std::fill(n_fail.begin(), n_fail.end(), 0u);
+          std::vector<uint32_t> stk; stk.reserve(64);
+          if (!live[0]) return tests;
+          for (uint32_t r : segs) {
+            const float t_max = (float)rays[9][r].t_max; stk.clear(); uint32_t cur = 0; bool done = false;
+            while (!done) {
+              const rt_bvh_node& n = desc->nodes[cur];
+              const bool would = node_t(9, r, cur) < t_max;
+              (would ? n_pass : n_fail)[cur] += 1u;
+              bool hit = true;
+              if (kp[cur]) { tests += 1; hit = would; }
+              if (hit && n.n_prims != 0) for (uint32_t t = n.offset; t < n.offset + n.n_prims && !done; ++t) { tri_tests += 1; if (prim_t(9, r, t) < t_max) done = true; }
+              if (done) break;
+              bool moved = false;
+              if (hit && n.n_prims == 0) {
+                const uint32_t first = any_swap[cur] ? n.offset : cur + 1, second = any_swap[cur] ? cur + 1 : n.offset;
+                if (live[second]) stk.push_back(second);
+                if (live[first]) { cur = first; moved = true; }
+              }
+              if (!moved) { if (stk.empty()) break; cur = stk.back(); stk.pop_back(); }
+            }
+          }
+          return tests;
+        };
+        std::vector<uint32_t> order, pos(nn), end_(nn), size(nn, 1u);
+        for (uint32_t i = nn; i-- > 0;) if (desc->nodes[i].n_prims == 0) size[i] = 1u + size[i + 1] + size[desc->nodes[i].offset];
+        {
+          st.clear(); uint32_t cur = 0;
+          for (;;) {
+            pos[cur] = (uint32_t)order.size(); order.push_back(cur);
+            const rt_bvh_node& n = desc->nodes[cur];
+            if (n.n_prims == 0) { if (any_swap[cur]) { st.push_back(cur + 1); cur = n.offset; } else { st.push_back(n.offset); cur = cur + 1; } }
+            else { if (st.empty()) break; cur = st.back(); st.pop_back(); }
+          }
+          for (uint32_t i = 0; i < nn; ++i) end_[i] = pos[i] + size[i];
+        }
+        rows->link.assign((size_t)n_rows * nn + n_rows, 0u);
+        rows->segs.assign(n_rows, 0.0); rows->nodes_row0.assign(n_rows, 0.0); rows->nodes_own.assign(n_rows, 0.0); rows->tris_row0.assign(n_rows, 0.0); rows->tris_own.assign(n_rows, 0.0);
+        std::vector<char> live(nn), kp(nn), live0(nn, 1);
+        std::vector<uint32_t> segs;
+        for (uint32_t r = 0; r < n_rows; ++r) {
+          const std::vector<char>& lf = rows->leaf[r];
+          for (uint32_t i = nn; i-- > 0;) live[i] = desc->nodes[i].n_prims != 0 ? lf[i] : (char)(live[i + 1] | live[desc->nodes[i].offset]);
+          segs.clear();
+          for (uint32_t k = 0; k < (uint32_t)seg_row.size(); ++k) if (seg_row[k] == r) segs.push_back(k);
+          unsigned long long tri_tests = 0;
+          if (r == 0) kp = kept[8];
+          else {
+            for (uint32_t i = 0; i < nn; ++i) kp[i] = live[i];
+            for (int sweep = 0; sweep < 6 && segs.size() >= 64; ++sweep) {
+              (void)simulate_row(segs, kp, live, n_pass, n_fail, tri_tests);
+              bool changed = false;
+              for (uint32_t i = nn; i-- > 0;) {
+                const rt_bvh_node& n = desc->nodes[i];
+                if (n.n_prims != 0) { frontier[i] = 1u; continue; }
+                if (!live[i]) { frontier[i] = 0u; continue; }
+                const uint32_t a = i + 1, b2 = n.offset;
+                frontier[i] = (live[a] ? (kp[a] ? 1u : frontier[a]) : 0u) + (live[b2] ? (kp[b2] ? 1u : frontier[b2]) : 0u);
+                const char keep = (n_pass[i] + n_fail[i] < 8u || (unsigned long long)n_fail[i] * (frontier[i] - 1u) > (unsigned long long)n_pass[i]) ? 1 : 0;
+                if (keep != kp[i]) { kp[i] = keep; changed = true; }
+              }
+              if (!changed) break;
+            }
+          }
+          rows->tested[r] = kp;
+          std::vector<uint32_t> next_tested(nn + 1, nn);
+          for (uint32_t p_ = nn; p_-- > 0;) next_tested[p_] = kp[order[p_]] ? order[p_] : next_tested[p_ + 1];
+          for (uint32_t i = 0; i < nn; ++i) {
+            const uint32_t skp = end_[i] < nn ? next_tested[end_[i]] : nn;
+            uint32_t enter = pos[i] + 1 < end_[i] ? next_tested[pos[i] + 1] : nn;
+            if (enter >= nn || pos[enter] >= end_[i]) enter = skp;
+            const rt_bvh_node& nd = desc->nodes[i];
+            const int off_bits = RT_LINK_OFF_BITS(RT_SMALL_NODES);
+            rows->link[(size_t)r * nn + i] = nd.n_prims != 0 ? (0x80000000u | ((uint32_t)nd.n_prims << (16 + off_bits)) | ((uint32_t)nd.offset << 16) | skp) : ((enter << 16) | skp);
+          }
+          rows->link[(size_t)n_rows * nn + r] = next_tested[0];
+          rows->segs[r] = (double)segs.size();
+          rows->nodes_own[r] = (double)simulate_row(segs, kp, live, n_pass, n_fail, tri_tests); rows->tris_own[r] = (double)tri_tests;
+          rows->nodes_row0[r] = (double)simulate_row(segs, kept[8], live0, n_pass, n_fail, tri_tests); rows->tris_row0[r] = (double)tri_tests;
+        }
+        rows->n_rows = n_rows;
+      }
     }
     {
       const size_t tab = (size_t)9 * nn + 9;
diff --git a/rustracer_amd/csrc/rtx_scene_plan.h b/rustracer_amd/csrc/rtx_scene_plan.h
--- a/rustracer_amd/csrc/rtx_scene_plan.h
+++ b/rustracer_amd/csrc/rtx_scene_plan.h
@@ -16,7 +16,7 @@
   std::vector<DLight> lights; std::vector<float> dist; std::vector<unsigned short> guides;
   int n_infinite = 0, infinite_ids[4] = {0, 0, 0, 0};
   std::vector<float> pairs, top_pairs, quads;
-  RtLinkTables links; RtShadowSets shadow;
+  RtLinkTables links; RtShadowSets shadow; RtShadowRows rows;
   uint32_t n_top_nodes = 0, n_top_prims = 0, n_all_lights = 0;
   int stack_depth = 64, quad_stack_depth = 0, needs_differentials = 0, obj_pairs = 0, route_quadric_hits = 0;
   bool small = false, mid = false, general_prims = false, obj_general = false, has_masks = false, has_spheres = false, has_instances = false, masked_emitters = false;
@@ -624,13 +624,21 @@
   }
   p.stack_depth = maxd + 1 + max_obj_depth;
   p.deep_column = p.stack_depth > 64;
-  if (p.small || p.mid) rt_build_link_tables(desc, p.mid, false, p.links);
   const char* sets = getenv("RTX_SHADOW_SETS");
-  if (shadow_sets_apply(desc, p.small && !p.general_prims && !p.has_instances) && !(sets && sets[0] == '0')) {
+  const char* srows = getenv("RTX_SHADOW_ROWS");
+  const bool with_sets = shadow_sets_apply(desc, p.small && !p.general_prims && !p.has_instances) && !(sets && sets[0] == '0');
+  const bool with_rows = with_sets && !(srows && srows[0] == '0');
+  if (with_sets) {
     int32_t lp[2] = {0, 0};
     for (uint32_t k = 0; k < desc->n_lights; ++k) lp[k] = desc->lights[k].prim;
+    p.shadow.want_cand = with_rows;
     rt_build_shadow_sets(desc->tri_p, desc->n_tris, lp, (int)desc->n_lights, desc->nodes[0].bmin, desc->nodes[0].bmax, p.shadow);
-    p.shadow_sets = p.shadow.empty > 0;
+  }
+  if (p.small || p.mid) rt_build_link_tables(desc, p.mid, false, p.links, with_rows ? &p.shadow : nullptr, with_rows ? &p.rows : nullptr);
+  if (with_sets) {
+    if (p.rows.n_rows > 1) for (size_t i = 0; i < p.shadow.word.size(); ++i) if (RT_SHADOW_KIND(p.shadow.word[i]) == RT_SHADOW_WALK) p.shadow.word[i] |= (uint32_t)p.rows.pair_row[i] << 2;
+    p.shadow.cand.clear(); p.shadow.cand.shrink_to_fit();
+    p.shadow_sets = p.shadow.empty > 0 || p.rows.n_rows > 1;
   }
   if (p.small || p.deep_column) return RT_OK;
   const uint32_t n_pair_nodes = n_top_nodes;
diff --git a/rustracer_amd/csrc/rtx_shadow_sets.h b/rustracer_amd/csrc/rtx_shadow_sets.h
--- a/rustracer_amd/csrc/rtx_shadow_sets.h
+++ b/rustracer_amd/csrc/rtx_shadow_sets.h
@@ -10,6 +10,8 @@
   int n_lights = 0;
   std::vector<uint32_t> word;
   uint64_t pairs = 0, empty = 0;
+  bool want_cand = false;
+  std::vector<uint64_t> cand;
 };
 
 namespace rtss {
@@ -42,6 +44,9 @@
   const size_t total = (size_t)nx * ny * nz;
   out.word.assign(total * 2, RT_SHADOW_WALK);
   out.pairs = out.empty = 0;
+  out.cand.clear();
+  if (out.want_cand && n_tris <= 128) out.cand.assign(total * 4, 0ull);
+  const bool cand = !out.cand.empty();
   if (n_lights != 2 || n_tris == 0) return;
   const D3 wmin{wb_min[0], wb_min[1], wb_min[2]}, wmax{wb_max[0], wb_max[1], wb_max[2]};
   const D3 ext = sub(wmax, wmin);
@@ -143,7 +148,8 @@
             return false;
           };
           bool empty = true;
-          for (uint32_t t = 0; t < n_tris && empty; ++t) if (!behind(t) && !separated(t)) empty = false;
+          for (uint32_t t = 0; t < n_tris && (empty || cand); ++t)
+            if (!behind(t) && !separated(t)) { empty = false; if (cand) out.cand[2 * (2 * v + l) + (t >> 6)] |= 1ull << (t & 63u); }
           if (empty) { out.word[2 * v + l] = RT_SHADOW_EMPTY; out.empty += 1; }
         }
       }
diff --git a/rustracer_amd/host.py b/rustracer_amd/host.py
--- a/rustracer_amd/host.py
+++ b/rustracer_amd/host.py
@@ -287,6 +287,34 @@
         _check(lib().rtxh_scene_shadow_sets(self.h, _p(words, C.c_uint32), C.c_uint64(words.size), _p(nv, C.c_int32), _p(st, C.c_uint64)), "rtxh_scene_shadow_sets")
         return dict(nvox=tuple(int(x) for x in nv), kind=(words & 3).reshape(int(nv[2]), int(nv[1]), int(nv[0]), 2), pairs=int(st[0]), empty=int(st[1]))
 
+    def shadow_rows(self):
+        nn = self.bvh_sizes()[0]
+        nv, nr = np.zeros(3, np.int32), C.c_uint32(0)
+        L = lib()
+        _check(L.rtxh_scene_shadow_sets(self.h, None, C.c_uint64(0), _p(nv, C.c_int32), None), "rtxh_scene_shadow_sets")
+        words = np.zeros(2 * int(np.prod(nv)), np.uint32)
+        cap = 1536 + nn
+        links, starts, stats = np.zeros(cap, np.uint32), np.zeros(16, np.uint32), np.zeros(80, np.float64)
+        leaf, tested = np.zeros(cap, np.uint8), np.zeros(cap, np.uint8)
+        cand = np.zeros(2 * words.size, np.uint64)
+        _check(L.rtxh_scene_shadow_rows(self.h, _p(words, C.c_uint32), C.c_uint64(words.size), _p(nv, C.c_int32), C.byref(nr), _p(links, C.c_uint32), _p(starts, C.c_uint32),
+                                        _p(leaf, C.c_uint8), _p(tested, C.c_uint8), C.c_uint64(cap), _p(stats, C.c_double), _p(cand, C.c_uint64)), "rtxh_scene_shadow_rows")
+        r = int(nr.value)
+        shape = (int(nv[2]), int(nv[1]), int(nv[0]), 2)
+        st = stats.reshape(5, 16)[:, :r]
+        return dict(nvox=tuple(int(x) for x in nv), n_rows=r, words=words.reshape(shape), row=((words >> 2) & 15).reshape(shape), links=links[:r * nn].reshape(r, nn).copy(),
+                    start=starts[:r].copy(), leaf=leaf[:r * nn].reshape(r, nn) > 0, tested=tested[:r * nn].reshape(r, nn) > 0,
+                    cand=cand.reshape(shape + (2,)), segs=st[0], nodes_row0=st[1], nodes_own=st[2], tris_row0=st[3], tris_own=st[4])
+
+    def trace_any_rows(self, rays, rows):
+        rays = np.ascontiguousarray(rays, np.float32)
+        rows = np.ascontiguousarray(rows, np.uint32)
+        n = rays.shape[0]
+        assert rows.shape == (n,)
+        occ = np.zeros(n, np.uint32)
+        _check(lib().rtxh_trace_any_rows(self.h, _p(rays), _p(rows, C.c_uint32), C.c_uint64(n), _p(occ, C.c_uint32)), "trace_any_rows")
+        return occ > 0
+
     def scene_query(self, what):
         return _check(lib().rtxh_scene_query(self.h, C.c_int32(what)), "scene_query")
 
```
